# zxhuang1698/ZeroShape

Hardware: AMD Instinct MI355X
Metric: sdf_query_points_per_sec_vox128 (higher is better)
Workload: dtype f16x3; 1 GPU; compute_level_grid vox_res=128: (128+1)^3 = 2146689 points/image, range [-1.5,1.5], prologue + fused decoder (f32) + sigmoid; batch = n_gpus images, each sharded into equal point ranges, RCCL all_gather for n_gpus>1; global_batch_images=1, weights=seeded random (zeroshape_amd/synthetic.py)

## Files before the change

include/zeroshape_hip.h:

```cpp
#ifndef ZEROSHAPE_HIP_H
#define ZEROSHAPE_HIP_H

#include <stddef.h>
#include <stdint.h>

#ifdef __cplusplus
extern "C" {
#endif

#define ZS_ABI_VERSION 38

int zs_abi_version(void);

const char *zs_last_error(void);


int zs_chamfer_forward(const float *xyz1, const float *xyz2, int b, int n, int m,
                       float *dist1, float *dist2, int *idx1, int *idx2, void *stream);

size_t zs_chamfer_workspace_bytes(int b, int n, int m);
int zs_chamfer_forward_ws(const float *xyz1, const float *xyz2, int b, int n, int m,
                          float *dist1, float *dist2, int *idx1, int *idx2,
                          void *workspace, size_t workspace_bytes, void *stream);

int zs_chamfer_backward(const float *xyz1, const float *xyz2, int b, int n, int m,
                        float *gradxyz1, float *gradxyz2,
                        const float *graddist1, const float *graddist2,
                        const int *idx1, const int *idx2, void *stream);


size_t zs_sdf_program_bytes(void);
size_t zs_sdf_prologue_scratch_bytes(void);
size_t zs_sdf_workspace_bytes(void);
size_t zs_sdf_attn_scratch_bytes(int batch, int m);

int zs_sdf_prologue(void *programs, size_t program_stride_bytes, const float *lat_params,
                    const float *latent_depth, int batch, void *scratch, void *stream);
#define ZS_SDF_POS_PERLAYER 1
int zs_sdf_prologue_ex(void *programs, size_t program_stride_bytes, const float *lat_params,
                       const float *latent_depth, int batch, void *scratch, int flags, void *stream);

int zs_sdf_verdict_stats(const float *got, const float *want, int batch, int m, float flip_band, float tol, float tol_occ,
                         float *stats, int *flags, void *stream);

int zs_sdf_query_points(const void *programs, size_t program_stride_bytes, int batch,
                        const float *points, int m, float *logits, float *attn,
                        const int *tile_mask, void *workspace, void *stream);

int zs_sdf_query_grid(const void *programs, size_t program_stride_bytes, int batch,
                      const float *axis, int G, int slice_begin, int slice_end,
                      int apply_sigmoid, float *out, const int *tile_mask, void *workspace,
                      void *stream);

int zs_sdf_split_programs(const void *programs, size_t program_stride_bytes, void *split_programs,
                          size_t split_stride_bytes, int batch, void *stream);
int zs_sdf_query_points_split(const void *split_programs, size_t program_stride_bytes, int batch,
                              const float *points, int m, float *logits, int *tile_flags,
                              void *workspace, void *stream);
int zs_sdf_query_grid_split(const void *split_programs, size_t program_stride_bytes, int batch,
                            const float *axis, int G, int slice_begin, int slice_end,
                            int apply_sigmoid, float *out, int *tile_flags, void *workspace,
                            void *stream);

int zs_sdf_query_grid_range(const void *programs, size_t program_stride_bytes, int batch,
                            const float *axis, int G, long long point_begin, long long point_end,
                            int apply_sigmoid, float *out, const int *tile_mask, void *workspace,
                            void *stream);
int zs_sdf_query_grid_range_split(const void *split_programs, size_t program_stride_bytes, int batch,
                                  const float *axis, int G, long long point_begin,
                                  long long point_end, int apply_sigmoid, float *out,
                                  int *tile_flags, void *workspace, void *stream);

size_t zs_bf_grid_bytes(void);
size_t zs_bf_scratch_bytes(void);
int zs_bf_lower_bounds(const float *pred, int n, const float *gt_normalized, int m,
                       const float *rotations, int k, float *grid_gt, float *grid_pred,
                       void *scratch, float *lower_bounds, void *stream);

int zs_pose_max_batch(void);
size_t zs_pose_scratch_bytes(int n, int m, int count);
size_t zs_pose_best_bytes(void);
int zs_pose_best_init(float *best, void *stream);
int zs_pose_search_batch(const float *pred, int n, const float *gt_normalized, int m,
                         const float *rotations, const int *order, int count, int index_offset,
                         const float *lower_bound, const float *thresholds6, float *best,
                         void *scratch, void *stream);
size_t zs_pose_grid_bytes(int n, int m, int count);
int zs_pose_gt_grid(const float *gt_normalized, int m, void *grids, void *stream);
int zs_pose_search_batch_grid(const float *pred, int n, const float *gt_normalized, int m, const float *rotations,
                              const int *order, int count, int index_offset, const float *lower_bound,
                              const float *thresholds6, float *best, void *scratch, void *grids, const float *pred_stats,
                              void *stream);
size_t zs_morton_scratch_bytes(int n);
int zs_morton_sort(const float *points, int n, float *sorted, int *perm, float *tile_boxes, int tile, void *scratch,
                   void *stream);
size_t zs_str_scratch_bytes(int n);
int zs_str_sort(const float *points, int n, float *sorted, int *perm, void *scratch, void *stream);
size_t zs_pose_pack_bytes(int points);
int zs_pose_pack(const float *sorted_points, int points, float *pack, void *stream);
size_t zs_pose_sorted_scratch_bytes(int n, int m, int count);
int zs_pose_search_batch_sorted(const float *pred, const float *pred_sorted, int n, const float *gt_sorted,
                                const float *gt_pack, int m, const float *rotations, const int *order, int count,
                                int index_offset, const float *lower_bound, const float *thresholds6, float *best,
                                void *scratch, int mode, void *stream);
int zs_pose_apply(const float *pred, int n, const float *rotations, const int *index, float *out,
                  void *scratch, void *stream);
int zs_normalize_pc(const float *pc, int b, int n, float *out, void *scratch, void *stream);
int zs_standardize_pc(const float *pc, int b, int n, float *out, void *stream);
size_t zs_icp_scratch_bytes(int b);
int zs_icp_step(const float *x1, int n, const float *x2, int m, const int *idx1, int b, float *x1_out, void *scratch,
                void *stream);
int zs_fscore(const float *dist1, int n, const float *dist2, int m, int b, const float *thresholds,
              int n_thresholds, float *out, void *stream);

size_t zs_mc_scratch_bytes(int G);
size_t zs_mesh_sample_scratch_doubles(int n_tris);
int zs_mc_count(const float *vol, int G, float iso, const uint8_t *tri_count, void *scratch,
                int *total, void *stream);
int zs_mc_emit(const float *vol, int G, float iso, const int8_t *tri_table, int table_stride,
               const uint8_t *tri_count, const void *scratch, float scale, float offset,
               float *tris, int n_tris, void *stream);
int zs_mesh_sample(const float *tris, int n_tris, int n_samples, uint64_t seed, double *cum_area,
                   float *points, void *stream);

int zs_intr_param2mtx(const float *params, int batch, int H, int W, float *intr, void *stream);
int zs_unproj_depth(const float *depth, const float *intr, int batch, int H, int W, float *points,
                    void *stream);
int zs_valid_norm_fac(const float *points, const uint8_t *mask, int batch, int n, float *mean,
                      float *max_dist, void *stream);
int zs_masked_resample(const float *map, const float *mask, int batch, int channels, int H, int W,
                       int Ho, int Wo, float bg, float *out, float *mask_out, void *stream);
int zs_seen_surface(const float *depth, const float *intr, const float *mask, int batch, int H, int W,
                    int Ho, int Wo, float *seen_points, float *mean, float *scale, float *coord_dsp,
                    float *mask_dsp, void *stream);
size_t zs_seen_surface_workspace_bytes(int batch);
int zs_seen_surface_ws(const float *depth, const float *intr, const float *mask, int batch, int H, int W,
                       int Ho, int Wo, float *seen_points, float *mean, float *scale, float *coord_dsp,
                       float *mask_dsp, void *workspace, void *stream);

#define ZS_DEPTH_PRED_IS_DISPARITY 1
#define ZS_DEPTH_SOLVE_ONLY 2
int zs_depth_metrics(const float *prediction, const float *target, const float *mask, int batch, int n,
                     int flags, float depth_cap, const float *thresholds,
                     int n_thresholds, float *metrics, float *prediction_depth, float *scale_shift,
                     void *stream);

#define ZS_ACT_NONE 0
#define ZS_ACT_RELU 1
#define ZS_ACT_GELU 2
#define ZS_ACT_RELU_CLAMP1 3
#define ZS_ACT_SOFTPLUS 4
#define ZS_CONV_IN_RELU 1
#define ZS_CONV_FORCE_LARGE 2
#define ZS_CONV_FORCE_SMALL 4
#define ZS_CONV_F16X3 16
#define ZS_CONV_SPLIT_SMALL 32
#define ZS_CONV_STREAM_K 64
#define ZS_CONV_STREAM_K_ALWAYS 256
#define ZS_CONV_W_PRESPLIT 128
#define ZS_CONV_IN_DILATE2 8
#define ZS_CONV_FORCE_TILE256 1024
#define ZS_CONV_OUT_K16 2048
#define ZS_CONV_IN_K16 4096
#define ZS_CONV_IN_UPSAMPLE2 512
size_t zs_conv2d_packed_floats(int Cin, int Cout, int kh, int kw);
int zs_conv2d_presplit_weight(const float *packed_w, float *split_w, int Cin, int Cout, int kh, int kw, void *stream);
int zs_conv2d_presplit_weight_multi(const void *const *packed, void *const *split, const int *cout_pad,
                                    const unsigned long long *pair_prefix, int n, unsigned long long total_pairs,
                                    void *stream);
int zs_conv2d_nhwc(const float *in, const float *packed_w, const float *scale, const float *shift,
                   const float *res1, const float *res2, float *out, int batch, int Hin, int Win, int Cin,
                   int Hout, int Wout, int Cout, int kh, int kw, int stride, int pad_t, int pad_l, int flags,
                   float in_scale, float in_shift, int act, void *stream);
size_t zs_conv2d_splitk_workspace_bytes(void);
int zs_conv2d_nhwc_ws(const float *in, const float *packed_w, const float *scale, const float *shift,
                   const float *res1, const float *res2, float *out, int batch, int Hin, int Win, int Cin,
                   int Hout, int Wout, int Cout, int kh, int kw, int stride, int pad_t, int pad_l, int flags,
                   float in_scale, float in_shift, int act, void *workspace, void *stream);

typedef struct zs_conv_fuse {
    int in_mode, in_tiles, in_groups;
    int in_gshift;
    const float *in_stats, *in_gamma, *in_beta;
    float in_eps;
    int out_mode, out_groups;
    float *out_stats;
} zs_conv_fuse;
int zs_conv2d_nhwc_fused(const float *in, const float *packed_w, const float *scale, const float *shift,
                         const float *res1, const float *res2, float *out, int batch, int Hin, int Win,
                         int Cin, int Hout, int Wout, int Cout, int kh, int kw, int stride, int pad_t,
                         int pad_l, int flags, float in_scale, float in_shift, int act, const zs_conv_fuse *fuse,
                         void *workspace, void *stream);
int zs_conv2d_fused_cols(int M, int Cout);
int zs_conv2d_k16_ok(int M, int Cin, int Cout, int flags, int ln_in_tiles, int row_stats_out, int has_res);
int zs_gn_relu_max_pool_nhwc(const float *x, const float *stats, int tiles, const float *gamma, const float *beta,
                             float *table, float *y, int batch, int Hin, int Win, int C, int Hout, int Wout, int k,
                             int stride, int pad_t, int pad_l, float eps, void *stream);
int zs_group_norm_apply_stats(const float *x, const float *stats, int tiles, const float *gamma, const float *beta,
                              const float *residual, const float *res_stats, int res_tiles, const float *res_gamma,
                              const float *res_beta, float *y, int batch, int HW, int C, float eps, int relu, void *stream);
int zs_conv3x3_tail_nhwc(const float *in, const float *packed_w, const float *scale, const float *shift, float *out,
                         int batch, int H, int W, int Cin, int Cout, int flags, int act, const float *tail_w,
                         const float *tail_b, int tail_act, void *stream);
int zs_group_norm_nhwc(const float *x, const float *gamma, const float *beta, const float *residual, float *y,
                       int batch, int HW, int C, int groups, float eps, int relu, void *stream);
size_t zs_group_norm_workspace_bytes(int batch, int HW, int C, int groups);
int zs_group_norm_nhwc_ws(const float *x, const float *gamma, const float *beta, const float *residual, float *y,
                          int batch, int HW, int C, int groups, float eps, int relu, void *workspace, void *stream);
int zs_layer_norm(const float *x, const float *gamma, const float *beta, float *y, int rows, int C, float eps,
                  void *stream);
int zs_attention(const float *qkv, float *out, int batch, int L, int heads, int head_dim, void *stream);
int zs_attention_split(const float *qkv, float *out, int batch, int L, int heads, int head_dim, void *stream);
int zs_max_pool_nhwc(const float *x, float *y, int batch, int Hin, int Win, int C, int Hout, int Wout, int k,
                     int stride, int pad_t, int pad_l, void *stream);
int zs_global_mean_nhwc(const float *x, float *y, int batch, int HW, int C, void *stream);
int zs_upsample2x_nhwc(const float *x, float *y, int batch, int Hin, int Win, int C, void *stream);
int zs_nchw_to_nhwc(const float *x, const float *mask, float *y, int batch, int C, int HW, int Cpad,
                    void *stream);
int zs_nhwc_to_nchw(const float *x, float *y, int batch, int C, int HW, void *stream);
int zs_assemble_tokens(const float *feat, const float *cls, const float *pos, float *tokens, int batch, int n,
                       int C, void *stream);
int zs_readout_concat(const float *tokens, float *out, int batch, int n, int C, void *stream);
int zs_window_tokens(const float *emb, const uint8_t *mask, const float *invalid_token, const float *cls,
                     const float *pos, float *out, int batch, int H, int W, int C, int win, void *stream);

typedef struct zs_tensor_entry {
    float *param;
    const float *grad;
    float *exp_avg, *exp_avg_sq;
    unsigned long long n;
    float lr, weight_decay;
} zs_tensor_entry;

int zs_pack_conv_weight(const float *w, float *packed, int Cout, int Cin, int cin0, int CinTot, int kh, int kw,
                        int dgrad, void *stream);
typedef struct zs_pack_entry {
    const float *src;
    float *dst;
    int Cout, Cin, cin0, ld, taps, dgrad, K16, NPad;
} zs_pack_entry;
int zs_pack_chunk_elems(void);
int zs_pack_entry_chunks(int Cout, int Cin, int taps, int dgrad, int K16, int NPad);
int zs_pack_conv_weight_multi(const zs_pack_entry *table, const int *chunk_entry, const unsigned long long *chunk_start,
                              int n_chunks, void *stream);
int zs_pack_entry_inline_split(int Cout, int Cin, int taps, int dgrad);
int zs_pack_conv_weight_multi_split(const zs_pack_entry *table, const int *chunk_entry,
                                    const unsigned long long *chunk_start, int n_chunks, float *const *split_dst,
                                    int split_only, void *stream);
size_t zs_conv2d_wgrad_workspace_bytes(int batch, int Hout, int Wout, int Cin, int Cout, int kh, int kw);
int zs_conv2d_wgrad(const float *in, const float *dy, float *dw, float *db, void *workspace, int batch, int Hin, int Win,
                    int CinP, int Hout, int Wout, int Cout, int kh, int kw, int stride, int pad_t, int pad_l,
                    int flags, float in_scale, float in_shift, int Cin, int cin0, int CinTot, int accumulate,
                    void *stream);
int zs_conv2d_dgrad_small_cin(const float *dy, const float *w, float *dx, int batch, int H, int W, int CinP, int Hout,
                              int Wout, int Cout, int kh, int kw, int stride, int pad_t, int pad_l, int Cin, int cin0,
                              int CinTot, float scale, void *stream);
int zs_standardize_weight(const float *w, float *out, int Cout, int n, float eps, void *stream);
typedef struct zs_std_entry {
    const float *w;
    float *out;
    int rows, n;
    float eps;
    int pad;
} zs_std_entry;
int zs_standardize_weight_multi(const zs_std_entry *table, const int *row_prefix, int n_entries, int total_rows, void *stream);
int zs_standardize_weight_bwd(const float *w, const float *grad_out, float *dw, int Cout, int n, float eps,
                              void *stream);
int zs_act_forward(const float *x, float *y, size_t n, int act, float beta, void *stream);
int zs_act_backward(const float *dy, const float *ref, float *dx, size_t n, int act, float beta, void *stream);
int zs_posenc3d(const float *points, size_t n, int L, float *out, int stride, void *stream);
int zs_add_scaled_rows(const float *x, const float *branch, const float *scale, float *y, int batch,
                       size_t per_sample, void *stream);
size_t zs_column_sum_workspace_bytes(int rows, int C);
int zs_column_sum(const float *x, float *out, int rows, int C, float scale, void *workspace, void *stream);
size_t zs_layer_norm_bwd_workspace_bytes(int rows, int C);
int zs_layer_norm_bwd(const float *dy, const float *x, const float *gamma, float *dx, float *dgamma, float *dbeta,
                      int rows, int C, float eps, void *workspace, void *stream);
int zs_layer_norm_bwd_add(const float *dy, const float *x, const float *gamma, const float *add, float *dx, float *dgamma,
                          float *dbeta, int rows, int C, float eps, void *workspace, void *stream);
size_t zs_attention_bwd_workspace_bytes(int batch, int L, int heads);
int zs_attention_bwd(const float *qkv, const float *dout, float *dqkv, void *workspace, int batch, int L, int heads,
                     int head_dim, void *stream);
int zs_point_attention(const float *qkv_points, const float *qkv_latent, float *out, int batch, int M, int Ll,
                       int heads, int head_dim, void *stream);
int zs_point_attention_probs(const float *qkv_points, const float *qkv_latent, float *attn, int batch, int M, int Ll,
                             int heads, int head_dim, float weight, int accumulate, void *stream);
size_t zs_point_attention_bwd_workspace_bytes(int batch, int M, int Ll, int heads);
int zs_point_attention_bwd(const float *qkv_points, const float *qkv_latent, const float *dout, float *dqkv_points,
                           float *dqkv_latent, int accumulate_latent, void *workspace, int batch, int M, int Ll,
                           int heads, int head_dim, void *stream);
size_t zs_bce_logits_workspace_bytes(size_t n);
int zs_bce_logits(const float *logits, const float *sdf, size_t n, float impt_thres, float impt_weight, float *loss,
                  void *workspace, void *stream);
int zs_bce_logits_bwd(const float *logits, const float *sdf, size_t n, float impt_thres, float impt_weight,
                      const float *grad_loss, float *dlogits, void *stream);
int zs_erode_mask(const float *mask, int batch, int H, int W, int pool, float *out, void *stream);
size_t zs_midas_loss_workspace_bytes(int batch);
int zs_midas_loss(const float *prediction, const float *target, const float *mask, int batch, int H, int W, float alpha,
                  int scales, int inverse_depth, float *loss, void *workspace, void *stream);
int zs_midas_loss_bwd(const float *prediction, const float *target, const float *mask, int batch, int H, int W,
                      float alpha, int scales, int inverse_depth, const void *workspace, const float *grad_loss,
                      float *dprediction, void *stream);
int zs_intr_loss(const float *seen_pred, const float *seen_gt, const float *mask, size_t n, float *out2, void *stream);
int zs_intr_loss_bwd(const float *seen_pred, const float *seen_gt, const float *mask, size_t n, const float *out2,
                     const float *grad_loss, float *dseen_pred, void *stream);
int zs_multi_tensor_chunk_elems(void);
int zs_adamw_multi(const zs_tensor_entry *table, const int *chunk_tensor, const unsigned long long *chunk_start,
                   int n_chunks, float beta1, float beta2, float eps, int step, const float *grad_scale,
                   const int *skipped_steps, void *stream);
int zs_copy_multi(const zs_tensor_entry *table, const int *chunk_tensor, const unsigned long long *chunk_start,
                  int n_chunks, float scale, void *stream);
int zs_sumsq_multi(const zs_tensor_entry *table, const int *chunk_tensor, const unsigned long long *chunk_start,
                   int n_chunks, float *partial, float *sumsq, void *stream);

size_t zs_batch_norm_workspace_bytes(int rows, int C);
int zs_batch_norm_train(const float *x, const float *gamma, const float *beta, const float *residual, float *y,
                        float *running_mean, float *running_var, float *save_mean, float *save_rstd, int rows, int C,
                        float eps, float momentum, int relu, void *workspace, void *stream);
int zs_batch_norm_bwd(const float *x, const float *dy, const float *y_relu, const float *gamma, const float *save_mean,
                      const float *save_rstd, float *dx, float *dresidual, float *dgamma, float *dbeta, int rows, int C,
                      void *workspace, void *stream);
size_t zs_group_norm_bwd_workspace_bytes(int batch, int C);
int zs_group_norm_bwd(const float *x, const float *dy, const float *y_relu, const float *gamma, float *dx,
                      float *dresidual, float *dgamma, float *dbeta, int batch, int HW, int C, int groups, float eps,
                      void *workspace, void *stream);
int zs_max_pool_bwd_nhwc(const float *x, const float *dy, float *dx, int batch, int Hin, int Win, int C, int Hout,
                         int Wout, int k, int stride, int pad_t, int pad_l, void *stream);
int zs_global_mean_bwd_nhwc(const float *dy, float *dx, int batch, int HW, int C, void *stream);
int zs_upsample2x_bwd_nhwc(const float *dy, float *dx, int batch, int Hin, int Win, int C, void *stream);
int zs_nhwc_to_nchw_masked(const float *x, const float *mask, float *y, int batch, int C, int HW, int Cpad,
                           void *stream);
int zs_seen_surface_bwd(const float *depth, const float *intr, const float *mask, const float *mean, const float *scale,
                        const float *d_seen_points, const float *d_coord_dsp, int batch, int H, int W, float *d_depth,
                        float *d_intr, void *stream);
int zs_intr_param2mtx_bwd(const float *params, const float *d_intr, int batch, int H, int W, float *d_params,
                          void *stream);
int zs_window_tokens_bwd(const float *d_out, const uint8_t *mask, float *d_emb, float *d_inv_rows, float *d_cls_rows,
                         int batch, int H, int W, int C, int win, void *stream);
int zs_coord_dsp2_bwd(const float *d_dsp, const float *mask, const float *mask_dsp, float *d_full, int batch, int H,
                      int W, void *stream);
int zs_transform_points(const float *points, const float *pose, const float *mean, const float *scale, float *out,
                        int batch, int n, void *stream);
int zs_resize_bilinear_nhwc(const float *x, float *y, int Hi, int Wi, int Ho, int Wo, int C, int backward,
                            void *stream);
int zs_readout_concat_bwd(const float *dout, float *dtokens, int batch, int n, int C, void *stream);

#ifdef __cplusplus
}
#endif
#endif
```

zeroshape_amd/_lib.py:

```python
import contextlib
import ctypes
import os

_HERE = os.path.dirname(os.path.abspath(__file__))
LIB_PATH = os.environ.get("ZS_LIB_PATH") or os.path.join(_HERE, "libzeroshape_hip.so")

_c_void_p = ctypes.c_void_p
_c_int = ctypes.c_int
_c_size_t = ctypes.c_size_t
_c_float = ctypes.c_float

class ConvFuse(ctypes.Structure):
    _fields_ = [("in_mode", ctypes.c_int), ("in_tiles", ctypes.c_int), ("in_groups", ctypes.c_int), ("in_gshift", ctypes.c_int),
                ("in_stats", ctypes.c_void_p), ("in_gamma", ctypes.c_void_p), ("in_beta", ctypes.c_void_p),
                ("in_eps", ctypes.c_float), ("out_mode", ctypes.c_int), ("out_groups", ctypes.c_int),
                ("out_stats", ctypes.c_void_p)]


SIGNATURES = {
    "zs_abi_version": (_c_int, []),
    "zs_last_error": (ctypes.c_char_p, []),
    "zs_chamfer_forward": (_c_int, [_c_void_p, _c_void_p, _c_int, _c_int, _c_int,
                                    _c_void_p, _c_void_p, _c_void_p, _c_void_p, _c_void_p]),
    "zs_chamfer_workspace_bytes": (_c_size_t, [_c_int, _c_int, _c_int]),
    "zs_chamfer_forward_ws": (_c_int, [_c_void_p, _c_void_p, _c_int, _c_int, _c_int,
                                       _c_void_p, _c_void_p, _c_void_p, _c_void_p, _c_void_p, _c_size_t,
                                       _c_void_p]),
    "zs_chamfer_backward": (_c_int, [_c_void_p, _c_void_p, _c_int, _c_int, _c_int,
                                     _c_void_p, _c_void_p, _c_void_p, _c_void_p,
                                     _c_void_p, _c_void_p, _c_void_p]),
    "zs_sdf_program_bytes": (_c_size_t, []),
    "zs_sdf_prologue_scratch_bytes": (_c_size_t, []),
    "zs_sdf_workspace_bytes": (_c_size_t, []),
    "zs_sdf_attn_scratch_bytes": (_c_size_t, [_c_int, _c_int]),
    "zs_sdf_prologue": (_c_int, [_c_void_p, _c_size_t, _c_void_p, _c_void_p, _c_int,
                                 _c_void_p, _c_void_p]),
    "zs_sdf_prologue_ex": (_c_int, [_c_void_p, _c_size_t, _c_void_p, _c_void_p, _c_int,
                                    _c_void_p, _c_int, _c_void_p]),
    "zs_sdf_verdict_stats": (_c_int, [_c_void_p, _c_void_p, _c_int, _c_int, _c_float, _c_float, _c_float, _c_void_p, _c_void_p,
                                      _c_void_p]),
    "zs_sdf_query_points": (_c_int, [_c_void_p, _c_size_t, _c_int, _c_void_p, _c_int,
                                     _c_void_p, _c_void_p, _c_void_p, _c_void_p, _c_void_p]),
    "zs_sdf_query_grid": (_c_int, [_c_void_p, _c_size_t, _c_int, _c_void_p, _c_int, _c_int,
                                   _c_int, _c_int, _c_void_p, _c_void_p, _c_void_p, _c_void_p]),
    "zs_sdf_split_programs": (_c_int, [_c_void_p, _c_size_t, _c_void_p, _c_size_t, _c_int, _c_void_p]),
    "zs_sdf_query_points_split": (_c_int, [_c_void_p, _c_size_t, _c_int, _c_void_p, _c_int,
                                           _c_void_p, _c_void_p, _c_void_p, _c_void_p]),
    "zs_sdf_query_grid_split": (_c_int, [_c_void_p, _c_size_t, _c_int, _c_void_p, _c_int, _c_int,
                                         _c_int, _c_int, _c_void_p, _c_void_p, _c_void_p, _c_void_p]),
    "zs_sdf_query_grid_range": (_c_int, [_c_void_p, _c_size_t, _c_int, _c_void_p, _c_int, ctypes.c_longlong,
                                         ctypes.c_longlong, _c_int, _c_void_p, _c_void_p, _c_void_p, _c_void_p]),
    "zs_sdf_query_grid_range_split": (_c_int, [_c_void_p, _c_size_t, _c_int, _c_void_p, _c_int,
                                               ctypes.c_longlong, ctypes.c_longlong, _c_int, _c_void_p,
                                               _c_void_p, _c_void_p, _c_void_p]),
    "zs_erode_mask": (_c_int, [_c_void_p, _c_int, _c_int, _c_int, _c_int, _c_void_p, _c_void_p]),
    "zs_bf_grid_bytes": (_c_size_t, []),
    "zs_bf_scratch_bytes": (_c_size_t, []),
    "zs_bf_lower_bounds": (_c_int, [_c_void_p, _c_int, _c_void_p, _c_int, _c_void_p, _c_int, _c_void_p,
                                    _c_void_p, _c_void_p, _c_void_p, _c_void_p]),
    "zs_pose_max_batch": (_c_int, []),
    "zs_pose_scratch_bytes": (_c_size_t, [_c_int, _c_int, _c_int]),
    "zs_pose_best_bytes": (_c_size_t, []),
    "zs_pose_best_init": (_c_int, [_c_void_p, _c_void_p]),
    "zs_pose_search_batch": (_c_int, [_c_void_p, _c_int, _c_void_p, _c_int, _c_void_p, _c_void_p, _c_int, _c_int,
                                      _c_void_p, _c_void_p, _c_void_p, _c_void_p, _c_void_p]),
    "zs_pose_grid_bytes": (_c_size_t, [_c_int, _c_int, _c_int]),
    "zs_pose_gt_grid": (_c_int, [_c_void_p, _c_int, _c_void_p, _c_void_p]),
    "zs_pose_search_batch_grid": (_c_int, [_c_void_p, _c_int, _c_void_p, _c_int, _c_void_p, _c_void_p, _c_int, _c_int,
                                           _c_void_p, _c_void_p, _c_void_p, _c_void_p, _c_void_p, _c_void_p, _c_void_p]),
    "zs_morton_scratch_bytes": (_c_size_t, [_c_int]),
    "zs_morton_sort": (_c_int, [_c_void_p, _c_int, _c_void_p, _c_void_p, _c_void_p, _c_int, _c_void_p, _c_void_p]),
    "zs_str_scratch_bytes": (_c_size_t, [_c_int]),
    "zs_str_sort": (_c_int, [_c_void_p, _c_int, _c_void_p, _c_void_p, _c_void_p, _c_void_p]),
    "zs_pose_pack_bytes": (_c_size_t, [_c_int]),
    "zs_pose_pack": (_c_int, [_c_void_p, _c_int, _c_void_p, _c_void_p]),
    "zs_pose_sorted_scratch_bytes": (_c_size_t, [_c_int, _c_int, _c_int]),
    "zs_pose_search_batch_sorted": (_c_int, [_c_void_p, _c_void_p, _c_int, _c_void_p, _c_void_p, _c_int, _c_void_p,
                                             _c_void_p, _c_int, _c_int, _c_void_p, _c_void_p, _c_void_p, _c_void_p,
                                             _c_int, _c_void_p]),
    "zs_pose_apply": (_c_int, [_c_void_p, _c_int, _c_void_p, _c_void_p, _c_void_p, _c_void_p, _c_void_p]),
    "zs_standardize_pc": (_c_int, [_c_void_p, _c_int, _c_int, _c_void_p, _c_void_p]),
    "zs_icp_scratch_bytes": (_c_size_t, [_c_int]),
    "zs_icp_step": (_c_int, [_c_void_p, _c_int, _c_void_p, _c_int, _c_void_p, _c_int, _c_void_p, _c_void_p, _c_void_p]),
    "zs_normalize_pc": (_c_int, [_c_void_p, _c_int, _c_int, _c_void_p, _c_void_p, _c_void_p]),
    "zs_fscore": (_c_int, [_c_void_p, _c_int, _c_void_p, _c_int, _c_int, _c_void_p, _c_int, _c_void_p, _c_void_p]),
    "zs_mc_scratch_bytes": (_c_size_t, [_c_int]),
    "zs_mesh_sample_scratch_doubles": (_c_size_t, [_c_int]),
    "zs_mc_count": (_c_int, [_c_void_p, _c_int, ctypes.c_float, _c_void_p, _c_void_p, _c_void_p, _c_void_p]),
    "zs_mc_emit": (_c_int, [_c_void_p, _c_int, ctypes.c_float, _c_void_p, _c_int, _c_void_p, _c_void_p,
                            ctypes.c_float, ctypes.c_float, _c_void_p, _c_int, _c_void_p]),
    "zs_mesh_sample": (_c_int, [_c_void_p, _c_int, _c_int, ctypes.c_uint64, _c_void_p, _c_void_p, _c_void_p]),
    "zs_intr_param2mtx": (_c_int, [_c_void_p, _c_int, _c_int, _c_int, _c_void_p, _c_void_p]),
    "zs_unproj_depth": (_c_int, [_c_void_p, _c_void_p, _c_int, _c_int, _c_int, _c_void_p, _c_void_p]),
    "zs_valid_norm_fac": (_c_int, [_c_void_p, _c_void_p, _c_int, _c_int, _c_void_p, _c_void_p, _c_void_p]),
    "zs_masked_resample": (_c_int, [_c_void_p, _c_void_p, _c_int, _c_int, _c_int, _c_int, _c_int, _c_int,
                                    ctypes.c_float, _c_void_p, _c_void_p, _c_void_p]),
    "zs_seen_surface": (_c_int, [_c_void_p, _c_void_p, _c_void_p, _c_int, _c_int, _c_int, _c_int, _c_int,
                                 _c_void_p, _c_void_p, _c_void_p, _c_void_p, _c_void_p, _c_void_p]),
    "zs_seen_surface_workspace_bytes": (_c_size_t, [_c_int]),
    "zs_seen_surface_ws": (_c_int, [_c_void_p, _c_void_p, _c_void_p, _c_int, _c_int, _c_int, _c_int, _c_int,
                                    _c_void_p, _c_void_p, _c_void_p, _c_void_p, _c_void_p, _c_void_p, _c_void_p]),
    "zs_depth_metrics": (_c_int, [_c_void_p, _c_void_p, _c_void_p, _c_int, _c_int, _c_int, ctypes.c_float,
                                  ctypes.POINTER(ctypes.c_float), _c_int, _c_void_p, _c_void_p, _c_void_p,
                                  _c_void_p]),
    "zs_conv2d_packed_floats": (_c_size_t, [_c_int, _c_int, _c_int, _c_int]),
    "zs_conv2d_presplit_weight": (_c_int, [_c_void_p, _c_void_p, _c_int, _c_int, _c_int, _c_int, _c_void_p]),
    "zs_conv2d_nhwc": (_c_int, [_c_void_p] * 7 + [_c_int] * 13 + [ctypes.c_float, ctypes.c_float, _c_int,
                                                                  _c_void_p]),
    "zs_conv2d_splitk_workspace_bytes": (_c_size_t, []),
    "zs_conv2d_presplit_weight_multi": (_c_int, [_c_void_p] * 4 + [_c_int, ctypes.c_ulonglong, _c_void_p]),
    "zs_conv3x3_tail_nhwc": (_c_int, [_c_void_p] * 5 + [_c_int] * 7 + [_c_void_p, _c_void_p, _c_int, _c_void_p]),
    "zs_conv2d_nhwc_ws": (_c_int, [_c_void_p] * 7 + [_c_int] * 13 + [ctypes.c_float, ctypes.c_float, _c_int,
                                                                     _c_void_p, _c_void_p]),
    "zs_conv2d_nhwc_fused": (_c_int, [_c_void_p] * 7 + [_c_int] * 13 + [ctypes.c_float, ctypes.c_float, _c_int,
                                                                        _c_void_p, _c_void_p, _c_void_p]),
    "zs_conv2d_fused_cols": (_c_int, [_c_int, _c_int]),
    "zs_conv2d_k16_ok": (_c_int, [_c_int] * 7),
    "zs_gn_relu_max_pool_nhwc": (_c_int, [_c_void_p, _c_void_p, _c_int] + [_c_void_p] * 4 + [_c_int] * 10 + [ctypes.c_float, _c_void_p]),
    "zs_group_norm_apply_stats": (_c_int, [_c_void_p, _c_void_p, _c_int] + [_c_void_p] * 4 + [_c_int] + [_c_void_p] * 3 +
                                  [_c_int, _c_int, _c_int, ctypes.c_float, _c_int, _c_void_p]),
    "zs_group_norm_nhwc": (_c_int, [_c_void_p] * 5 + [_c_int, _c_int, _c_int, _c_int, ctypes.c_float, _c_int,
                                                      _c_void_p]),
    "zs_group_norm_workspace_bytes": (_c_size_t, [_c_int, _c_int, _c_int, _c_int]),
    "zs_group_norm_nhwc_ws": (_c_int, [_c_void_p] * 5 + [_c_int, _c_int, _c_int, _c_int, ctypes.c_float, _c_int,
                                       _c_void_p, _c_void_p]),
    "zs_layer_norm": (_c_int, [_c_void_p] * 4 + [_c_int, _c_int, ctypes.c_float, _c_void_p]),
    "zs_attention": (_c_int, [_c_void_p, _c_void_p, _c_int, _c_int, _c_int, _c_int, _c_void_p]),
    "zs_attention_split": (_c_int, [_c_void_p, _c_void_p, _c_int, _c_int, _c_int, _c_int, _c_void_p]),
    "zs_max_pool_nhwc": (_c_int, [_c_void_p, _c_void_p] + [_c_int] * 10 + [_c_void_p]),
    "zs_global_mean_nhwc": (_c_int, [_c_void_p, _c_void_p, _c_int, _c_int, _c_int, _c_void_p]),
    "zs_upsample2x_nhwc": (_c_int, [_c_void_p, _c_void_p, _c_int, _c_int, _c_int, _c_int, _c_void_p]),
    "zs_nchw_to_nhwc": (_c_int, [_c_void_p, _c_void_p, _c_void_p, _c_int, _c_int, _c_int, _c_int, _c_void_p]),
    "zs_window_tokens": (_c_int, [_c_void_p] * 6 + [_c_int] * 5 + [_c_void_p]),
    "zs_nhwc_to_nchw": (_c_int, [_c_void_p, _c_void_p, _c_int, _c_int, _c_int, _c_void_p]),
    "zs_assemble_tokens": (_c_int, [_c_void_p] * 4 + [_c_int, _c_int, _c_int, _c_void_p]),
    "zs_readout_concat": (_c_int, [_c_void_p, _c_void_p, _c_int, _c_int, _c_int, _c_void_p]),
    "zs_pack_conv_weight": (_c_int, [_c_void_p, _c_void_p] + [_c_int] * 7 + [_c_void_p]),
    "zs_pack_chunk_elems": (_c_int, []),
    "zs_pack_entry_chunks": (_c_int, [_c_int] * 6),
    "zs_pack_conv_weight_multi": (_c_int, [_c_void_p, _c_void_p, _c_void_p, _c_int, _c_void_p]),
    "zs_pack_entry_inline_split": (_c_int, [_c_int] * 4),
    "zs_pack_conv_weight_multi_split": (_c_int, [_c_void_p, _c_void_p, _c_void_p, _c_int, _c_void_p, _c_int, _c_void_p]),
    "zs_conv2d_wgrad_workspace_bytes": (_c_size_t, [_c_int] * 7),
    "zs_conv2d_wgrad": (_c_int, [_c_void_p] * 5 + [_c_int] * 13 + [_c_float, _c_float] + [_c_int] * 4 + [_c_void_p]),
    "zs_conv2d_dgrad_small_cin": (_c_int, [_c_void_p] * 3 + [_c_int] * 15 + [_c_float, _c_void_p]),
    "zs_standardize_weight": (_c_int, [_c_void_p, _c_void_p, _c_int, _c_int, _c_float, _c_void_p]),
    "zs_standardize_weight_multi": (_c_int, [_c_void_p, _c_void_p, _c_int, _c_int, _c_void_p]),
    "zs_standardize_weight_bwd": (_c_int, [_c_void_p, _c_void_p, _c_void_p, _c_int, _c_int, _c_float, _c_void_p]),
    "zs_act_forward": (_c_int, [_c_void_p, _c_void_p, _c_size_t, _c_int, _c_float, _c_void_p]),
    "zs_act_backward": (_c_int, [_c_void_p, _c_void_p, _c_void_p, _c_size_t, _c_int, _c_float, _c_void_p]),
    "zs_posenc3d": (_c_int, [_c_void_p, _c_size_t, _c_int, _c_void_p, _c_int, _c_void_p]),
    "zs_add_scaled_rows": (_c_int, [_c_void_p] * 4 + [_c_int, _c_size_t, _c_void_p]),
    "zs_column_sum_workspace_bytes": (_c_size_t, [_c_int, _c_int]),
    "zs_column_sum": (_c_int, [_c_void_p, _c_void_p, _c_int, _c_int, _c_float, _c_void_p, _c_void_p]),
    "zs_layer_norm_bwd_workspace_bytes": (_c_size_t, [_c_int, _c_int]),
    "zs_layer_norm_bwd": (_c_int, [_c_void_p] * 6 + [_c_int, _c_int, _c_float, _c_void_p, _c_void_p]),
    "zs_layer_norm_bwd_add": (_c_int, [_c_void_p] * 7 + [_c_int, _c_int, _c_float, _c_void_p, _c_void_p]),
    "zs_attention_bwd_workspace_bytes": (_c_size_t, [_c_int, _c_int, _c_int]),
    "zs_attention_bwd": (_c_int, [_c_void_p] * 4 + [_c_int] * 4 + [_c_void_p]),
    "zs_point_attention": (_c_int, [_c_void_p] * 3 + [_c_int] * 5 + [_c_void_p]),
    "zs_point_attention_probs": (_c_int, [_c_void_p, _c_void_p, _c_void_p, _c_int, _c_int, _c_int, _c_int, _c_int, _c_float, _c_int,
                                          _c_void_p]),
    "zs_point_attention_bwd_workspace_bytes": (_c_size_t, [_c_int] * 4),
    "zs_point_attention_bwd": (_c_int, [_c_void_p] * 5 + [_c_int, _c_void_p] + [_c_int] * 5 + [_c_void_p]),
    "zs_bce_logits_workspace_bytes": (_c_size_t, [_c_size_t]),
    "zs_bce_logits": (_c_int, [_c_void_p, _c_void_p, _c_size_t, _c_float, _c_float, _c_void_p, _c_void_p,
                               _c_void_p]),
    "zs_bce_logits_bwd": (_c_int, [_c_void_p, _c_void_p, _c_size_t, _c_float, _c_float, _c_void_p, _c_void_p,
                                   _c_void_p]),
    "zs_midas_loss_workspace_bytes": (_c_size_t, [_c_int]),
    "zs_midas_loss": (_c_int, [_c_void_p] * 3 + [_c_int] * 3 + [_c_float, _c_int, _c_int, _c_void_p, _c_void_p, _c_void_p]),
    "zs_midas_loss_bwd": (_c_int, [_c_void_p] * 3 + [_c_int] * 3 + [_c_float, _c_int, _c_int, _c_void_p, _c_void_p,
                                                                    _c_void_p, _c_void_p]),
    "zs_intr_loss": (_c_int, [_c_void_p] * 3 + [_c_size_t, _c_void_p, _c_void_p]),
    "zs_intr_loss_bwd": (_c_int, [_c_void_p] * 3 + [_c_size_t] + [_c_void_p] * 4),
    "zs_multi_tensor_chunk_elems": (_c_int, []),
    "zs_adamw_multi": (_c_int, [_c_void_p, _c_void_p, _c_void_p, _c_int, _c_float, _c_float, _c_float, _c_int,
                                _c_void_p, _c_void_p, _c_void_p]),
    "zs_copy_multi": (_c_int, [_c_void_p, _c_void_p, _c_void_p, _c_int, _c_float, _c_void_p]),
    "zs_sumsq_multi": (_c_int, [_c_void_p, _c_void_p, _c_void_p, _c_int, _c_void_p, _c_void_p, _c_void_p]),
    "zs_batch_norm_workspace_bytes": (_c_size_t, [_c_int, _c_int]),
    "zs_batch_norm_train": (_c_int, [_c_void_p] * 9 + [_c_int, _c_int, _c_float, _c_float, _c_int, _c_void_p,
                                                       _c_void_p]),
    "zs_batch_norm_bwd": (_c_int, [_c_void_p] * 10 + [_c_int, _c_int, _c_void_p, _c_void_p]),
    "zs_group_norm_bwd_workspace_bytes": (_c_size_t, [_c_int, _c_int]),
    "zs_group_norm_bwd": (_c_int, [_c_void_p] * 8 + [_c_int, _c_int, _c_int, _c_int, _c_float, _c_void_p, _c_void_p]),
    "zs_max_pool_bwd_nhwc": (_c_int, [_c_void_p] * 3 + [_c_int] * 10 + [_c_void_p]),
    "zs_global_mean_bwd_nhwc": (_c_int, [_c_void_p, _c_void_p, _c_int, _c_int, _c_int, _c_void_p]),
    "zs_upsample2x_bwd_nhwc": (_c_int, [_c_void_p, _c_void_p, _c_int, _c_int, _c_int, _c_int, _c_void_p]),
    "zs_nhwc_to_nchw_masked": (_c_int, [_c_void_p, _c_void_p, _c_void_p, _c_int, _c_int, _c_int, _c_int, _c_void_p]),
    "zs_seen_surface_bwd": (_c_int, [_c_void_p] * 7 + [_c_int, _c_int, _c_int, _c_void_p, _c_void_p, _c_void_p]),
    "zs_intr_param2mtx_bwd": (_c_int, [_c_void_p, _c_void_p, _c_int, _c_int, _c_int, _c_void_p, _c_void_p]),
    "zs_window_tokens_bwd": (_c_int, [_c_void_p] * 5 + [_c_int] * 5 + [_c_void_p]),
    "zs_coord_dsp2_bwd": (_c_int, [_c_void_p] * 4 + [_c_int] * 3 + [_c_void_p]),
    "zs_transform_points": (_c_int, [_c_void_p] * 5 + [_c_int, _c_int, _c_void_p]),
    "zs_resize_bilinear_nhwc": (_c_int, [_c_void_p, _c_void_p] + [_c_int] * 6 + [_c_void_p]),
    "zs_readout_concat_bwd": (_c_int, [_c_void_p, _c_void_p, _c_int, _c_int, _c_int, _c_void_p]),
}

ABI_VERSION = 38
_lib = None


class ZeroShapeHipError(RuntimeError):
    pass


def load():
    global _lib
    if _lib is not None:
        return _lib
    if not os.path.exists(LIB_PATH):
        raise ZeroShapeHipError(
            "HIP library not built: %s is missing (run `python -m zeroshape_amd.build`). "
            "zeroshape_amd has no CPU/PyTorch fallback for this path." % LIB_PATH)
    import torch
    try:
        lib = ctypes.CDLL(LIB_PATH)
    except OSError as e:
        raise ZeroShapeHipError("cannot load %s: %s" % (LIB_PATH, e)) from e
    for name, (res, args) in SIGNATURES.items():
        try:
            fn = getattr(lib, name)
        except AttributeError as e:
            raise ZeroShapeHipError("%s does not export %s" % (LIB_PATH, name)) from e
        fn.restype = res
        fn.argtypes = args
    v = lib.zs_abi_version()
    if v != ABI_VERSION:
        raise ZeroShapeHipError("ABI mismatch: library %d, binding %d" % (v, ABI_VERSION))
    _lib = lib
    return lib


CALLS = [0]


def check(rc, what):
    CALLS[0] += 1
    if rc != 1:
        msg = load().zs_last_error()
        raise ZeroShapeHipError("%s failed: %s" % (what, (msg or b"").decode(errors="replace")))


def ptr(t):
    return None if t is None else ctypes.c_void_p(t.data_ptr())


def current_stream_ptr(device=None):
    import torch
    idx = getattr(device, "index", device)
    if idx is None:
        idx = torch.cuda.current_device()
    return ctypes.c_void_p(torch._C._cuda_getCurrentRawStream(idx))


_NULL_GUARD = contextlib.nullcontext()


def on(device):
    import torch
    idx = getattr(device, "index", device)
    if idx is None or idx == torch.cuda.current_device():
        return _NULL_GUARD
    return torch.cuda.device(device)
```

zeroshape_amd/csrc/sdf_decoder_split.hip:

```cpp
#include "zs_common.h"
#include <stdlib.h>
#include "sdf_layout.h"
#include "sdf_math.h"
#include "zs_split16.h"
#include "../../include/zeroshape_hip.h"

#include <math.h>
#include <stdint.h>
#include <type_traits>

namespace {

using namespace zs::lay;
using zs::dm::gelu_erf;
using zs::dm::softplus100;

typedef float f32x16 __attribute__((ext_vector_type(16)));
typedef float f32x4 __attribute__((ext_vector_type(4)));
typedef float f32x2 __attribute__((ext_vector_type(2)));
typedef unsigned u32x4 __attribute__((ext_vector_type(4)));

constexpr float S_GUARD = 64.0f;
constexpr int WAVES = 4;
constexpr int PTS_PER_WAVE = 32;
constexpr int PTS_PER_BLOCK = WAVES * PTS_PER_WAVE;
constexpr int MAX_WGS = 256;
constexpr int KB_U4 = 128;
constexpr int CK = 8;
constexpr int KPW = CK / WAVES;
constexpr int CHUNK_BYTES = CK * KB_U4 * 16;
constexpr int NBUF = 2;
constexpr int KB_TOTAL = G_TOTAL / 2;
constexpr int PRM_WINDOW = 4096;
constexpr int STAGE_FLOATS = NBUF * CHUNK_BYTES / 4;
constexpr int SLAB_TILES = NT - 1;
constexpr int SLAB_U4 = SLAB_TILES * 4 * 64;
constexpr int ZTILES_F4 = NT * 4 * 64;
constexpr int ZSLAB_F4 = 3 * ZTILES_F4;
constexpr int LDS_FLOATS = PRM_WINDOW + STAGE_FLOATS + WAVES * SLAB_U4 * 4;
static_assert(LDS_FLOATS * 4 == 160 * 1024, "the kernel owns the whole LDS of a CU");
static_assert(KB_TOTAL % CK == 0 && CK % WAVES == 0 && KPW * 2048 <= 4096, "chunking");
static_assert((RING * GROUP_FLOATS + PARAM_FLOATS) * 4 >= NBUF * CHUNK_BYTES, "prefetch stays inside the program");

constexpr int W_PP = P_PP;
constexpr int W_BLK = P_BLK0;
constexpr int W_IA = P_LNFG;
constexpr int W_IB = P_IMPL_PAIR + P_IMPL_PAIR_STRIDE;
static_assert(P_BLK_STRIDE <= PRM_WINDOW && W_IB - W_IA <= PRM_WINDOW && P_USED - W_IB <= PRM_WINDOW,
              "params windows");

#define DEV __device__ __forceinline__
#ifdef ZS_FENCE_SCHED
#define ZS_FENCE __builtin_amdgcn_sched_barrier(0)
#else
#define ZS_FENCE do { } while (0)
#endif

DEV void pin(u32x4 &a, u32x4 &b) { asm volatile("" : "+v"(a), "+v"(b) : : "memory"); }

using zs::s16::mfma3;
using zs::s16::split2;

struct PT {
    u32x4 v[4];
};
template <typename T>
DEV PT pack_tile(const T &x) {
    PT p;
#pragma unroll
    for (int j = 0; j < 2; j++)
#pragma unroll
        for (int i = 0; i < 4; i++) {
            unsigned h, l;
            split2(x[8 * j + 2 * i], x[8 * j + 2 * i + 1], h, l);
            p.v[2 * j][i] = h;
            p.v[2 * j + 1][i] = l;
        }
    return p;
}

DEV void glds_kblocks(const char *gsrc, unsigned lds_dst) {
#ifdef ZS_EXP_NO_DMA
    if (gsrc != nullptr) return;
#endif
#ifndef ZS_DMA_MOD
#define ZS_DMA_MOD ""
#endif
    asm volatile("s_mov_b32 m0, %1\n\ts_nop 0\n\tglobal_load_lds_dwordx4 %0, off" ZS_DMA_MOD
                 "\n\tglobal_load_lds_dwordx4 %0, off offset:1024" ZS_DMA_MOD
                 "\n\tglobal_load_lds_dwordx4 %0, off offset:2048" ZS_DMA_MOD
                 "\n\tglobal_load_lds_dwordx4 %0, off offset:3072" ZS_DMA_MOD
                 :
                 : "v"(gsrc), "s"(lds_dst)
                 : "memory");
}

struct AStream {
    const u32x4 *buf[NBUF];
    unsigned dst[NBUF];
    u32x4 hi, lo;
    const char *gsrc;

    DEV void init(const char *prog, u32x4 *stage, unsigned stage_addr, int wave, int lane) {
        const char *g = prog + wave * (KPW * KB_U4 * 16) + lane * 16;
        asm volatile("s_waitcnt vmcnt(0) lgkmcnt(0)\n\ts_barrier" ::: "memory");
#pragma unroll
        for (int i = 0; i < NBUF; i++) {
            buf[i] = stage + i * (CK * KB_U4) + lane;
            dst[i] = stage_addr + i * CHUNK_BYTES + wave * (KPW * KB_U4 * 16);
            glds_kblocks(g + i * CHUNK_BYTES, dst[i]);
        }
        gsrc = g + NBUF * CHUNK_BYTES;
        asm volatile("s_waitcnt vmcnt(4)\n\ts_barrier" ::: "memory");
        hi = buf[0][0];
        lo = buf[0][64];
    }
    template <int EXTRA_VM = 0>
    DEV void step(int pos, u32x4 &ahi, u32x4 &alo) {
        ahi = hi;
        alo = lo;
        if (pos == CK - 1) {
            static_assert(EXTRA_VM == 0 || EXTRA_VM == 4, "wait-count variants");
            if (EXTRA_VM == 4)
                asm volatile("s_waitcnt vmcnt(4) lgkmcnt(0)\n\ts_barrier" ::: "memory");
            else
                asm volatile("s_waitcnt vmcnt(0) lgkmcnt(0)\n\ts_barrier" ::: "memory");
            glds_kblocks(gsrc, dst[0]);
            gsrc += CHUNK_BYTES;
            const u32x4 *t = buf[0];
            const unsigned u = dst[0];
            buf[0] = buf[1];
            dst[0] = dst[1];
            buf[1] = t;
            dst[1] = u;
            hi = buf[0][0];
            lo = buf[0][64];
        } else {
#ifndef ZS_EXP_NO_AREAD
            hi = buf[0][(pos + 1) * KB_U4];
            lo = buf[0][(pos + 1) * KB_U4 + 64];
#endif
        }
    }
    DEV void drain() { asm volatile("s_waitcnt vmcnt(0) lgkmcnt(0)" ::: "memory"); }
};

struct Slab {
    u32x4 *fl;
    PT t7;
    DEV void store(int tile, const PT &p) {
        if (tile == SLAB_TILES) {
            t7 = p;
        } else {
#pragma unroll
            for (int q = 0; q < 4; q++) fl[(tile * 4 + q) * 64] = p.v[q];
        }
    }
};

DEV f32x16 zero16() {
    f32x16 v;
#pragma unroll
    for (int r = 0; r < 16; r++) v[r] = 0.f;
    return v;
}

struct NoSide {
    DEV void operator()(int, int) const {}
};
template <typename SIDE>
DEV void mfma3_gaps(f32x16 &acc, const u32x4 &ahi, const u32x4 &alo, const u32x4 &bhi, const u32x4 &blo, int kb,
                    SIDE &side) {
    using zs::s16::as_h;
    if (std::is_same<SIDE, NoSide>::value) {
        mfma3(acc, ahi, alo, bhi, blo);
        return;
    }
    acc = __builtin_amdgcn_mfma_f32_32x32x16_f16(as_h(alo), as_h(bhi), acc, 0, 0, 0);
    ZS_FENCE;
    side(kb, 0);
    ZS_FENCE;
    acc = __builtin_amdgcn_mfma_f32_32x32x16_f16(as_h(ahi), as_h(blo), acc, 0, 0, 0);
    ZS_FENCE;
    side(kb, 1);
    ZS_FENCE;
    acc = __builtin_amdgcn_mfma_f32_32x32x16_f16(as_h(ahi), as_h(bhi), acc, 0, 0, 0);
    ZS_FENCE;
    side(kb, 2);
    ZS_FENCE;
}

struct TilePacker {
    PT p;
    float prev;
    DEV void feed(int kb, float v) {
        if (kb & 1) {
            unsigned h, l;
            split2(prev, v, h, l);
            p.v[2 * (kb >> 3)][(kb & 7) >> 1] = h;
            p.v[2 * (kb >> 3) + 1][(kb & 7) >> 1] = l;
        }
        prev = v;
    }
};

struct GeluStager {
    float x, u, q, t, e, p;
    DEV void s0(float v) {
        x = v;
        u = fabsf(v) * 0.70710678118654752440f;
        q = (u * u) * -1.44269504088896340736f;
    }
    DEV void s1() { t = __builtin_amdgcn_rcpf(fmaf(0.3275911f, u, 1.0f)); }
    DEV void s2() {
        e = __builtin_amdgcn_exp2f(q);
        p = fmaf(0.75052702f, t, -1.02753365f);
    }
    DEV void s3() {
        p = fmaf(p, t, 1.00509130f);
        p = fmaf(p, t, -0.20116957f);
        p = fmaf(p, t, 0.18019173f);
        p = p * t;
        u = u * p;
    }
    DEV float s4() const { return fmaf(-u, e, fmaxf(x, 0.0f)); }
    DEV float all(float v) {
        s0(v); s1(); s2(); s3();
        return s4();
    }
    DEV void stage(int st, float v, int idx, TilePacker &pk) {
        if (st == 0) s0(v);
        else if (st == 1) s1();
        else if (st == 2) s2();
        else if (st == 3) s3();
        else if (st == 4) pk.feed(idx, s4());
    }
};
struct SoftplusStager {
    float x, t;
    DEV void s0(float v) {
        x = v;
        t = __builtin_amdgcn_exp2f(fabsf(v) * -144.26950408889634074f);
    }
    DEV void s1() { t = __builtin_amdgcn_logf(1.0f + t); }
    DEV float s2() const { return fmaf(t, 0.0069314718055994530942f, fmaxf(x, 0.0f)); }
};

DEV float kblock_gelu(f32x16 &acc, const u32x4 &ahi, const u32x4 &alo, const u32x4 &bhi, const u32x4 &blo, float x) {
    float u, q, d, t, e, m, p;
    const float c0 = 0.70710678118654752440f, c1 = 0.3275911f, c2 = -1.02753365f;
    asm volatile(
#ifndef ZS_EXP_TWO_TERM
                 "v_mfma_f32_32x32x16_f16 %[acc], %[alo], %[bh], %[acc]\n\t"
#endif
                 "v_mul_f32_e64 %[u], |%[x]|, %[c0]\n\t"
                 "v_mul_f32_e32 %[q], %[u], %[u]\n\t"
                 "v_mul_f32_e32 %[q], 0xbfb8aa3b, %[q]\n\t"
                 "v_fma_f32 %[d], %[u], %[c1], 1.0\n\t"
                 "v_mfma_f32_32x32x16_f16 %[acc], %[ahi], %[bl], %[acc]\n\t"
                 "v_rcp_f32_e32 %[t], %[d]\n\t"
                 "v_exp_f32_e32 %[e], %[q]\n\t"
                 "v_max_f32_e32 %[m], 0, %[x]\n\t"
                 "v_mfma_f32_32x32x16_f16 %[acc], %[ahi], %[bh], %[acc]\n\t"
                 "v_fmamk_f32 %[p], %[t], 0x3f40228a, %[c2]\n\t"
                 "v_fmaak_f32 %[p], %[p], %[t], 0x3f80a6d5\n\t"
                 "v_fmaak_f32 %[p], %[p], %[t], 0xbe4dff65\n\t"
                 "v_fmaak_f32 %[p], %[p], %[t], 0x3e38842e\n\t"
                 "v_mul_f32_e64 %[p], %[t], -%[p]\n\t"
                 "v_mul_f32_e32 %[p], %[u], %[p]\n\t"
                 "v_fmac_f32_e32 %[m], %[p], %[e]"
                 : [acc] "+v"(acc), [u] "=&v"(u), [q] "=&v"(q), [d] "=&v"(d), [t] "=&v"(t), [e] "=&v"(e), [m] "=&v"(m),
                   [p] "=&v"(p)
                 : [alo] "v"(alo), [ahi] "v"(ahi), [bh] "v"(bhi), [bl] "v"(blo), [x] "v"(x), [c0] "s"(c0), [c1] "s"(c1),
                   [c2] "v"(c2));
    return m;
}
DEV float kblock_softplus(f32x16 &acc, const u32x4 &ahi, const u32x4 &alo, const u32x4 &bhi, const u32x4 &blo, float x) {
    float t, m;
    const float c0 = -144.26950408889634074f;
    asm volatile(
#ifndef ZS_EXP_TWO_TERM
                 "v_mfma_f32_32x32x16_f16 %[acc], %[alo], %[bh], %[acc]\n\t"
#endif
                 "v_mul_f32_e64 %[t], |%[x]|, %[c0]\n\t"
                 "v_exp_f32_e32 %[t], %[t]\n\t"
                 "v_mfma_f32_32x32x16_f16 %[acc], %[ahi], %[bl], %[acc]\n\t"
                 "v_max_f32_e32 %[m], 0, %[x]\n\t"
                 "v_add_f32_e32 %[t], 1.0, %[t]\n\t"
                 "v_log_f32_e32 %[t], %[t]\n\t"
                 "v_mfma_f32_32x32x16_f16 %[acc], %[ahi], %[bh], %[acc]\n\t"
                 "s_nop 0\n\t"
                 "v_fmac_f32_e32 %[m], 0x3be32166, %[t]"
                 : [acc] "+v"(acc), [t] "=&v"(t), [m] "=&v"(m)
                 : [alo] "v"(alo), [ahi] "v"(ahi), [bh] "v"(bhi), [bl] "v"(blo), [x] "v"(x), [c0] "s"(c0));
    return m;
}

template <int KT, int EXTRA_VM = 0, typename SIDE = NoSide>
DEV void gemm_reg(AStream &s, const PT *X, f32x16 &acc, SIDE side = SIDE()) {
#pragma unroll
    for (int kt = 0; kt < KT; kt++)
#pragma unroll
        for (int j = 0; j < 2; j++) {
            u32x4 ahi, alo;
            s.step((kt * 2 + j) & (CK - 1), ahi, alo);
            pin(ahi, alo);
            mfma3_gaps(acc, ahi, alo, X[kt].v[2 * j], X[kt].v[2 * j + 1], kt * 2 + j, side);
        }
}
template <typename SIDE>
DEV void mfma3_breg(f32x16 &acc, const u32x4 &ahi, const u32x4 &alo, const u32x4 &bhi, const u32x4 &blo, int kb,
                    SIDE &side) {
    asm volatile("s_nop 1\n\tv_mfma_f32_32x32x16_f16 %0, %1, %2, %0" : "+v"(acc) : "v"(alo), "a"(bhi));
    ZS_FENCE;
    side(kb, 0);
    ZS_FENCE;
    asm volatile("s_nop 1\n\tv_mfma_f32_32x32x16_f16 %0, %1, %2, %0" : "+v"(acc) : "v"(ahi), "a"(blo));
    ZS_FENCE;
    side(kb, 1);
    ZS_FENCE;
    asm volatile("s_nop 1\n\tv_mfma_f32_32x32x16_f16 %0, %1, %2, %0" : "+v"(acc) : "v"(ahi), "a"(bhi));
    ZS_FENCE;
    side(kb, 2);
    ZS_FENCE;
}
template <int KT, typename SIDE = NoSide>
DEV void gemm_areg(AStream &s, const PT *X, f32x16 &acc, SIDE side = SIDE()) {
#pragma unroll
    for (int kt = 0; kt < KT; kt++)
#pragma unroll
        for (int j = 0; j < 2; j++) {
            u32x4 ahi, alo;
            s.step((kt * 2 + j) & (CK - 1), ahi, alo);
            pin(ahi, alo);
            mfma3_breg(acc, ahi, alo, X[kt].v[2 * j], X[kt].v[2 * j + 1], kt * 2 + j, side);
        }
}
template <typename SIDE>
DEV void mfma3_cacc(f32x16 &acc, const u32x4 &ahi, const u32x4 &alo, const u32x4 &bhi, const u32x4 &blo, int kb,
                    SIDE &side) {
    asm volatile("s_nop 1\n\tv_mfma_f32_32x32x16_f16 %0, %1, %2, %0" : "+a"(acc) : "v"(alo), "v"(bhi));
    ZS_FENCE;
    side(kb, 0);
    ZS_FENCE;
    asm volatile("s_nop 1\n\tv_mfma_f32_32x32x16_f16 %0, %1, %2, %0" : "+a"(acc) : "v"(ahi), "v"(blo));
    ZS_FENCE;
    side(kb, 1);
    ZS_FENCE;
    asm volatile("s_nop 1\n\tv_mfma_f32_32x32x16_f16 %0, %1, %2, %0" : "+a"(acc) : "v"(ahi), "v"(bhi));
    ZS_FENCE;
    side(kb, 2);
    ZS_FENCE;
}
template <bool YACC = false, typename SIDE = NoSide>
DEV void gemm_one(AStream &s, const PT &X, f32x16 &acc, int pos0, int kb0 = 0, SIDE side = SIDE()) {
#pragma unroll
    for (int j = 0; j < 2; j++) {
        u32x4 ahi, alo;
        s.step((pos0 + j) & (CK - 1), ahi, alo);
        pin(ahi, alo);
        if (YACC)
            mfma3_cacc(acc, ahi, alo, X.v[2 * j], X.v[2 * j + 1], kb0 + j, side);
        else
            mfma3_gaps(acc, ahi, alo, X.v[2 * j], X.v[2 * j + 1], kb0 + j, side);
    }
}
DEV void slab_b(const Slab &sl, int kb, u32x4 &bh, u32x4 &bl) {
    if (kb >= SLAB_TILES * 2) {
        bh = sl.t7.v[(kb & 1) * 2];
        bl = sl.t7.v[(kb & 1) * 2 + 1];
    } else {
        bh = sl.fl[kb * KB_U4];
        bl = sl.fl[kb * KB_U4 + 64];
    }
}
template <typename SIDE = NoSide>
DEV void gemm_lds(AStream &s, const Slab &sl, f32x16 &acc, int pos0 = 0, SIDE side = SIDE()) {
    u32x4 bh, bl;
    slab_b(sl, 0, bh, bl);
#pragma unroll
    for (int kb = 0; kb < NT * 2; kb++) {
        u32x4 ahi, alo;
        s.step((pos0 + kb) & (CK - 1), ahi, alo);
        u32x4 nh = bh, nl = bl;
        if (kb + 1 < NT * 2) slab_b(sl, kb + 1, nh, nl);
        pin(ahi, alo);
        mfma3_gaps(acc, ahi, alo, bh, bl, kb, side);
        bh = nh;
        bl = nl;
    }
}

template <int ACT, typename FIN, typename TAIL>
DEV void gemm_lds_act(AStream &s, const Slab &sl, f32x16 &acc, const f32x16 &cur, FIN fin, TAIL tail) {
    u32x4 bh, bl;
    slab_b(sl, 0, bh, bl);
#pragma unroll
    for (int kb = 0; kb < NT * 2; kb++) {
        u32x4 ahi, alo;
        s.step(kb & (CK - 1), ahi, alo);
        u32x4 nh = bh, nl = bl;
        if (kb + 1 < NT * 2) slab_b(sl, kb + 1, nh, nl);
        const float r = ACT == 0 ? kblock_gelu(acc, ahi, alo, bh, bl, cur[kb]) : kblock_softplus(acc, ahi, alo, bh, bl, cur[kb]);
        bh = nh;
        bl = nl;
        fin(kb, r);
        tail(kb);
    }
}
template <int ACT, typename FIN, typename TAIL>
DEV void gemm_reg_act(AStream &s, const PT *X, f32x16 &acc, const f32x16 &cur, FIN fin, TAIL tail) {
#pragma unroll
    for (int kt = 0; kt < NT; kt++)
#pragma unroll
        for (int j = 0; j < 2; j++) {
            u32x4 ahi, alo;
            const int kb = kt * 2 + j;
            s.step(kb & (CK - 1), ahi, alo);
            const float r = ACT == 0 ? kblock_gelu(acc, ahi, alo, X[kt].v[2 * j], X[kt].v[2 * j + 1], cur[kb])
                                     : kblock_softplus(acc, ahi, alo, X[kt].v[2 * j], X[kt].v[2 * j + 1], cur[kb]);
            fin(kb, r);
            tail(kb);
        }
}

#ifndef ZS_SPLIT_PERMLANE
DEV float half_sum(float v) { return v + __shfl_xor(v, 32, 64); }
DEV float half_max(float v) { return fmaxf(v, __shfl_xor(v, 32, 64)); }
#else
DEV void half_pair(float v, float &lo, float &hi) {
    lo = v;
    hi = v;
    asm volatile("s_nop 4\n\tv_permlane32_swap_b32 %0, %1\n\ts_nop 4" : "+v"(lo), "+v"(hi));
}
DEV float half_sum(float v) {
    float lo, hi;
    half_pair(v, lo, hi);
    return lo + hi;
}
#ifdef ZS_SPLIT_PERMLANE_SUM_ONLY
DEV float half_max(float v) { return fmaxf(v, __shfl_xor(v, 32, 64)); }
#else
DEV float half_max(float v) {
    float lo, hi;
    half_pair(v, lo, hi);
    return fmaxf(lo, hi);
}
#endif
#endif

DEV void rp(const float *prm, int off, int tile, int hi, float *v) {
    const f32x4 *q = reinterpret_cast<const f32x4 *>(prm + off + tile * 32 + hi * 16);
#pragma unroll
    for (int i = 0; i < 4; i++) {
        const f32x4 a = q[i];
        v[4 * i + 0] = a.x; v[4 * i + 1] = a.y; v[4 * i + 2] = a.z; v[4 * i + 3] = a.w;
    }
}
DEV f32x16 rp16(const float *prm, int off, int tile, int hi) {
    float t[16];
    rp(prm, off, tile, hi, t);
    f32x16 v;
#pragma unroll
    for (int r = 0; r < 16; r++) v[r] = t[r];
    return v;
}
DEV f32x16 xyz_affine(const float *prm, int off, int tile, int hi, float x, float y, float z) {
    const f32x4 *q = reinterpret_cast<const f32x4 *>(prm + off + tile * 128 + hi * 64);
    f32x16 v;
#pragma unroll
    for (int r = 0; r < 16; r++) {
        const f32x4 w = q[r];
        v[r] = fmaf(w.z, z, fmaf(w.y, y, fmaf(w.x, x, w.w)));
    }
    return v;
}

struct XyzInit {
    const f32x4 *q;
    f32x4 w;
    f32x16 v;
    DEV void start(const float *prm, int off, int tile, int hi) {
        q = reinterpret_cast<const f32x4 *>(prm + off + tile * 128 + hi * 64);
        w = q[0];
    }
    DEV void step(int r, float x, float y, float z) {
        v[r] = fmaf(w.z, z, fmaf(w.y, y, fmaf(w.x, x, w.w)));
        if (r + 1 < 16) w = q[r + 1];
    }
};
struct RowInit {
    const f32x4 *q;
    f32x4 w;
    f32x16 v;
    DEV void start(const float *prm, int off, int tile, int hi) {
        q = reinterpret_cast<const f32x4 *>(prm + off + tile * 32 + hi * 16);
        w = q[0];
    }
    DEV void step(int r) {
        if ((r & 3) == 0) {
            v[r] = w.x; v[r + 1] = w.y; v[r + 2] = w.z; v[r + 3] = w.w;
            if (r + 4 < 16) w = q[(r >> 2) + 1];
        }
    }
};

DEV void ln_stats(const f32x16 *x, float &mean, float &rstd) {
    float s = 0.f;
#pragma unroll
    for (int kt = 0; kt < NT; kt++)
#pragma unroll
        for (int r = 0; r < 16; r++) s += x[kt][r];
    s = half_sum(s);
    mean = s * (1.0f / 256.0f);
    float v = 0.f;
#pragma unroll
    for (int kt = 0; kt < NT; kt++)
#pragma unroll
        for (int r = 0; r < 16; r++) {
            const float d = x[kt][r] - mean;
            v = fmaf(d, d, v);
        }
    v = half_sum(v);
    rstd = 1.0f / sqrtf(v * (1.0f / 256.0f) + 1e-6f);
}
DEV void layer_norm_lds(const f32x16 *x, Slab &sl, const float *prm, int g_off, int b_off, int hi) {
    float mean, rstd;
    ln_stats(x, mean, rstd);
#pragma unroll
    for (int kt = 0; kt < NT; kt++) {
        float g[16], b[16], t[16];
        rp(prm, g_off, kt, hi, g);
        rp(prm, b_off, kt, hi, b);
#pragma unroll
        for (int r = 0; r < 16; r++) t[r] = fmaf((x[kt][r] - mean) * rstd, g[r], b[r]);
        sl.store(kt, pack_tile(t));
    }
}

DEV void load_params(float *prm, const float *prog_params, int start, int count) {
    __syncthreads();
    const f32x4 *src = reinterpret_cast<const f32x4 *>(prog_params + start);
    f32x4 *dst = reinterpret_cast<f32x4 *>(prm);
    for (int i = threadIdx.x; i < count / 4; i += WAVES * 64) dst[i] = src[i];
    __syncthreads();
}

template <bool MASK>
DEV void attn_tile(AStream &s, const PT &q, f32x16 &o, float &m_run, float &z_run, float c, int hi,
                   int pos0) {
    f32x16 S = zero16();
    gemm_one(s, q, S, pos0);
    float mt = -INFINITY;
#pragma unroll
    for (int r = 0; r < 16; r++) {
        if (MASK) {
            const int rw = (r & 3) + 8 * (r >> 2) + 4 * hi;
            S[r] = rw < L - 32 * (LT - 1) ? S[r] : -INFINITY;
        }
        mt = fmaxf(mt, S[r]);
    }
    mt *= c;
    constexpr float LAZY = 8.0f;
    if (__builtin_amdgcn_ballot_w64(mt > m_run + LAZY) != 0) {
        mt = half_max(mt);
        const float m_new = fmaxf(m_run, mt);
        const float alpha = __builtin_amdgcn_exp2f(m_run - m_new);
        z_run *= alpha;
#pragma unroll
        for (int r = 0; r < 16; r++) o[r] *= alpha;
        m_run = m_new;
    }
    float zs_ = 0.f;
#pragma unroll
    for (int r = 0; r < 16; r++) {
        const float p = __builtin_amdgcn_exp2f(fmaf(S[r], c, -m_run));
        S[r] = p;
        zs_ += p;
    }
    z_run += zs_;
    gemm_one(s, pack_tile(S), o, pos0 + 2);
}

#ifdef ZS_EXP_TIMING
#define ZS_STAMP(i) do { if (dbg) dbg[i] = __builtin_amdgcn_s_memtime(); } while (0)
#else
#define ZS_STAMP(i) do { } while (0)
#endif
DEV float decode_tile(const char *prog, float *prm, u32x4 *stage, unsigned stage_addr, u32x4 *slab,
                      f32x4 *zs, float px, float py, float pz, int wave, int lane, float &guard,
                      unsigned long long *dbg) {
    const int hi = lane >> 5;
    const float *prog_params = reinterpret_cast<const float *>(prog) + REC_FLOATS;
    AStream s;
    s.init(prog, stage, stage_addr, wave, lane);
    Slab sl;
    sl.fl = slab;
    ZS_STAMP(0);

    load_params(prm, prog_params, W_PP, 1024);
    f32x16 y[NT];
#pragma unroll
    for (int kt = 0; kt < NT; kt++) y[kt] = xyz_affine(prm, 0, kt, hi, px, py, pz);

    ZS_STAMP(1);

    const float scale = 0.17677669529663688110f;

#pragma unroll 1
    for (int blk = 0; blk < BLOCKS; blk++) {
        load_params(prm, prog_params, W_BLK + blk * P_BLK_STRIDE, P_BLK_STRIDE);
        layer_norm_lds(y, sl, prm, PB_LN1G, PB_LN1B, hi);
        ZS_STAMP(2 + blk * 4);
#pragma unroll
        for (int nt = 0; nt < NT; nt++) y[nt] += rp16(prm, PB_BPROJ, nt, hi);

        auto head = [&](int hd, auto Ptag) {
            constexpr int P = decltype(Ptag)::value;
            f32x16 q = rp16(prm, PB_BQKV, hd * 3 + 0, hi);
            gemm_lds(s, sl, q, P);
            f32x16 k = rp16(prm, PB_BQKV, hd * 3 + 1, hi);
            gemm_lds(s, sl, k, P);
            f32x16 v = rp16(prm, PB_BQKV, hd * 3 + 2, hi);
            gemm_lds(s, sl, v, P);

            const float c = scale * 1.44269504088896340736f;
            float s_self = 0.f;
            float qq = 0.f;
#pragma unroll
            for (int r = 0; r < 16; r++) {
                s_self = fmaf(q[r], k[r], s_self);
                qq = fmaf(q[r], q[r], qq);
            }
            s_self = half_sum(s_self) * c;
            {
                const float km = prog_params[P_KMAX + blk * HEADS + hd] * scale;
                guard = fmaxf(guard, half_sum(qq) * (km * km));
            }
            const PT qp = pack_tile(q);

            float m_run = -INFINITY, z_run = 0.f;
            f32x16 o = zero16();
#pragma unroll 1
            for (int l2 = 0; l2 < (LT - 1) / 2; l2++) {
                attn_tile<false>(s, qp, o, m_run, z_run, c, hi, P);
                attn_tile<false>(s, qp, o, m_run, z_run, c, hi, (P + 4) & (CK - 1));
            }
            attn_tile<true>(s, qp, o, m_run, z_run, c, hi, P);
            {
                const float m_new = fmaxf(m_run, s_self);
                const float alpha = __builtin_amdgcn_exp2f(m_run - m_new);
                const float p_self = __builtin_amdgcn_exp2f(s_self - m_new);
                const float z = fmaf(half_sum(z_run), alpha, p_self);
                const float inv = 1.0f / z;
                const float a_i = alpha * inv, p_i = p_self * inv;
#pragma unroll
                for (int r = 0; r < 16; r++) o[r] = fmaf(p_i, v[r], o[r] * a_i);
            }
            const PT op = pack_tile(o);
#pragma unroll
            for (int nt = 0; nt < NT; nt++) gemm_one(s, op, y[nt], (P + 4 + 2 * nt) & (CK - 1));
        };
        static_assert((LT - 1) % 2 == 0 && (3 * NT * 2 + LT * 4 + NT * 2) % CK == 4, "head = 11.5 chunks");
#pragma unroll 1
        for (int hd = 0; hd < HEADS; hd += 2) {
            head(hd, std::integral_constant<int, 0>());
            head(hd + 1, std::integral_constant<int, 4>());
        }

        ZS_STAMP(3 + blk * 4);
        layer_norm_lds(y, sl, prm, PB_LN2G, PB_LN2B, hi);
#pragma unroll
        for (int nt = 0; nt < NT; nt++) y[nt] += rp16(prm, PB_B2, nt, hi);
        ZS_STAMP(4 + blk * 4);
        RowInit bi;
        f32x16 hid = rp16(prm, PB_B1, 0, hi);
        bi.start(prm, PB_B1, 1, hi);
        gemm_lds(s, sl, hid, 0, [&](int kb, int g) {
            if (g == 2 && (kb & 3) == 1) bi.step(kb & ~3);
        });
#pragma unroll 1
        for (int ht = 0; ht < HT - 1; ht++) {
            f32x16 nxt = bi.v;
            bi.start(prm, PB_B1, ht + 2 < HT ? ht + 2 : HT - 1, hi);
            TilePacker e;
            gemm_lds_act<0>(s, sl, nxt, hid, [&](int kb, float r) { e.feed(kb, r); },
                            [&](int kb) { if ((kb & 3) == 1) bi.step(kb & ~3); });
#pragma unroll
            for (int nt = 0; nt < NT; nt++) gemm_one(s, e.p, y[nt], (2 * nt) & (CK - 1));
            hid = nxt;
        }
        {
#pragma unroll
            for (int r = 0; r < 16; r++) hid[r] = gelu_erf(hid[r]);
            const PT hp = pack_tile(hid);
#pragma unroll
            for (int nt = 0; nt < NT; nt++) gemm_one(s, hp, y[nt], (2 * nt) & (CK - 1));
        }
        ZS_STAMP(5 + blk * 4);
    }

    load_params(prm, prog_params, W_IA, W_IB - W_IA);
    float h[NT * 16];
    {
        float mean, rstd;
        ln_stats(y, mean, rstd);
#pragma unroll
        for (int kt = 0; kt < NT; kt++) {
            float g[16], b[16];
            rp(prm, P_LNFG - W_IA, kt, hi, g);
            rp(prm, P_LNFB - W_IA, kt, hi, b);
#pragma unroll
            for (int r = 0; r < 16; r++) h[kt * 16 + r] = fmaf((y[kt][r] - mean) * rstd, g[r], b[r]);
        }
    }
    ZS_STAMP(10);
    PT hp[NT];

#pragma unroll
    for (int kt = 0; kt < NT; kt++) hp[kt] = pack_tile(h + kt * 16);
    {
        f32x16 prev;
        XyzInit ini;
        ini.v = xyz_affine(prm, P_IMPL0 - W_IA, 0, hi, px, py, pz);
#pragma unroll
        for (int nt = 0; nt <= NT; nt++) {
            TilePacker e;
            if (nt < NT) {
                f32x16 acc = ini.v;
                if (nt + 1 < NT) ini.start(prm, P_IMPL0 - W_IA, nt + 1, hi);
                if (nt > 0)
                    gemm_reg_act<1>(s, hp, acc, prev, [&](int kb, float r) { e.feed(kb, r); },
                                    [&](int kb) { if (nt + 1 < NT) ini.step(kb, px, py, pz); });
                else
                    gemm_reg<NT, 0>(s, hp, acc, [&](int kb, int g) { if (g == 2) ini.step(kb, px, py, pz); });
                if (nt > 0) sl.store(nt - 1, e.p);
                prev = acc;
            } else {
#pragma unroll
                for (int kb = 0; kb < 16; kb++) e.feed(kb, softplus100(prev[kb]));
                sl.store(nt - 1, e.p);
            }
        }
    }
    ZS_STAMP(11);
    const float rsqrt2 = 0.70710678118654752440f;
    PT fp[NT];
#pragma unroll
    for (int kt = 0; kt < NT; kt++) {
        float t[16];
#pragma unroll
        for (int r = 0; r < 16; r++) t[r] = h[kt * 16 + r] * rsqrt2;
        fp[kt] = pack_tile(t);
    }
    const float sx = px * rsqrt2, sy = py * rsqrt2, sz = pz * rsqrt2;

    ZS_STAMP(12);
    {
        f32x16 prev;
        RowInit ini;
        ini.v = rp16(prm, P_IMPL1 - W_IA, 0, hi);
#pragma unroll
        for (int nt = 0; nt <= NT; nt++) {
            TilePacker e;
            if (nt < NT) {
                f32x16 acc = ini.v;
                if (nt + 1 < NT) ini.start(prm, P_IMPL1 - W_IA, nt + 1, hi);
                if (nt > 0)
                    gemm_lds_act<1>(s, sl, acc, prev, [&](int kb, float r) { e.feed(kb, r * rsqrt2); },
                                    [&](int kb) { if (nt + 1 < NT) ini.step(kb); });
                else
                    gemm_lds(s, sl, acc, 0, [&](int kb, int g) { if (g == 2) ini.step(kb); });
                if (nt > 0) hp[nt - 1] = e.p;
                prev = acc;
            } else {
#pragma unroll
                for (int kb = 0; kb < 16; kb++) e.feed(kb, softplus100(prev[kb]) * rsqrt2);
                hp[nt - 1] = e.p;
            }
        }
    }
    ZS_STAMP(13);
    float out = 0.f;
#pragma unroll 1
    for (int i = 0; i < 3; i++) {
        if (i == 1) load_params(prm, prog_params, W_IB, P_USED - W_IB);
        const int pp = i == 0 ? P_IMPL_PAIR - W_IA : (i - 1) * P_IMPL_PAIR_STRIDE;
        {
            f32x16 prev;
            XyzInit ini;
            ini.v = xyz_affine(prm, pp, 0, hi, sx, sy, sz);
#pragma unroll
            for (int nt = 0; nt <= NT; nt++) {
                TilePacker e;
                if (nt < NT) {
                    f32x16 acc = ini.v;
                    if (nt + 1 < NT) ini.start(prm, pp, nt + 1, hi);
                    if (nt > 0)
                        gemm_reg_act<1>(s, hp, acc, prev, [&](int kb, float r) { e.feed(kb, r); }, [&](int) {});
                    else
                        gemm_reg<NT>(s, hp, acc);
                    gemm_areg<NT>(s, fp, acc, [&](int kb, int g) {
                        if (g == 2 && nt + 1 < NT) ini.step(kb, sx, sy, sz);
                    });
                    if (nt > 0) sl.store(nt - 1, e.p);
                    prev = acc;
                } else {
#pragma unroll
                    for (int kb = 0; kb < 16; kb++) e.feed(kb, softplus100(prev[kb]));
                    sl.store(nt - 1, e.p);
                }
            }
        }
        const float post = i < 2 ? rsqrt2 : 1.0f;
        {
            f32x16 prev;
            RowInit ini, w8;
            const float wsel = i == 2 ? 1.0f : 0.0f;
            ini.v = rp16(prm, pp + 1024, 0, hi);
#pragma unroll
            for (int r = 0; r < 16; r++) w8.v[r] = 0.f;
#pragma unroll
            for (int nt = 0; nt <= NT; nt++) {
                TilePacker e;
                const f32x16 w = w8.v * wsel;
                auto finish = [&](int kb, float v) {
                    const float t = v * post;
                    e.feed(kb, t);
                    out = fmaf(t, w[kb], out);
                };
                if (nt < NT) {
                    f32x16 acc = ini.v;
                    if (nt + 1 < NT) ini.start(prm, pp + 1024, nt + 1, hi);
                    w8.start(prm, P_W8 - W_IB, nt, hi);
                    auto tail = [&](int kb) {
                        if (nt + 1 < NT) ini.step(kb);
                        w8.step(kb);
                    };
                    if (nt > 0)
                        gemm_lds_act<1>(s, sl, acc, prev, [&](int kb, float r) { finish(kb, r); }, tail);
                    else
                        gemm_lds(s, sl, acc, 0, [&](int kb, int g) { if (g == 2) tail(kb); });
                    if (nt > 0) hp[nt - 1] = e.p;
                    prev = acc;
                } else {
#pragma unroll
                    for (int kb = 0; kb < 16; kb++) finish(kb, softplus100(prev[kb]));
                    hp[nt - 1] = e.p;
                }
            }
        }
    }
    ZS_STAMP(14);
    s.drain();
    out = half_sum(out);
    ZS_STAMP(15);
    return out + prm[P_B8 - W_IB];
}

template <bool GRID>
__global__ __launch_bounds__(WAVES * 64, 1) void sdf_decode_split_kernel(
    const char *__restrict__ programs, size_t program_stride_bytes, int batch,
    const float *__restrict__ points,
    const float *__restrict__ axis,
    int G, long long first_point,
    int m,
    float *__restrict__ out, int apply_sigmoid, f32x4 *__restrict__ workspace,
    int *__restrict__ tile_flags,
    int static_order) {
    __shared__ __attribute__((aligned(16))) float lds[LDS_FLOATS];
    float *prm = lds;
    const int lane = threadIdx.x & 63;
    const int wave = __builtin_amdgcn_readfirstlane(threadIdx.x >> 6);
    u32x4 *stage = reinterpret_cast<u32x4 *>(lds + PRM_WINDOW);
    const unsigned stage_addr = __builtin_amdgcn_readfirstlane(
        (unsigned)(uintptr_t)(__attribute__((address_space(3))) float *)(lds + PRM_WINDOW));
    u32x4 *fl = reinterpret_cast<u32x4 *>(lds + PRM_WINDOW + STAGE_FLOATS) + wave * SLAB_U4 + lane;
    f32x4 *zslab = workspace + ((size_t)blockIdx.x * WAVES + wave) * ZSLAB_F4 + lane;

    const int tiles_per_img = (m + PTS_PER_BLOCK - 1) / PTS_PER_BLOCK;
    const int total = tiles_per_img * batch;
    int *tile_counter = reinterpret_cast<int *>(workspace + (size_t)MAX_WGS * WAVES * ZSLAB_F4) + 256;
    int *tile_slot = tile_counter + 16 + blockIdx.x;
    const int dyn_tiles = total > (int)gridDim.x ? total - (int)gridDim.x : 0;
    for (int tile = blockIdx.x;;) {
      if (tile < total) {
        const int img = tile / tiles_per_img;
        const int t = tile - img * tiles_per_img;
        const char *prog = programs + (size_t)img * program_stride_bytes;

        const int p = t * PTS_PER_BLOCK + wave * PTS_PER_WAVE + (lane & 31);
        const int pc = p < m ? p : m - 1;
        float px, py, pz;
        if (GRID) {
            const long long gp = first_point + pc;
            const long long gg = (long long)G * G;
            const int ix = (int)(gp / gg);
            const int rem = (int)(gp - (long long)ix * gg);
            const int iy = rem / G;
            const int iz = rem - iy * G;
            px = axis[ix];
            py = axis[iy];
            pz = axis[iz];
        } else {
            const float *q = points + ((size_t)img * m + pc) * 3;
            px = q[0];
            py = q[1];
            pz = q[2];
        }
#ifdef ZS_EXP_TIMING
        unsigned long long *dbg = (blockIdx.x == 0 && threadIdx.x == 0 && tile == 0)
            ? reinterpret_cast<unsigned long long *>(workspace + (size_t)MAX_WGS * WAVES * ZSLAB_F4) : nullptr;
#else
        unsigned long long *dbg = nullptr;
#endif
        float guard = 0.f;
        float logit = decode_tile(prog, prm, stage, stage_addr, fl, zslab, px, py, pz, wave, lane, guard, dbg);
        if (apply_sigmoid) logit = 1.0f / (1.0f + expf(-logit));
        const unsigned bad = reinterpret_cast<const unsigned *>(prog)[REC_FLOATS + P_FLAG];
        const bool pt_bad = (__builtin_bit_cast(unsigned, px) & 0x7f800000u) == 0x7f800000u ||
                            (__builtin_bit_cast(unsigned, py) & 0x7f800000u) == 0x7f800000u ||
                            (__builtin_bit_cast(unsigned, pz) & 0x7f800000u) == 0x7f800000u;
        if (bad || pt_bad) logit = __builtin_bit_cast(float, 0x7fc00000u);
        if (tile_flags) {
            const bool over = !(__builtin_bit_cast(unsigned, guard) <= __builtin_bit_cast(unsigned, S_GUARD * S_GUARD));
            if (__builtin_amdgcn_ballot_w64(over || bad != 0) != 0 && lane == 0) tile_flags[tile] = 1;
        }
        if (lane < 32 && p < m) out[(size_t)img * m + p] = logit;
      }
        if (static_order) {
            tile += (int)gridDim.x;
            if (tile >= total) break;
            continue;
        }
        if (threadIdx.x == 0) {
            const int d = __hip_atomic_fetch_add(tile_counter, 1, __ATOMIC_RELAXED, __HIP_MEMORY_SCOPE_AGENT);
            if (d == dyn_tiles + (int)gridDim.x - 1)
                __hip_atomic_store(tile_counter, 0, __ATOMIC_RELAXED, __HIP_MEMORY_SCOPE_AGENT);
            __hip_atomic_store(tile_slot, d, __ATOMIC_RELAXED, __HIP_MEMORY_SCOPE_AGENT);
        }
        __syncthreads();
        const int d = __builtin_amdgcn_readfirstlane(__hip_atomic_load(tile_slot, __ATOMIC_RELAXED, __HIP_MEMORY_SCOPE_AGENT));
        if ((unsigned)d >= (unsigned)dyn_tiles) break;
        tile = (int)gridDim.x + d;
    }
}

DEV bool out_of_range(const f32x4 &v) {
    const unsigned lim = 0x477fe000u;
    return (__builtin_bit_cast(unsigned, v.x) & 0x7fffffffu) > lim || (__builtin_bit_cast(unsigned, v.y) & 0x7fffffffu) > lim ||
           (__builtin_bit_cast(unsigned, v.z) & 0x7fffffffu) > lim || (__builtin_bit_cast(unsigned, v.w) & 0x7fffffffu) > lim;
}

__host__ __device__ inline int split_source_kblock(int kb) {
    constexpr int KB_BLOCK = G_BLOCK / 2, KB_ATT = HEADS * G_HEAD / 2;
    static_assert(KB_BLOCK - KB_ATT == HT * 32, "an MLP section is 32 K-blocks per hidden tile");
    constexpr int KB_IMPL0 = BLOCKS * KB_BLOCK, KB_L = NT * NT * 2;
    if (kb >= KB_IMPL0 + G_IMPL / 2) return kb;
    if (kb >= KB_IMPL0) {
        const int p = kb - KB_IMPL0;
        if (p < KB_L) return kb;
        if (p < 2 * KB_L) return KB_IMPL0 + 4 * KB_L + (p - KB_L);
        const int q = p - 2 * KB_L, pair = q / (3 * KB_L), r = q - pair * 3 * KB_L;
        if (r >= 2 * KB_L) return KB_IMPL0 + (5 + 2 * pair + 1) * KB_L + (r - 2 * KB_L);
        const int nt = r / (4 * NT), w = r - nt * 4 * NT;
        return w < 2 * NT ? KB_IMPL0 + (5 + 2 * pair) * KB_L + nt * 2 * NT + w
                          : KB_IMPL0 + (1 + pair) * KB_L + nt * 2 * NT + (w - 2 * NT);
    }
    const int blk = kb / KB_BLOCK, p = kb - blk * KB_BLOCK - KB_ATT;
    if (p < 16) return kb;
    const int q = p - 16, it = q >> 5, r = q & 31;
    int src;
    if (it < HT - 1)
        src = r < 16 ? (it + 1) * 32 + r : it * 32 + r;
    else
        src = it * 32 + 16 + r;
    return blk * KB_BLOCK + KB_ATT + src;
}

__global__ __launch_bounds__(256) void split_program_kernel(const float *__restrict__ src,
                                                            size_t src_stride_floats,
                                                            u32x4 *__restrict__ dst,
                                                            size_t dst_stride_u4) {
    const int img = blockIdx.y;
    const float *s = src + (size_t)img * src_stride_floats;
    u32x4 *d = dst + (size_t)img * dst_stride_u4;
    const int e = blockIdx.x * 256 + threadIdx.x;
    constexpr int REC_KB = REC_FLOATS / (KB_U4 * 4);
    if (e < REC_KB * 64) {
        const int kb = e >> 6, lane = e & 63;
        const f32x4 *g = reinterpret_cast<const f32x4 *>(s) + (size_t)split_source_kblock(kb) * 128;
        const f32x4 a = g[lane], b = g[64 + lane];
        if (out_of_range(a) || out_of_range(b)) atomicOr(reinterpret_cast<unsigned *>(d) + REC_FLOATS + P_FLAG, 1u);
        unsigned h[4], l[4];
        split2(a.x, a.y, h[0], l[0]);
        split2(a.z, a.w, h[1], l[1]);
        split2(b.x, b.y, h[2], l[2]);
        split2(b.z, b.w, h[3], l[3]);
        const u32x4 hi = {h[0], h[1], h[2], h[3]}, lo = {l[0], l[1], l[2], l[3]};
        d[(size_t)kb * KB_U4 + lane] = hi;
        d[(size_t)kb * KB_U4 + 64 + lane] = lo;
    } else {
        const int i = e - REC_KB * 64;
        if (i < PARAM_FLOATS / 4 && i != P_FLAG / 4 && (i < P_KMAX / 4 || i >= (P_KMAX + BLOCKS * HEADS) / 4)) {
            const f32x4 v = reinterpret_cast<const f32x4 *>(s + REC_FLOATS)[i];
            if (i < (P_USED + 3) / 4 && out_of_range(v))
                atomicOr(reinterpret_cast<unsigned *>(d) + REC_FLOATS + P_FLAG, 1u);
            d[REC_FLOATS / 4 + i] = __builtin_bit_cast(u32x4, v);
        }
    }
}

__global__ __launch_bounds__(256) void k_bound_kernel(const float *__restrict__ src, size_t src_stride_floats,
                                                      u32x4 *__restrict__ dst, size_t dst_stride_u4) {
    __shared__ float red[256];
    const int img = blockIdx.y, bh = blockIdx.x, blk = bh / HEADS, hd = bh - blk * HEADS;
    const float *kv = src + (size_t)img * src_stride_floats +
                      (size_t)(blk * G_BLOCK + hd * G_HEAD + G_QKV_HEAD) * GROUP_FLOATS;
    float sq = 0.f;
    const int t = threadIdx.x;
    if (t < LT * 32) {
        const int lt = t >> 5;
#pragma unroll
        for (int half = 0; half < 2; half++)
#pragma unroll
            for (int g = 0; g < 4; g++) {
                const f32x4 v = reinterpret_cast<const f32x4 *>(kv + (lt * 8 + g) * GROUP_FLOATS)[(t & 31) + 32 * half];
                sq = fmaf(v.x, v.x, fmaf(v.y, v.y, fmaf(v.z, v.z, fmaf(v.w, v.w, sq))));
            }
    }
    red[t] = sq;
    __syncthreads();
    for (int o = 128; o > 0; o >>= 1) {
        if (t < o) red[t] = fmaxf(red[t], red[t + o]);
        __syncthreads();
    }
    if (t == 0)
        reinterpret_cast<float *>(dst + (size_t)img * dst_stride_u4)[REC_FLOATS + P_KMAX + bh] = sqrtf(red[0]);
}

int decode_grid_size(int batch, int m) {
    const long long tiles = (long long)batch * ((m + PTS_PER_BLOCK - 1) / PTS_PER_BLOCK);
    return (int)(tiles < MAX_WGS ? tiles : MAX_WGS);
}

bool check_programs(const char *what, const void *programs, size_t stride) {
    if (!programs) {
        zs::set_err("%s: null pointer", what);
        return false;
    }
    if (stride % 16 != 0 || stride < zs_sdf_program_bytes()) {
        zs::set_err("%s: bad program stride %zu", what, stride);
        return false;
    }
    return true;
}

}

extern "C" int zs_sdf_split_programs(const void *programs, size_t program_stride_bytes,
                                     void *split_programs, size_t split_stride_bytes, int batch,
                                     void *stream) {
    if (batch < 0 || batch > 65535) {
        zs::set_err("zs_sdf_split_programs: bad batch %d", batch);
        return 0;
    }
    if (batch == 0) return 1;
    if (!check_programs("zs_sdf_split_programs", programs, program_stride_bytes) ||
        !check_programs("zs_sdf_split_programs", split_programs, split_stride_bytes))
        return 0;
    const int elems = (REC_FLOATS / (KB_U4 * 4)) * 64 + PARAM_FLOATS / 4;
    hipStream_t st = static_cast<hipStream_t>(stream);
    if (hipMemset2DAsync(static_cast<char *>(split_programs) + (size_t)(REC_FLOATS + P_FLAG) * 4, split_stride_bytes,
                         0, 16, batch, st) != hipSuccess) {
        zs::set_err("zs_sdf_split_programs: hipMemset2DAsync failed");
        return 0;
    }
    hipLaunchKernelGGL(split_program_kernel, dim3((elems + 255) / 256, batch), dim3(256), 0, st,
                       static_cast<const float *>(programs), program_stride_bytes / sizeof(float),
                       static_cast<u32x4 *>(split_programs), split_stride_bytes / sizeof(u32x4));
    hipLaunchKernelGGL(k_bound_kernel, dim3(BLOCKS * HEADS, batch), dim3(256), 0, st,
                       static_cast<const float *>(programs), program_stride_bytes / sizeof(float),
                       static_cast<u32x4 *>(split_programs), split_stride_bytes / sizeof(u32x4));
    return zs::check_launch("zs_sdf_split_programs") ? 1 : 0;
}

static int launch_counter_reset(void *workspace, hipStream_t st) {
    const char *e = getenv("ZS_SPLIT_STATIC_TILES");
    if (e && atoi(e) != 0) return 1;
    int *tile_counter = reinterpret_cast<int *>(static_cast<f32x4 *>(workspace) + (size_t)MAX_WGS * WAVES * ZSLAB_F4) + 256;
    (void)hipMemsetAsync(tile_counter, 0, sizeof(int), st);
    return 0;
}

extern "C" int zs_sdf_query_points_split(const void *split_programs, size_t program_stride_bytes,
                                         int batch, const float *points, int m, float *logits,
                                         int *tile_flags, void *workspace, void *stream) {
    if (batch < 0 || m < 0) {
        zs::set_err("zs_sdf_query_points_split: negative size (batch=%d m=%d)", batch, m);
        return 0;
    }
    if (batch == 0 || m == 0) return 1;
    if (!points || !logits || !workspace) {
        zs::set_err("zs_sdf_query_points_split: null pointer");
        return 0;
    }
    if (!check_programs("zs_sdf_query_points_split", split_programs, program_stride_bytes)) return 0;
    if ((long long)batch * ((m + PTS_PER_BLOCK - 1) / PTS_PER_BLOCK) > 0x7fffffffLL) {
        zs::set_err("zs_sdf_query_points_split: too many tiles");
        return 0;
    }
    const int static_order = launch_counter_reset(workspace, static_cast<hipStream_t>(stream));
    hipLaunchKernelGGL((sdf_decode_split_kernel<false>), dim3(decode_grid_size(batch, m)),
                       dim3(WAVES * 64), 0, static_cast<hipStream_t>(stream),
                       static_cast<const char *>(split_programs), program_stride_bytes, batch, points,
                       nullptr, 0, 0LL, m, logits, 0, static_cast<f32x4 *>(workspace), tile_flags, static_order);
    return zs::check_launch("zs_sdf_query_points_split") ? 1 : 0;
}

extern "C" int zs_sdf_query_grid_range_split(const void *split_programs, size_t program_stride_bytes,
                                             int batch, const float *axis, int G, long long point_begin,
                                             long long point_end, int apply_sigmoid, float *out,
                                             int *tile_flags, void *workspace, void *stream) {
    const long long P = (long long)G * G * G;
    if (batch < 0 || G <= 0 || point_begin < 0 || point_end > P || point_begin > point_end) {
        zs::set_err("zs_sdf_query_grid_range_split: bad range (batch=%d G=%d points=[%lld,%lld))", batch, G,
                    point_begin, point_end);
        return 0;
    }
    const long long mm = point_end - point_begin;
    if (batch == 0 || mm == 0) return 1;
    if (!axis || !out || !workspace) {
        zs::set_err("zs_sdf_query_grid_range_split: null pointer");
        return 0;
    }
    if (mm > 0x7fffffffLL - PTS_PER_BLOCK) {
        zs::set_err("zs_sdf_query_grid_range_split: %lld points per launch exceed 2^31; split the range", mm);
        return 0;
    }
    if (!check_programs("zs_sdf_query_grid_range_split", split_programs, program_stride_bytes)) return 0;
    const int m = (int)mm;
    const int static_order = launch_counter_reset(workspace, static_cast<hipStream_t>(stream));
    hipLaunchKernelGGL((sdf_decode_split_kernel<true>), dim3(decode_grid_size(batch, m)),
                       dim3(WAVES * 64), 0, static_cast<hipStream_t>(stream),
                       static_cast<const char *>(split_programs), program_stride_bytes, batch, nullptr,
                       axis, G, point_begin, m, out, apply_sigmoid, static_cast<f32x4 *>(workspace), tile_flags, static_order);
    return zs::check_launch("zs_sdf_query_grid_range_split") ? 1 : 0;
}

extern "C" int zs_sdf_query_grid_split(const void *split_programs, size_t program_stride_bytes,
                                       int batch, const float *axis, int G, int slice_begin,
                                       int slice_end, int apply_sigmoid, float *out, int *tile_flags,
                                       void *workspace, void *stream) {
    if (batch < 0 || G <= 0 || slice_begin < 0 || slice_end > G || slice_begin > slice_end) {
        zs::set_err("zs_sdf_query_grid_split: bad range (batch=%d G=%d slices=[%d,%d))", batch, G,
                    slice_begin, slice_end);
        return 0;
    }
    const long long mm = (long long)(slice_end - slice_begin) * G * G;
    if (batch == 0 || mm == 0) return 1;
    if (!axis || !out || !workspace) {
        zs::set_err("zs_sdf_query_grid_split: null pointer");
        return 0;
    }
    if (mm > 0x7fffffffLL - PTS_PER_BLOCK) {
        zs::set_err("zs_sdf_query_grid_split: %lld points per launch exceed 2^31; split the slab", mm);
        return 0;
    }
    if (!check_programs("zs_sdf_query_grid_split", split_programs, program_stride_bytes)) return 0;
    const int m = (int)mm;
    const int static_order = launch_counter_reset(workspace, static_cast<hipStream_t>(stream));
    hipLaunchKernelGGL((sdf_decode_split_kernel<true>), dim3(decode_grid_size(batch, m)),
                       dim3(WAVES * 64), 0, static_cast<hipStream_t>(stream),
                       static_cast<const char *>(split_programs), program_stride_bytes, batch, nullptr,
                       axis, G, (long long)slice_begin * G * G, m, out, apply_sigmoid,
                       static_cast<f32x4 *>(workspace), tile_flags, static_order);
    return zs::check_launch("zs_sdf_query_grid_split") ? 1 : 0;
}
```

zeroshape_amd/csrc/sdf_layout.h:

```cpp
#pragma once

namespace zs {
namespace lay {

constexpr int C = 256, NT = 8, HEADS = 8, HD = 32, L = 197, LT = 7, HID = 1024, HT = 32;
constexpr int BLOCKS = 2;
constexpr int GROUP_FLOATS = 256;
constexpr int RING = 8;

constexpr int G_QKV_HEAD = 3 * NT * 4;
constexpr int G_KV_HEAD = LT * 8;
constexpr int G_PROJ_HEAD = NT * 4;
constexpr int G_HEAD = G_QKV_HEAD + G_KV_HEAD + G_PROJ_HEAD;
constexpr int G_MLP_TILE = 64;
constexpr int G_BLOCK = HEADS * G_HEAD + HT * G_MLP_TILE;
constexpr int G_IMPL = 256 * 5 + 512 * 3;
constexpr int G_TOTAL = BLOCKS * G_BLOCK + G_IMPL;
constexpr int REC_FLOATS = (G_TOTAL + RING) * GROUP_FLOATS;
constexpr int PARAM_FLOATS = 13824;
constexpr int PROGRAM_FLOATS = REC_FLOATS + PARAM_FLOATS;

constexpr int P_PP = 0;
constexpr int P_BLK0 = 1024;
constexpr int P_BLK_STRIDE = 3328;
constexpr int PB_LN1G = 0, PB_LN1B = 256, PB_BPROJ = 512, PB_BQKV = 768, PB_LN2G = 1536,
              PB_LN2B = 1792, PB_B2 = 2048, PB_B1 = 2304;
constexpr int P_LNFG = 7680, P_LNFB = 7936;
constexpr int P_IMPL0 = 8192;
constexpr int P_IMPL1 = 9216;
constexpr int P_IMPL_PAIR = 9472;
constexpr int P_IMPL_PAIR_STRIDE = 1280;
constexpr int P_W8 = 13312, P_B8 = 13568;
constexpr int P_USED = 13584;
constexpr int P_FLAG = 13600;
constexpr int P_KMAX = 13616;
constexpr int P_PHASE_B = 8192;

constexpr int LQ_WLP = 0, LQ_BLP = 65536, LQ_POS = 65792, LQ_LN1G0 = 116224, LQ_LN1B0 = 116480,
              LQ_WQKV0 = 116736, LQ_BQKV0 = 313344, LQ_WPROJ0 = 314112, LQ_BPROJ0 = 379648,
              LQ_LN2G0 = 379904, LQ_LN2B0 = 380160, LQ_W1 = 380416, LQ_B1 = 642560,
              LQ_W2 = 643584, LQ_B2 = 905728, LQ_LN1G1 = 905984, LQ_LN1B1 = 906240,
              LQ_WKV1 = 906496, LQ_BKV1 = 1037568, LQ_TOTAL = 1038080;

constexpr int LPAD = 200;
constexpr int S_LAT = 0;
constexpr int S_X1 = S_LAT + LPAD * C;
constexpr int S_X2 = S_X1 + LPAD * C;
constexpr int S_QKV0 = S_X2 + LPAD * C;
constexpr int S_ATT = S_QKV0 + LPAD * 3 * C;
constexpr int S_HID = S_ATT + LPAD * C;
constexpr int S_KV1 = S_HID + LPAD * HID;
constexpr int SCRATCH_FLOATS = S_KV1 + LPAD * 2 * C;

}
}
```

zeroshape_amd/model/shape/implicit.py:

```python
import contextlib
import os
from functools import partial

import numpy as np
import torch
import torch.nn as nn

from ... import _lib
from ... import program as P
from ...nn import autograd as A
from ...utils.pos_embed import get_2d_sincos_pos_embed


class _Mlp(nn.Module):

    def __init__(self, in_features, hidden_features):
        super().__init__()
        self.fc1 = nn.Linear(in_features, hidden_features)
        self.fc2 = nn.Linear(hidden_features, in_features)


class _Attention(nn.Module):
    def __init__(self, dim):
        super().__init__()
        self.qkv = nn.Linear(dim, dim * 3, bias=True)
        self.proj = nn.Linear(dim, dim)


class _Block(nn.Module):
    def __init__(self, dim, mlp_ratio, norm_layer):
        super().__init__()
        self.norm1 = norm_layer(dim)
        self.attn = _Attention(dim)
        self.norm2 = norm_layer(dim)
        self.mlp = _Mlp(dim, int(dim * mlp_ratio))


class _Proj3D(nn.Module):
    def __init__(self, embed_dim):
        super().__init__()
        self.proj = nn.Linear(3, embed_dim)


class _MLPBlocks(nn.Module):
    def __init__(self, num_hidden_layers, n_channels, latent_dim, skip_in, posenc_res=0):
        super().__init__()
        dims = [3 + 6 * int(posenc_res) + latent_dim] + [n_channels] * num_hidden_layers + [1]
        self.layers = nn.ModuleList([
            nn.Linear(dims[l] + (dims[0] if l in skip_in else 0), dims[l + 1])
            for l in range(len(dims) - 1)])


class DecoderState(object):

    def __init__(self, programs, batch, precision="f32", exact=None):
        self.programs, self.batch, self.precision, self.exact = programs, batch, precision, exact
        self.image_flags = None
        self.image_flags_occ = None
        self.check_event = None
        self.logit_ok = True
        self.occ_ok = True

    @property
    def stride_bytes(self):
        return self.programs.stride(0) * 4


class Implicit(nn.Module):

    def __init__(self, num_patches, latent_dim=768, semantic=False, n_channels=512,
                 n_blocks_attn=2, n_layers_mlp=6, num_heads=16, posenc_3D=0,
                 mlp_ratio=4., norm_layer=partial(nn.LayerNorm, eps=1e-6), drop_path=0.1,
                 skip_in=[], pos_perlayer=True):
        super().__init__()
        self.num_patches = num_patches
        self.pos_perlayer = pos_perlayer
        self.semantic = semantic
        self.num_heads = num_heads
        self.skip_in = tuple(skip_in)
        self.cfg = dict(num_patches=num_patches, latent_dim=latent_dim, n_channels=n_channels,
                        n_blocks_attn=n_blocks_attn, n_layers_mlp=n_layers_mlp, num_heads=num_heads,
                        posenc_3D=posenc_3D, mlp_ratio=float(mlp_ratio), skip_in=tuple(skip_in),
                        pos_perlayer=bool(pos_perlayer), semantic=bool(semantic))
        self.point_proj = _Proj3D(n_channels)
        self.latent_proj = nn.Linear(latent_dim, n_channels, bias=True)
        self.pos_embed = nn.Parameter(torch.zeros(1, num_patches + 1, n_channels), requires_grad=False)
        self.blocks_attn = nn.ModuleList([_Block(n_channels, mlp_ratio, norm_layer)
                                          for _ in range(n_blocks_attn)])
        self.norm = norm_layer(n_channels)
        self.posenc_3D = int(posenc_3D)
        self.impl_mlp = _MLPBlocks(n_layers_mlp, n_channels, n_channels, self.skip_in, self.posenc_3D) \
            if n_layers_mlp > 0 else None
        if self.impl_mlp is None:
            self.pred_head = nn.Linear(n_channels, 1, bias=True)
        self.drop_path = float(drop_path)
        self.drop_scales = None
        self.initialize_weights()
        self._packed = None
        self.precision = os.environ.get("ZS_DECODER_PRECISION", "f16x3")
        self._workspace = {}
        self._check_streams = {}
        self._probe_cache = {}
        self._check_keepalive = []
        self.last_tile_flags = None
        self.envelope_guard = True
        self.calibrate = os.environ.get("ZS_DECODER_CALIBRATE", "1") != "0"
        self.image_check = os.environ.get("ZS_DECODER_IMAGE_CHECK", "1") != "0"
        self.calibration_range = (-1.5, 1.5)
        self._last_calibration = None
        self._last_check_event = None
        self._calibration = None

    def initialize_weights(self):
        pe = get_2d_sincos_pos_embed(self.pos_embed.shape[-1], int(self.num_patches ** .5), cls_token=True)
        self.pos_embed.data.copy_(torch.from_numpy(pe).float().unsqueeze(0))
        self.apply(self._init_weights)

    def _init_weights(self, m):
        if isinstance(m, nn.Linear):
            torch.nn.init.xavier_uniform_(m.weight)
            if m.bias is not None:
                nn.init.constant_(m.bias, 0)
        elif isinstance(m, nn.LayerNorm):
            nn.init.constant_(m.bias, 0)
            nn.init.constant_(m.weight, 1.0)

    @property
    def fused(self):
        c = self.cfg
        want = dict(num_patches=P.L - 1, n_channels=P.C, latent_dim=P.C, n_blocks_attn=P.BLOCKS,
                    n_layers_mlp=P.MLP_LAYERS - 1, num_heads=P.HEADS, posenc_3D=0, mlp_ratio=4.0,
                    skip_in=P.SKIP_IN, semantic=False)
        return all(c[k] == v for k, v in want.items())

    def _check_supported(self, fused=True):
        c = self.cfg
        if fused:
            if not self.fused:
                raise NotImplementedError(
                    "the fused HIP decoder kernels are specialised for options/shape.yaml:19-44; this configuration (%s) runs "
                    "layer by layer - call the module (forward) instead of prepare / query_*" % c)
            return
        if c["n_channels"] % c["num_heads"] or c["n_channels"] // c["num_heads"] != 32:
            raise NotImplementedError("the HIP attention kernels need a head dimension of 32 (n_channels %d / num_heads %d)"
                                      % (c["n_channels"], c["num_heads"]))
        if c["num_patches"] + 1 > 256 or c["n_blocks_attn"] < 1:
            raise NotImplementedError("the HIP point-attention kernels take at most 256 latent rows (num_patches + 1 = %d) and "
                                      "at least one attention block" % (c["num_patches"] + 1))

    def _weights_key(self):
        return (A.GENERATION[0], bool(self.pos_perlayer)) + tuple((p.data_ptr(), p._version) for p in self.parameters())

    def packed(self, device):
        key = (str(device),) + self._weights_key()
        if self._packed is None or self._packed[0] != key:
            self._check_supported()
            sd = {k: v.detach().float().cpu().numpy() for k, v in self.state_dict().items()}
            prog = torch.from_numpy(P.pack_program(sd)).to(device)
            lat = torch.from_numpy(P.pack_latent_params(sd)).to(device)
            self._packed = (key, prog, lat, P.split_envelope(sd)[0])
        return self._packed[1], self._packed[2]

    @property
    def last_calibration(self):
        ev = self._last_check_event
        if ev is not None:
            torch.cuda.current_stream().wait_event(ev)
        return self._last_calibration

    @last_calibration.setter
    def last_calibration(self, value):
        self._last_calibration = value

    def split_allowed(self, device):
        self.packed(device)
        return self._packed[3]

    def workspace(self, device, extra_bytes=0):
        key = (str(device), torch.cuda.current_stream(device).cuda_stream)
        need = (_lib.load().zs_sdf_workspace_bytes() + extra_bytes + 3) // 4
        if key not in self._workspace or self._workspace[key].numel() < need:
            self._workspace[key] = torch.zeros(need, dtype=torch.float32, device=device)
        return self._workspace[key]

    CALIBRATION_POINTS = 4096
    CALIBRATION_TOL = 2.5e-5
    CALIBRATION_TOL_OCC = 2.5e-5
    FLIP_BAND = 1e-5

    def _probe_points(self, device):
        cached = self._probe_cache.get(str(device))
        if cached is not None:
            return cached
        i = torch.arange(self.CALIBRATION_POINTS, dtype=torch.float64)
        lo, hi = self.calibration_range
        frac = torch.stack([(i * a + b) % 1.0 for a, b in ((0.7548776662466927, 0.5), (0.5698402909980532, 0.25),
                                                            (0.4301597090019468, 0.75))], -1)
        pts = self._probe_cache[str(device)] = (lo + (hi - lo) * frac).to(torch.float32)[None].to(device)
        return pts

    def _verdict_stats(self, got, want):
        lib = _lib.load()
        got, want = got.contiguous(), want.contiguous()
        B, M = got.shape
        stats = torch.empty(B, 5, dtype=torch.float32, device=got.device)
        flags = torch.empty(B, 2, dtype=torch.int32, device=got.device)
        with _lib.on(got.device):
            _lib.check(lib.zs_sdf_verdict_stats(_lib.ptr(got), _lib.ptr(want), B, M, float(self.FLIP_BAND), float(self.CALIBRATION_TOL),
                                                float(self.CALIBRATION_TOL_OCC), _lib.ptr(stats), _lib.ptr(flags),
                                                _lib.current_stream_ptr(got.device)), "zs_sdf_verdict_stats")
        return stats, flags

    @torch.no_grad()
    def _calibrate(self, split, exact):
        key = self._weights_key()
        if self._calibration is not None and self._calibration[0] == key:
            self.last_calibration = self._calibration[1]
            return self.last_calibration["selected"] == "f16x3", self.last_calibration["selected_occ"] == "f16x3"
        if torch.cuda.is_current_stream_capturing():
            raise RuntimeError("Implicit.prepare: the f16x3 calibration of new weights needs one host read; run one "
                               "eager prepare() before capturing, or request precision='f32'")
        pts = self._probe_points(split.device)
        guard, flags = self.envelope_guard, self.last_tile_flags
        self.envelope_guard = False
        try:
            raw = DecoderState(split[:1], 1, "f16x3", exact=exact[:1])
            got = self.query_points(raw, pts)
        finally:
            self.envelope_guard, self.last_tile_flags = guard, flags
        want = self.query_points(DecoderState(exact[:1], 1), pts)
        stats = self._verdict_stats(got, want)[0][0].cpu()
        if not bool(torch.isfinite(stats[2])):
            self.last_calibration = None
            return False, False
        finite = bool(torch.isfinite(stats).all())
        ok = finite and float(stats[0]) <= self.CALIBRATION_TOL
        ok_occ = finite and float(stats[3]) <= self.CALIBRATION_TOL_OCC and float(stats[4]) == 0.0
        self.last_calibration = dict(max_abs_diff=float(stats[0]), mean_abs_diff=float(stats[1]),
                                     max_abs_logit=float(stats[2]), max_abs_occ_diff=float(stats[3]),
                                     flips_outside_band=int(stats[4]) if finite else -1,
                                     points=self.CALIBRATION_POINTS, tol=self.CALIBRATION_TOL, tol_occ=self.CALIBRATION_TOL_OCC,
                                     flip_band=self.FLIP_BAND,
                                     selected="f16x3" if ok else "f32", selected_occ="f16x3" if ok_occ else "f32")
        self._calibration = (key, self.last_calibration)
        return ok, ok_occ

    @torch.no_grad()
    def prepare(self, latent_depth, precision=None, calibrate=None, shard=None):
        precision = self.precision if precision is None else precision
        calibrate = self.calibrate if calibrate is None else calibrate
        self._check_supported()
        if precision not in ("f32", "f16x3"):
            raise ValueError("decoder precision must be 'f32' or 'f16x3', got %r" % (precision,))
        if not latent_depth.is_cuda:
            raise ValueError("latent_depth must be a GPU tensor; zeroshape_amd has no CPU path")
        lib = _lib.load()
        lat = latent_depth.detach().to(torch.float32).contiguous()
        B = lat.shape[0]
        if tuple(lat.shape[1:]) != (P.L, P.C):
            raise ValueError("latent_depth must be [B,%d,%d], got %s" % (P.L, P.C, tuple(lat.shape)))
        template, lat_params = self.packed(lat.device)
        assert lib.zs_sdf_program_bytes() == P.PROGRAM_BYTES, "layout mismatch between program.py and the library"
        programs = template.unsqueeze(0).repeat(B, 1)
        scratch = torch.empty(B * (lib.zs_sdf_prologue_scratch_bytes() // 4), dtype=torch.float32,
                              device=lat.device)
        with _lib.on(lat.device):
            rc = lib.zs_sdf_prologue_ex(_lib.ptr(programs), programs.stride(0) * 4, _lib.ptr(lat_params),
                                        _lib.ptr(lat), B, _lib.ptr(scratch), 1 if self.pos_perlayer else 0,
                                        _lib.current_stream_ptr(lat.device))
        _lib.check(rc, "zs_sdf_prologue_ex")
        if precision == "f16x3" and self.split_allowed(lat.device):
            split = torch.empty_like(programs)
            with _lib.on(lat.device):
                rc = lib.zs_sdf_split_programs(_lib.ptr(programs), programs.stride(0) * 4, _lib.ptr(split),
                                               split.stride(0) * 4, B, _lib.current_stream_ptr(lat.device))
            _lib.check(rc, "zs_sdf_split_programs")
            if not calibrate:
                return DecoderState(split, B, "f16x3", exact=programs)
            ok, ok_occ = self._calibrate(split, programs)
            if ok or ok_occ:
                state = DecoderState(split, B, "f16x3", exact=programs)
                state.logit_ok, state.occ_ok = ok, ok_occ
                if self.image_check:
                    self._launch_image_check(state, split, programs, shard)
                return state
        return DecoderState(programs, B)

    def _sharded_image_check(self, split, exact, shard, streams=None):
        rank, world, exchange = shard
        B = split.shape[0]
        k = (B + world - 1) // world
        a = streams[0] if streams is not None else None
        ctx = (lambda st: torch.cuda.stream(st)) if streams is not None else (lambda st: contextlib.nullcontext())
        mine = len(range(rank, B, world))
        if mine:
            f, f_occ, mx, mx_occ = self._image_check(split[rank::world], exact[rank::world], streams=streams)
        with ctx(a):
            own = torch.zeros(k, 2, dtype=torch.int32, device=split.device)
            maxima = torch.full((B,), -1.0, dtype=torch.float32, device=split.device)
            maxima_occ = maxima.clone()
            if mine:
                own[:mine, 0], own[:mine, 1] = f, f_occ
                maxima[rank::world], maxima_occ[rank::world] = mx, mx_occ
            flags = exchange(own, B)
            return flags[:, 0].contiguous(), flags[:, 1].contiguous(), maxima, maxima_occ

    def _launch_image_check(self, state, split, exact, shard=None):
        dev = split.device
        main = torch.cuda.current_stream(dev)
        if torch.cuda.is_current_stream_capturing() or os.environ.get("ZS_DECODER_CHECK_INLINE", "0") != "0":
            state.image_flags, state.image_flags_occ, maxima, maxima_occ = \
                self._image_check(split, exact) if shard is None else self._sharded_image_check(split, exact, shard)
            self._last_check_event = None
        else:
            pair = self._check_streams.get(str(dev))
            if pair is None:
                pair = self._check_streams[str(dev)] = (torch.cuda.Stream(device=dev, priority=-1),
                                                        torch.cuda.Stream(device=dev, priority=-1))
            side, side2 = pair
            side.wait_stream(main)
            side2.wait_stream(main)
            for st_ in (side, side2):
                head = torch.cuda.Event()
                head.record(st_)
                main.wait_event(head)
            state.image_flags, state.image_flags_occ, maxima, maxima_occ = \
                self._image_check(split, exact, streams=(side, side2)) if shard is None else \
                self._sharded_image_check(split, exact, shard, streams=(side, side2))
            state.check_event = torch.cuda.Event()
            state.check_event.record(side)
            if os.environ.get("ZS_DECODER_CHECK_RECORD_STREAM", "0") != "0":
                for t in (split, exact):
                    t.record_stream(side)
                    t.record_stream(side2)
            else:
                while self._check_keepalive and self._check_keepalive[0][0].query():
                    self._check_keepalive.pop(0)
                self._check_keepalive.append((state.check_event, split, exact))
            for t in (state.image_flags, state.image_flags_occ, maxima, maxima_occ):
                t.record_stream(main)
            self._last_check_event = state.check_event
        self._last_calibration = dict(self._last_calibration, per_image_max_abs_diff=maxima, per_image_max_abs_occ_diff=maxima_occ)

    @torch.no_grad()
    def _image_check(self, split, exact, streams=None):
        B = split.shape[0]
        a, b = streams if streams is not None else (None, None)
        ctx = (lambda st: torch.cuda.stream(st)) if streams is not None else (lambda st: contextlib.nullcontext())
        with ctx(a):
            pts = self._probe_points(split.device).expand(B, -1, -1).contiguous()
        if b is not None:
            b.wait_stream(a)
        with ctx(a):
            want = self.query_points(DecoderState(exact, B), pts)
        guard, flags = self.envelope_guard, self.last_tile_flags
        self.envelope_guard = False
        try:
            with ctx(b):
                got = self.query_points(DecoderState(split, B, "f16x3", exact=exact), pts)
        finally:
            self.envelope_guard, self.last_tile_flags = guard, flags
        if b is not None:
            a.wait_stream(b)
            got.record_stream(a)
            pts.record_stream(b)
        with ctx(a):
            st, flags = self._verdict_stats(got, want)
            return flags[:, 0], flags[:, 1], st[:, 0], st[:, 3]

    def _tile_flags(self, batch, m, device, state=None):
        if not self.envelope_guard and getattr(state, "image_flags", None) is None:
            return None
        return torch.zeros(batch * ((m + 127) // 128), dtype=torch.int32, device=device)

    @staticmethod
    def _for_space(state, occupancy):
        if state.precision == "f16x3" and not (state.occ_ok if occupancy else state.logit_ok):
            return DecoderState(state.exact, state.batch)
        return state

    @staticmethod
    def _join_image_check(state, flags, occupancy=False):
        image_flags = getattr(state, "image_flags_occ" if occupancy else "image_flags", None)
        if image_flags is None or flags is None:
            return
        if state.check_event is not None:
            torch.cuda.current_stream(flags.device).wait_event(state.check_event)
        flags.view(state.batch, -1).bitwise_or_(image_flags[:, None])

    @torch.no_grad()
    def query_points(self, state, points_3D, need_attn=False):
        lib = _lib.load()
        state = self._for_space(state, False)
        pts = points_3D.detach().to(torch.float32).contiguous()
        if pts.dim() != 3 or pts.shape[2] != 3 or pts.shape[0] != state.batch:
            raise ValueError("points_3D must be [%d,M,3], got %s" % (state.batch, tuple(pts.shape)))
        if pts.device != state.programs.device:
            raise ValueError("points_3D and latent_depth live on different devices")
        M = pts.shape[1]
        out = torch.empty(state.batch, M, dtype=torch.float32, device=pts.device)
        attn, extra = None, 0
        if state.precision == "f16x3":
            if need_attn:
                raise ValueError("the attention map needs an fp32 DecoderState (prepare(..., precision='f32'))")
            flags = self._tile_flags(state.batch, M, pts.device, state)
            ws, st = _lib.ptr(self.workspace(pts.device)), _lib.current_stream_ptr(pts.device)
            with _lib.on(pts.device):
                rc = lib.zs_sdf_query_points_split(_lib.ptr(state.programs), state.stride_bytes, state.batch,
                                                   _lib.ptr(pts), M, _lib.ptr(out), _lib.ptr(flags), ws, st)
                _lib.check(rc, "zs_sdf_query_points_split")
                self._join_image_check(state, flags)
                if flags is not None:
                    rc = lib.zs_sdf_query_points(_lib.ptr(state.exact), state.exact.stride(0) * 4, state.batch,
                                                 _lib.ptr(pts), M, _lib.ptr(out), None, _lib.ptr(flags), ws, st)
            _lib.check(rc, "zs_sdf_query_points")
            self.last_tile_flags = flags
            return out
        if need_attn:
            attn = torch.empty(state.batch, M, P.L, dtype=torch.float32, device=pts.device)
            extra = lib.zs_sdf_attn_scratch_bytes(state.batch, M)
        with _lib.on(pts.device):
            rc = lib.zs_sdf_query_points(_lib.ptr(state.programs), state.stride_bytes, state.batch,
                                         _lib.ptr(pts), M, _lib.ptr(out), _lib.ptr(attn), None,
                                         _lib.ptr(self.workspace(pts.device, extra)),
                                         _lib.current_stream_ptr(pts.device))
        _lib.check(rc, "zs_sdf_query_points")
        return (out, attn) if need_attn else out

    @torch.no_grad()
    def query_grid(self, latent_depth, axis, apply_sigmoid=True, slice_begin=0, slice_end=None,
                   state=None):
        lib = _lib.load()
        if state is None:
            state = self.prepare(latent_depth)
        state = self._for_space(state, bool(apply_sigmoid))
        axis = axis.detach().to(torch.float32).contiguous()
        if axis.device != state.programs.device:
            raise ValueError("axis and latent_depth live on different devices")
        G = axis.numel()
        slice_end = G if slice_end is None else slice_end
        out = torch.empty(state.batch, slice_end - slice_begin, G, G, dtype=torch.float32,
                          device=axis.device)
        if state.precision == "f16x3":
            flags = self._tile_flags(state.batch, (slice_end - slice_begin) * G * G, axis.device, state)
            ws, st = _lib.ptr(self.workspace(axis.device)), _lib.current_stream_ptr(axis.device)
            with _lib.on(axis.device):
                rc = lib.zs_sdf_query_grid_split(_lib.ptr(state.programs), state.stride_bytes, state.batch,
                                                 _lib.ptr(axis), G, slice_begin, slice_end,
                                                 1 if apply_sigmoid else 0, _lib.ptr(out), _lib.ptr(flags), ws, st)
                _lib.check(rc, "zs_sdf_query_grid_split")
                self._join_image_check(state, flags, occupancy=bool(apply_sigmoid))
                if flags is not None:
                    rc = lib.zs_sdf_query_grid(_lib.ptr(state.exact), state.exact.stride(0) * 4, state.batch,
                                               _lib.ptr(axis), G, slice_begin, slice_end,
                                               1 if apply_sigmoid else 0, _lib.ptr(out), _lib.ptr(flags), ws, st)
            _lib.check(rc, "zs_sdf_query_grid")
            self.last_tile_flags = flags
            return out
        with _lib.on(axis.device):
            rc = lib.zs_sdf_query_grid(_lib.ptr(state.programs), state.stride_bytes, state.batch,
                                       _lib.ptr(axis), G, slice_begin, slice_end,
                                       1 if apply_sigmoid else 0, _lib.ptr(out), None,
                                       _lib.ptr(self.workspace(axis.device)),
                                       _lib.current_stream_ptr(axis.device))
        _lib.check(rc, "zs_sdf_query_grid")
        return out

    @torch.no_grad()
    def query_grid_range(self, latent_depth, axis, point_begin, point_end, apply_sigmoid=True, state=None):
        lib = _lib.load()
        if state is None:
            state = self.prepare(latent_depth)
        state = self._for_space(state, bool(apply_sigmoid))
        axis = axis.detach().to(torch.float32).contiguous()
        if axis.device != state.programs.device:
            raise ValueError("axis and latent_depth live on different devices")
        G = axis.numel()
        out = torch.empty(state.batch, point_end - point_begin, dtype=torch.float32, device=axis.device)
        ws, st = _lib.ptr(self.workspace(axis.device)), _lib.current_stream_ptr(axis.device)
        sig = 1 if apply_sigmoid else 0
        with _lib.on(axis.device):
            if state.precision == "f16x3":
                flags = self._tile_flags(state.batch, point_end - point_begin, axis.device, state)
                rc = lib.zs_sdf_query_grid_range_split(_lib.ptr(state.programs), state.stride_bytes, state.batch,
                                                       _lib.ptr(axis), G, point_begin, point_end, sig, _lib.ptr(out),
                                                       _lib.ptr(flags), ws, st)
                _lib.check(rc, "zs_sdf_query_grid_range_split")
                self._join_image_check(state, flags, occupancy=bool(apply_sigmoid))
                if flags is not None:
                    rc = lib.zs_sdf_query_grid_range(_lib.ptr(state.exact), state.exact.stride(0) * 4, state.batch,
                                                     _lib.ptr(axis), G, point_begin, point_end, sig, _lib.ptr(out),
                                                     _lib.ptr(flags), ws, st)
                self.last_tile_flags = flags
            else:
                rc = lib.zs_sdf_query_grid_range(_lib.ptr(state.programs), state.stride_bytes, state.batch,
                                                 _lib.ptr(axis), G, point_begin, point_end, sig, _lib.ptr(out),
                                                 None, ws, st)
        _lib.check(rc, "zs_sdf_query_grid_range")
        return out

    def forward(self, latent_depth, latent_semantic, points_3D, need_attn=True):
        if self.semantic:
            if latent_semantic is None:
                raise ValueError("this Implicit was built with semantic=True: latent_semantic is required")
            latent_depth = torch.cat([latent_depth.to(torch.float32), latent_semantic.to(torch.float32)], dim=-1)
        elif latent_semantic is not None:
            raise ValueError("latent_semantic given to an Implicit built with semantic=False")
        if not self.fused:
            return self._forward_autograd(latent_depth, points_3D, want_attn=need_attn)
        if torch.is_grad_enabled() and (self.training or points_3D.requires_grad or latent_depth.requires_grad):
            logits = self._forward_autograd(latent_depth, points_3D)[0]
            if not need_attn:
                return logits, None
            with torch.no_grad():
                return logits, self.query_points(self.prepare(latent_depth, "f32"), points_3D, need_attn=True)[1]
        state = self.prepare(latent_depth)
        if need_attn and state.precision == "f32":
            return self.query_points(state, points_3D, need_attn=True)
        logits = self.query_points(state, points_3D)
        if not need_attn:
            return logits, None
        return logits, self.query_points(DecoderState(state.exact, state.batch), points_3D, need_attn=True)[1]

    def _drop_scale(self, B, device):
        if not self.training or self.drop_path <= 0.0:
            return None
        keep = 1.0 - self.drop_path
        return torch.empty(B, dtype=torch.float32, device=device).bernoulli_(keep).div_(keep)

    def _forward_autograd(self, latent_depth, points_3D, want_attn=False):
        self._check_supported(fused=False)
        if not (latent_depth.is_cuda and points_3D.is_cuda):
            raise ValueError("latent_depth / points_3D must be GPU tensors; zeroshape_amd has no CPU path")
        lat = latent_depth.to(torch.float32)
        pts = points_3D.detach().to(torch.float32).contiguous()
        B, M = pts.shape[0], pts.shape[1]
        H = self.num_heads
        Ll = self.num_patches + 1
        if tuple(lat.shape[1:]) != (Ll, self.latent_proj.in_features):
            raise ValueError("latent codes must be [B,%d,%d], got %s" % (Ll, self.latent_proj.in_features, tuple(lat.shape)))
        attn = torch.empty(B, M, Ll, dtype=torch.float32, device=pts.device) if want_attn else None
        pts4 = A._pad_channels(pts, 4)
        xp = A.linear(pts4, self.point_proj.proj.weight, self.point_proj.proj.bias, cin=3)
        pos = self.pos_embed.detach().expand(B, -1, -1).contiguous()
        cl = lat.shape[-1]
        if cl % 4:
            lat = A.pad_channels(lat.contiguous(), (cl + 3) // 4 * 4)
        xl = A.linear(lat, self.latent_proj.weight, self.latent_proj.bias, res1=pos, cin=cl)
        nb = len(self.blocks_attn)
        scales = list(self.drop_scales) if self.drop_scales is not None else \
            [self._drop_scale(B, pts.device) for _ in range(2 * nb)]

        def residual(x, branch_in, w, b, scale):
            if scale is None:
                return A.linear(branch_in, w, b, res1=x)
            return A.add_scaled_rows(x, A.linear(branch_in, w, b), scale)

        ones = torch.ones(B, dtype=torch.float32, device=pts.device) if self.pos_perlayer and nb > 1 else None
        for i, blk in enumerate(self.blocks_attn):
            last = i == nb - 1
            s_attn, s_mlp = scales[2 * i], scales[2 * i + 1]
            if self.pos_perlayer and i > 0:
                xl = A.add_scaled_rows(xl, pos, ones)
            if last:
                hl, xl_res = A.layer_norm(xl, blk.norm1.weight, blk.norm1.bias), None
            else:
                hl, xl_res = A.layer_norm(xl, blk.norm1.weight, blk.norm1.bias, fork=True)
            qkv_l = A.linear(hl, blk.attn.qkv.weight, blk.attn.qkv.bias)
            hp, xp = A.layer_norm(xp, blk.norm1.weight, blk.norm1.bias, fork=True)
            qkv_p = A.linear(hp, blk.attn.qkv.weight, blk.attn.qkv.bias)
            if want_attn:
                A.point_attention_probs(qkv_p, qkv_l, H, attn, weight=1.0 / nb, accumulate=i > 0)
            op = A.point_attention(qkv_p, qkv_l, H)
            xp = residual(xp, op, blk.attn.proj.weight, blk.attn.proj.bias, s_attn)
            hp, xp = A.layer_norm(xp, blk.norm2.weight, blk.norm2.bias, fork=True)
            hp = A.gelu(A.linear(hp, blk.mlp.fc1.weight, blk.mlp.fc1.bias))
            xp = residual(xp, hp, blk.mlp.fc2.weight, blk.mlp.fc2.bias, s_mlp)
            if not last:
                ol = A.attention(qkv_l, H)
                xl = residual(xl_res, ol, blk.attn.proj.weight, blk.attn.proj.bias, s_attn)
                hl, xl = A.layer_norm(xl, blk.norm2.weight, blk.norm2.bias, fork=True)
                hl = A.gelu(A.linear(hl, blk.mlp.fc1.weight, blk.mlp.fc1.bias))
                xl = residual(xl, hl, blk.mlp.fc2.weight, blk.mlp.fc2.bias, s_mlp)
        feat = A.layer_norm(xp, self.norm.weight, self.norm.bias)
        if self.impl_mlp is None:
            return A.linear(feat, self.pred_head.weight, self.pred_head.bias).squeeze(-1), attn
        C = feat.shape[-1]
        layers = self.impl_mlp.layers
        r2 = 0.7071067811865476
        x = None
        E = 3 + 6 * self.posenc_3D
        enc = pts4 if self.posenc_3D == 0 else A.posenc3d(pts, self.posenc_3D)
        for l, lin in enumerate(layers):
            if l == 0:
                y = A.linear(enc, lin.weight, None, cin0=0, cin=E)
                y = A.linear(feat, lin.weight, lin.bias, res1=y, cin0=E, cin=C)
            elif l in self.skip_in:
                y = A.linear(enc, lin.weight, None, in_scale=r2, cin0=C, cin=E)
                y = A.linear(feat, lin.weight, None, in_scale=r2, res1=y, cin0=C + E, cin=C)
                y = A.linear(x, lin.weight, lin.bias, in_scale=r2, res1=y, cin0=0, cin=C)
            else:
                y = A.linear(x, lin.weight, lin.bias)
            x = A.softplus(y, 100.0) if l < len(layers) - 1 else y
        return x.squeeze(-1), attn
```

zeroshape_amd/program.py:

```python
import numpy as np

C = 256
NT = C // 32
HEADS = 8
HD = 32
L = 197
LT = 7
HID = 1024
HT = HID // 32
BLOCKS = 2
MLP_LAYERS = 9
SKIP_IN = (2, 4, 6)
GROUP_FLOATS = 256
RING = 8

LANE = np.arange(64)
LANE_I = LANE & 31
LANE_HI = LANE >> 5


def row(r, hi):
    return (r & 3) + 8 * (r >> 2) + 4 * hi


ROW_TABLE = np.array([[row(r, hi) for r in range(16)] for hi in range(2)])


def _records_linear(W, nt, kt):
    rows = 32 * nt + LANE_I
    cols = 32 * kt + ROW_TABLE[LANE_HI][:, :].T
    return W[rows[None, :], cols]


def _interleave(recs):
    n = recs.shape[0]
    assert n % 4 == 0
    return recs.reshape(n // 4, 4, 64).transpose(0, 2, 1).reshape(-1)


def records_for_linear(W, n_out_tiles=None, k_tiles=None):
    W = np.asarray(W, np.float32)
    n_out_tiles = W.shape[0] // 32 if n_out_tiles is None else n_out_tiles
    k_tiles = W.shape[1] // 32 if k_tiles is None else k_tiles
    out = [_records_linear(W, nt, kt) for nt in range(n_out_tiles) for kt in range(k_tiles)]
    return np.concatenate(out, axis=0)


def kv_records(K_h, V_h):
    Kp = np.zeros((LT * 32, HD), np.float32)
    Vp = np.zeros((LT * 32, HD), np.float32)
    Kp[:L], Vp[:L] = K_h, V_h
    out = []
    for lt in range(LT):
        krec = Kp[(32 * lt + LANE_I)[None, :], ROW_TABLE[LANE_HI].T]
        vrec = Vp[32 * lt + ROW_TABLE[LANE_HI].T, LANE_I[None, :]]
        out += [krec, vrec]
    return np.concatenate(out, axis=0)


G_QKV_HEAD = 3 * NT * 4
G_KV_HEAD = LT * 8
G_PROJ_HEAD = NT * 4
G_HEAD = G_QKV_HEAD + G_KV_HEAD + G_PROJ_HEAD
G_MLP_TILE = NT * 4 + NT * 4
G_BLOCK = HEADS * G_HEAD + HT * G_MLP_TILE
G_IMPL_PLAIN = NT * NT * 4
G_IMPL_SKIP = 2 * G_IMPL_PLAIN
G_IMPL = G_IMPL_PLAIN * 5 + G_IMPL_SKIP * 3
G_TOTAL = BLOCKS * G_BLOCK + G_IMPL
REC_FLOATS = (G_TOTAL + RING) * GROUP_FLOATS
PARAM_FLOATS = 13824
PROGRAM_FLOATS = REC_FLOATS + PARAM_FLOATS
PROGRAM_BYTES = PROGRAM_FLOATS * 4


def kv_group_offset(blk, head):
    return blk * G_BLOCK + head * G_HEAD + G_QKV_HEAD


def pack_records(sd, kv=None):
    out = []
    for blk in range(BLOCKS):
        p = "blocks_attn.%d." % blk
        Wqkv = np.asarray(sd[p + "attn.qkv.weight"], np.float32)
        Wproj = np.asarray(sd[p + "attn.proj.weight"], np.float32)
        W1 = np.asarray(sd[p + "mlp.fc1.weight"], np.float32)
        W2 = np.asarray(sd[p + "mlp.fc2.weight"], np.float32)
        for h in range(HEADS):
            for part in range(3):
                Wt = Wqkv[part * C + h * HD: part * C + (h + 1) * HD]
                out.append(records_for_linear(Wt))
            if kv is not None:
                out.append(kv_records(*kv[(blk, h)]))
            else:
                out.append(np.zeros((G_KV_HEAD * 4, 64), np.float32))
            out.append(records_for_linear(Wproj[:, h * HD:(h + 1) * HD]))
        for ht in range(HT):
            out.append(records_for_linear(W1[ht * 32:(ht + 1) * 32]))
            out.append(records_for_linear(W2[:, ht * 32:(ht + 1) * 32]))
    Wl = [np.asarray(sd["impl_mlp.layers.%d.weight" % l], np.float32) for l in range(MLP_LAYERS)]
    out.append(records_for_linear(Wl[0][:, 3:]))
    for l in SKIP_IN:
        out.append(records_for_linear(Wl[l][:, C + 3:]))
    for l in range(1, MLP_LAYERS - 1):
        if l in SKIP_IN:
            out.append(records_for_linear(Wl[l][:, :C]))
        else:
            out.append(records_for_linear(Wl[l]))
    recs = np.concatenate(out, axis=0)
    assert recs.shape == (G_TOTAL * 4, 64), recs.shape
    flat = _interleave(recs)
    out = np.concatenate([flat, np.zeros(RING * GROUP_FLOATS, np.float32)])
    assert out.size == REC_FLOATS
    return out


def rowparam(v):
    v = np.asarray(v, np.float32)
    T = v.shape[0] // 32
    idx = (32 * np.arange(T))[:, None, None] + ROW_TABLE[None, :, :]
    return v[idx].reshape(-1)


def rowparam4(cols):
    stacked = np.stack([rowparam(c).reshape(-1) for c in cols], axis=-1)
    return stacked.reshape(-1)


class ParamLayout(object):

    def __init__(self):
        o = 0

        def take(n):
            nonlocal o
            s = o
            o += n
            return s
        self.PP = take(C * 4)
        self.blk = []
        for _ in range(BLOCKS):
            d = {}
            d["ln1_g"] = take(C)
            d["ln1_b"] = take(C)
            d["bproj"] = take(C)
            d["bqkv"] = take(HEADS * 3 * 32)
            d["ln2_g"] = take(C)
            d["ln2_b"] = take(C)
            d["b2"] = take(C)
            d["b1"] = take(HID)
            self.blk.append(d)
        self.lnf_g = take(C)
        self.lnf_b = take(C)
        self.impl = []
        for l in range(MLP_LAYERS - 1):
            if l == 0 or l in SKIP_IN:
                self.impl.append(take(C * 4))
            else:
                self.impl.append(take(C))
        self.w8 = take(C)
        self.b8 = take(16)
        self.total = o


PARAMS = ParamLayout()
assert PARAMS.total <= PARAM_FLOATS
P_FLAG = 13600
P_KMAX = 13616
assert PARAMS.total <= P_FLAG and P_FLAG + 4 <= P_KMAX and P_KMAX + BLOCKS * HEADS <= PARAM_FLOATS
BLOCK_PARAM_FLOATS = 3 * C + HEADS * 96 + 3 * C + HID


def pack_params(sd):
    g = lambda k: np.asarray(sd[k], np.float32)
    out = np.zeros(PARAM_FLOATS, np.float32)

    def put(off, arr):
        out[off:off + arr.size] = arr
    Wp = g("point_proj.proj.weight")
    put(PARAMS.PP, rowparam4([Wp[:, 0], Wp[:, 1], Wp[:, 2], g("point_proj.proj.bias")]))
    for blk in range(BLOCKS):
        p, d = "blocks_attn.%d." % blk, PARAMS.blk[blk]
        put(d["ln1_g"], rowparam(g(p + "norm1.weight")))
        put(d["ln1_b"], rowparam(g(p + "norm1.bias")))
        put(d["bproj"], rowparam(g(p + "attn.proj.bias")))
        bq = g(p + "attn.qkv.bias")
        parts = []
        for h in range(HEADS):
            for part in range(3):
                parts.append(rowparam(bq[part * C + h * HD: part * C + (h + 1) * HD]))
        put(d["bqkv"], np.concatenate(parts))
        put(d["ln2_g"], rowparam(g(p + "norm2.weight")))
        put(d["ln2_b"], rowparam(g(p + "norm2.bias")))
        put(d["b2"], rowparam(g(p + "mlp.fc2.bias")))
        put(d["b1"], rowparam(g(p + "mlp.fc1.bias")))
    put(PARAMS.lnf_g, rowparam(g("norm.weight")))
    put(PARAMS.lnf_b, rowparam(g("norm.bias")))
    for l in range(MLP_LAYERS - 1):
        W, b = g("impl_mlp.layers.%d.weight" % l), g("impl_mlp.layers.%d.bias" % l)
        if l == 0:
            put(PARAMS.impl[l], rowparam4([W[:, 0], W[:, 1], W[:, 2], b]))
        elif l in SKIP_IN:
            put(PARAMS.impl[l], rowparam4([W[:, C], W[:, C + 1], W[:, C + 2], b]))
        else:
            put(PARAMS.impl[l], rowparam(b))
    put(PARAMS.w8, rowparam(g("impl_mlp.layers.8.weight")[0]))
    out[PARAMS.b8] = g("impl_mlp.layers.8.bias")[0]
    return out


def pack_program(sd, kv=None):
    out = np.concatenate([pack_records(sd, kv), pack_params(sd)])
    assert out.size == PROGRAM_FLOATS
    return out


class LatentLayout(object):
    def __init__(self, latent_dim=C):
        o = 0

        def take(n):
            nonlocal o
            s = o
            o += n
            return s
        self.latent_dim = latent_dim
        self.Wlp = take(latent_dim * C)
        self.blp = take(C)
        self.pos = take(L * C)
        self.ln1g0 = take(C)
        self.ln1b0 = take(C)
        self.Wqkv0 = take(C * 3 * C)
        self.bqkv0 = take(3 * C)
        self.Wproj0 = take(C * C)
        self.bproj0 = take(C)
        self.ln2g0 = take(C)
        self.ln2b0 = take(C)
        self.W1 = take(C * HID)
        self.b1 = take(HID)
        self.W2 = take(HID * C)
        self.b2 = take(C)
        self.ln1g1 = take(C)
        self.ln1b1 = take(C)
        self.Wkv1 = take(C * 2 * C)
        self.bkv1 = take(2 * C)
        self.total = o


LATENT = LatentLayout()


def pack_latent_params(sd):
    g = lambda k: np.asarray(sd[k], np.float32)
    assert g("latent_proj.weight").shape == (C, LATENT.latent_dim)
    out = np.zeros(LATENT.total, np.float32)

    def put(off, arr):
        arr = np.ascontiguousarray(arr, np.float32).reshape(-1)
        out[off:off + arr.size] = arr
    put(LATENT.Wlp, g("latent_proj.weight").T)
    put(LATENT.blp, g("latent_proj.bias"))
    put(LATENT.pos, g("pos_embed").reshape(L, C))
    b0, b1 = "blocks_attn.0.", "blocks_attn.1."
    put(LATENT.ln1g0, g(b0 + "norm1.weight"))
    put(LATENT.ln1b0, g(b0 + "norm1.bias"))
    put(LATENT.Wqkv0, g(b0 + "attn.qkv.weight").T)
    put(LATENT.bqkv0, g(b0 + "attn.qkv.bias"))
    put(LATENT.Wproj0, g(b0 + "attn.proj.weight").T)
    put(LATENT.bproj0, g(b0 + "attn.proj.bias"))
    put(LATENT.ln2g0, g(b0 + "norm2.weight"))
    put(LATENT.ln2b0, g(b0 + "norm2.bias"))
    put(LATENT.W1, g(b0 + "mlp.fc1.weight").T)
    put(LATENT.b1, g(b0 + "mlp.fc1.bias"))
    put(LATENT.W2, g(b0 + "mlp.fc2.weight").T)
    put(LATENT.b2, g(b0 + "mlp.fc2.bias"))
    put(LATENT.ln1g1, g(b1 + "norm1.weight"))
    put(LATENT.ln1b1, g(b1 + "norm1.bias"))
    put(LATENT.Wkv1, g(b1 + "attn.qkv.weight")[C:].T)
    put(LATENT.bkv1, g(b1 + "attn.qkv.bias")[C:])
    return out


LPAD = 200
SCRATCH_FLOATS = LPAD * (3 * C + 3 * C + C + HID + 2 * C)


KB_TOTAL = G_TOTAL // 2
KB_WORDS = 512


def split_source_kblocks(n=None):
    n = REC_FLOATS // GROUP_FLOATS // 2 if n is None else n
    src = np.arange(n)
    kb_block, kb_att = G_BLOCK // 2, HEADS * G_HEAD // 2
    order = list(range(16))
    for t in range(HT - 1):
        order += [(t + 1) * 32 + r for r in range(16)] + [t * 32 + 16 + r for r in range(16)]
    order += [(HT - 1) * 32 + 16 + r for r in range(16)]
    assert sorted(order) == list(range(HT * 32))
    for blk in range(BLOCKS):
        base = blk * kb_block + kb_att
        src[base:base + HT * 32] = base + np.array(order)
    b0, kl = BLOCKS * kb_block, NT * NT * 2
    impl = list(range(kl)) + [4 * kl + i for i in range(kl)]
    for pair in range(3):
        for nt in range(NT):
            impl += [(5 + 2 * pair) * kl + nt * 2 * NT + w for w in range(2 * NT)]
            impl += [(1 + pair) * kl + nt * 2 * NT + w for w in range(2 * NT)]
        impl += [(6 + 2 * pair) * kl + i for i in range(kl)]
    assert sorted(impl) == list(range(G_IMPL // 2))
    src[b0:b0 + G_IMPL // 2] = b0 + np.array(impl)
    return src


def f16_round(x):
    x = np.ascontiguousarray(x, np.float32)
    with np.errstate(over="ignore"):
        h = x.astype(np.float16)
    return h.view(np.uint16), h.astype(np.float32)


def f16_rtz(x):
    x = np.ascontiguousarray(x, np.float32)
    with np.errstate(over="ignore"):
        h = x.astype(np.float16)
    away = np.abs(h.astype(np.float32)) > np.abs(x)
    h = np.where(away, np.nextafter(h, np.float16(0)), h).astype(np.float16)
    return h.view(np.uint16), h.astype(np.float32)


def split_program(prog):
    prog = np.ascontiguousarray(prog, np.float32)
    rec = prog[:REC_FLOATS].reshape(-1, 2, 64, 4)
    rec = rec[split_source_kblocks(rec.shape[0])]
    vals = rec.transpose(0, 2, 1, 3).reshape(-1, 64, 8)
    hi16, hif = f16_round(vals)
    with np.errstate(invalid="ignore"):
        lo16, _ = f16_round(vals - hif)
    out = np.stack([hi16, lo16], axis=1)
    words = np.ascontiguousarray(out).reshape(-1).view(np.uint32)
    params = prog[REC_FLOATS:].copy()
    params[P_KMAX:P_KMAX + BLOCKS * HEADS] = latent_k_bounds(prog).reshape(-1)
    bad = not (np.all(np.isfinite(prog)) and float(np.abs(prog).max()) <= F16_MAX)
    params[P_FLAG:P_FLAG + 1].view(np.uint32)[0] = 1 if bad else 0
    return np.concatenate([words, params.view(np.uint32)])


S_GUARD = 64.0
W_MAX = 16.0
F16_MAX = 65504.0


def split_envelope(sd):
    vals = [np.asarray(v, np.float32) for k, v in sd.items() if k != "pos_embed"]
    wmax = max(float(np.max(np.abs(v))) if np.all(np.isfinite(v)) else float("inf") for v in vals)
    return wmax <= W_MAX, dict(max_abs_weight=wmax)


def latent_k_bounds(prog):
    prog = np.ascontiguousarray(prog, np.float32)
    out = np.zeros((BLOCKS, HEADS), np.float32)
    for blk in range(BLOCKS):
        for h in range(HEADS):
            o = kv_group_offset(blk, h) * GROUP_FLOATS
            g = prog[o:o + G_KV_HEAD * GROUP_FLOATS].reshape(LT, 8, 64, 4)[:, :4]
            rec = g.transpose(0, 1, 3, 2).reshape(LT, 16, 64)
            sq = (rec.astype(np.float64) ** 2).sum(1)
            row = sq[:, :32] + sq[:, 32:]
            out[blk, h] = np.sqrt(row.max())
    return out
```

Before: 76.11 million points/s.

## Fold first-block LayerNorm and QKV projection into low-rank per-point attention

```diff
diff --git a/include/zeroshape_hip.h b/include/zeroshape_hip.h
--- a/include/zeroshape_hip.h
+++ b/include/zeroshape_hip.h
@@ -8,7 +8,7 @@
 extern "C" {
 #endif
 
-#define ZS_ABI_VERSION 38
+#define ZS_ABI_VERSION 39
 
 int zs_abi_version(void);
 
@@ -70,6 +70,22 @@
                                   const float *axis, int G, long long point_begin,
                                   long long point_end, int apply_sigmoid, float *out,
                                   int *tile_flags, void *workspace, void *stream);
+
+size_t zs_sdf_fold_program_bytes(void);
+int zs_sdf_fold_programs(const void *programs, size_t program_stride_bytes, const void *split_programs,
+                         size_t split_stride_bytes, const float *fold_params, void *folded_programs,
+                         size_t folded_stride_bytes, int batch, void *stream);
+int zs_sdf_query_points_fold(const void *folded_programs, size_t program_stride_bytes, int batch,
+                             const float *points, int m, float *logits, int *tile_flags,
+                             void *workspace, void *stream);
+int zs_sdf_query_grid_fold(const void *folded_programs, size_t program_stride_bytes, int batch,
+                           const float *axis, int G, int slice_begin, int slice_end,
+                           int apply_sigmoid, float *out, int *tile_flags, void *workspace,
+                           void *stream);
+int zs_sdf_query_grid_range_fold(const void *folded_programs, size_t program_stride_bytes, int batch,
+                                 const float *axis, int G, long long point_begin,
+                                 long long point_end, int apply_sigmoid, float *out,
+                                 int *tile_flags, void *workspace, void *stream);
 
 size_t zs_bf_grid_bytes(void);
 size_t zs_bf_scratch_bytes(void);
diff --git a/zeroshape_amd/_lib.py b/zeroshape_amd/_lib.py
--- a/zeroshape_amd/_lib.py
+++ b/zeroshape_amd/_lib.py
@@ -53,6 +53,16 @@
     "zs_sdf_query_grid_range_split": (_c_int, [_c_void_p, _c_size_t, _c_int, _c_void_p, _c_int,
                                                ctypes.c_longlong, ctypes.c_longlong, _c_int, _c_void_p,
                                                _c_void_p, _c_void_p, _c_void_p]),
+    "zs_sdf_fold_program_bytes": (_c_size_t, []),
+    "zs_sdf_fold_programs": (_c_int, [_c_void_p, _c_size_t, _c_void_p, _c_size_t, _c_void_p, _c_void_p, _c_size_t, _c_int,
+                                      _c_void_p]),
+    "zs_sdf_query_points_fold": (_c_int, [_c_void_p, _c_size_t, _c_int, _c_void_p, _c_int,
+                                          _c_void_p, _c_void_p, _c_void_p, _c_void_p]),
+    "zs_sdf_query_grid_fold": (_c_int, [_c_void_p, _c_size_t, _c_int, _c_void_p, _c_int, _c_int,
+                                        _c_int, _c_int, _c_void_p, _c_void_p, _c_void_p, _c_void_p]),
+    "zs_sdf_query_grid_range_fold": (_c_int, [_c_void_p, _c_size_t, _c_int, _c_void_p, _c_int,
+                                              ctypes.c_longlong, ctypes.c_longlong, _c_int, _c_void_p,
+                                              _c_void_p, _c_void_p, _c_void_p]),
     "zs_erode_mask": (_c_int, [_c_void_p, _c_int, _c_int, _c_int, _c_int, _c_void_p, _c_void_p]),
     "zs_bf_grid_bytes": (_c_size_t, []),
     "zs_bf_scratch_bytes": (_c_size_t, []),
@@ -198,7 +208,7 @@
     "zs_readout_concat_bwd": (_c_int, [_c_void_p, _c_void_p, _c_int, _c_int, _c_int, _c_void_p]),
 }
 
-ABI_VERSION = 38
+ABI_VERSION = 39
 _lib = None
 
 
diff --git a/zeroshape_amd/csrc/sdf_decoder_split.hip b/zeroshape_amd/csrc/sdf_decoder_split.hip
--- a/zeroshape_amd/csrc/sdf_decoder_split.hip
+++ b/zeroshape_amd/csrc/sdf_decoder_split.hip
@@ -546,11 +546,18 @@
     __syncthreads();
 }
 
-template <bool MASK>
+template <bool MASK, bool FOLDED = false>
 DEV void attn_tile(AStream &s, const PT &q, f32x16 &o, float &m_run, float &z_run, float c, int hi,
                    int pos0) {
     f32x16 S = zero16();
-    gemm_one(s, q, S, pos0);
+    if (FOLDED) {
+        u32x4 ahi, alo;
+        s.step(pos0 & (CK - 1), ahi, alo);
+        pin(ahi, alo);
+        mfma3(S, ahi, alo, q.v[0], q.v[1]);
+    } else {
+        gemm_one(s, q, S, pos0);
+    }
     float mt = -INFINITY;
 #pragma unroll
     for (int r = 0; r < 16; r++) {
@@ -579,7 +586,7 @@
         zs_ += p;
     }
     z_run += zs_;
-    gemm_one(s, pack_tile(S), o, pos0 + 2);
+    gemm_one(s, pack_tile(S), o, pos0 + (FOLDED ? 1 : 2));
 }
 
 #ifdef ZS_EXP_TIMING
@@ -589,9 +596,9 @@
 #endif
 DEV float decode_tile(const char *prog, float *prm, u32x4 *stage, unsigned stage_addr, u32x4 *slab,
                       f32x4 *zs, float px, float py, float pz, int wave, int lane, float &guard,
-                      unsigned long long *dbg) {
+                      unsigned long long *dbg, int fold) {
     const int hi = lane >> 5;
-    const float *prog_params = reinterpret_cast<const float *>(prog) + REC_FLOATS;
+    const float *prog_params = reinterpret_cast<const float *>(prog) + (fold ? FREC_FLOATS : REC_FLOATS);
     AStream s;
     s.init(prog, stage, stage_addr, wave, lane);
     Slab sl;
@@ -609,6 +616,101 @@
 
 #pragma unroll 1
     for (int blk = 0; blk < BLOCKS; blk++) {
+      if (fold && blk == 0) {
+        load_params(prm, prog_params, FP_FOLD, FB_WINDOW);
+        float u[5];
+        {
+            const float *R = prm + FB_R;
+            const float r0 = fmaf(R[2], pz, fmaf(R[1], py, fmaf(R[0], px, R[3])));
+            const float r1 = fmaf(R[6], pz, fmaf(R[5], py, R[7]));
+            const float r2 = fmaf(R[10], pz, R[11]);
+            const float r3 = R[15];
+            const float ss = fmaf(r3, r3, fmaf(r2, r2, fmaf(r1, r1, r0 * r0)));
+            const float rs = 1.0f / sqrtf(ss + 1e-6f);
+            u[0] = px * rs;
+            u[1] = py * rs;
+            u[2] = pz * rs;
+            u[3] = rs;
+            u[4] = 1.0f;
+        }
+        if (!(fmaxf(fmaxf(fabsf(u[0]), fabsf(u[1])), fabsf(u[2])) <= 65504.0f)) guard = INFINITY;
+        PT up;
+        {
+            unsigned h0, l0, h1, l1;
+            split2(u[0], u[1], h0, l0);
+            split2(u[2], u[3], h1, l1);
+            const bool lo_half = hi == 0;
+            up.v[0] = u32x4{lo_half ? h0 : 0u, lo_half ? h1 : 0u, lo_half ? 0x3c00u : 0u, 0u};
+            up.v[1] = u32x4{lo_half ? l0 : 0u, lo_half ? l1 : 0u, 0u, 0u};
+            up.v[2] = up.v[3] = u32x4{0u, 0u, 0u, 0u};
+        }
+#pragma unroll
+        for (int nt = 0; nt < NT; nt++) y[nt] += rp16(prm, PB_BPROJ, nt, hi);
+
+        auto fhead = [&](int hd, auto Ptag) {
+            constexpr int P = decltype(Ptag)::value;
+            const float c = scale * 1.44269504088896340736f;
+            float m_run = -INFINITY, z_run = 0.f;
+            f32x16 o = zero16();
+            attn_tile<false, true>(s, up, o, m_run, z_run, c, hi, P);
+            attn_tile<false, true>(s, up, o, m_run, z_run, c, hi, P + 3);
+            attn_tile<false, true>(s, up, o, m_run, z_run, c, hi, P + 6);
+            attn_tile<false, true>(s, up, o, m_run, z_run, c, hi, P + 9);
+            attn_tile<false, true>(s, up, o, m_run, z_run, c, hi, P + 12);
+            attn_tile<false, true>(s, up, o, m_run, z_run, c, hi, P + 15);
+            attn_tile<true, true>(s, up, o, m_run, z_run, c, hi, P + 18);
+            float s_self, qq;
+            {
+                const float *M = prm + FB_M + hd * 32, *T = prm + FB_T + hd * 32;
+                s_self = 0.f;
+                qq = 0.f;
+#pragma unroll
+                for (int i = 0; i < 5; i++) {
+                    float mi = 0.f, ti = 0.f;
+#pragma unroll
+                    for (int j = 0; j < 5; j++) mi = fmaf(M[i * 5 + j], u[j], mi);
+#pragma unroll
+                    for (int j = i; j < 5; j++) ti = fmaf(T[i * 5 + j], u[j], ti);
+                    s_self = fmaf(u[i], mi, s_self);
+                    qq = fmaf(ti, ti, qq);
+                }
+                s_self *= c;
+            }
+            {
+                const float km = prog_params[P_KMAX + hd] * scale;
+                guard = fmaxf(guard, qq * (km * km));
+            }
+            f32x16 v = rp16(prm, FB_VC4, hd, hi);
+#pragma unroll
+            for (int cc = 0; cc < 4; cc++) {
+                const f32x16 w = rp16(prm, cc == 0 ? FB_VC0 : cc == 1 ? FB_VC1 : cc == 2 ? FB_VC2 : FB_VC3, hd, hi);
+#pragma unroll
+                for (int r = 0; r < 16; r++) v[r] = fmaf(w[r], u[cc], v[r]);
+            }
+            {
+                const float m_new = fmaxf(m_run, s_self);
+                const float alpha = __builtin_amdgcn_exp2f(m_run - m_new);
+                const float p_self = __builtin_amdgcn_exp2f(s_self - m_new);
+                const float z = fmaf(half_sum(z_run), alpha, p_self);
+                const float inv = 1.0f / z;
+                const float a_i = alpha * inv, p_i = p_self * inv;
+#pragma unroll
+                for (int r = 0; r < 16; r++) o[r] = fmaf(p_i, v[r], o[r] * a_i);
+            }
+            const PT op = pack_tile(o);
+#pragma unroll
+            for (int nt = 0; nt < NT; nt++) gemm_one(s, op, y[nt], (P + LT * 3 + 2 * nt) & (CK - 1));
+        };
+        static_assert(FKB_HEAD == 37 && (HEADS * FKB_HEAD) % CK == 0, "folded head = 37 K-blocks, section = 37 chunks");
+        fhead(0, std::integral_constant<int, 0>());
+        fhead(1, std::integral_constant<int, 5>());
+        fhead(2, std::integral_constant<int, 2>());
+        fhead(3, std::integral_constant<int, 7>());
+        fhead(4, std::integral_constant<int, 4>());
+        fhead(5, std::integral_constant<int, 1>());
+        fhead(6, std::integral_constant<int, 6>());
+        fhead(7, std::integral_constant<int, 3>());
+      } else {
         load_params(prm, prog_params, W_BLK + blk * P_BLK_STRIDE, P_BLK_STRIDE);
         layer_norm_lds(y, sl, prm, PB_LN1G, PB_LN1B, hi);
         ZS_STAMP(2 + blk * 4);
@@ -667,6 +769,7 @@
             head(hd, std::integral_constant<int, 0>());
             head(hd + 1, std::integral_constant<int, 4>());
         }
+      }
 
         ZS_STAMP(3 + blk * 4);
         layer_norm_lds(y, sl, prm, PB_LN2G, PB_LN2B, hi);
@@ -867,7 +970,8 @@
     int m,
     float *__restrict__ out, int apply_sigmoid, f32x4 *__restrict__ workspace,
     int *__restrict__ tile_flags,
-    int static_order) {
+    int static_order,
+    int fold) {
     __shared__ __attribute__((aligned(16))) float lds[LDS_FLOATS];
     float *prm = lds;
     const int lane = threadIdx.x & 63;
@@ -915,9 +1019,9 @@
         unsigned long long *dbg = nullptr;
 #endif
         float guard = 0.f;
-        float logit = decode_tile(prog, prm, stage, stage_addr, fl, zslab, px, py, pz, wave, lane, guard, dbg);
+        float logit = decode_tile(prog, prm, stage, stage_addr, fl, zslab, px, py, pz, wave, lane, guard, dbg, fold);
         if (apply_sigmoid) logit = 1.0f / (1.0f + expf(-logit));
-        const unsigned bad = reinterpret_cast<const unsigned *>(prog)[REC_FLOATS + P_FLAG];
+        const unsigned bad = reinterpret_cast<const unsigned *>(prog)[(fold ? FREC_FLOATS : REC_FLOATS) + P_FLAG];
         const bool pt_bad = (__builtin_bit_cast(unsigned, px) & 0x7f800000u) == 0x7f800000u ||
                             (__builtin_bit_cast(unsigned, py) & 0x7f800000u) == 0x7f800000u ||
                             (__builtin_bit_cast(unsigned, pz) & 0x7f800000u) == 0x7f800000u;
@@ -1039,17 +1143,89 @@
         reinterpret_cast<float *>(dst + (size_t)img * dst_stride_u4)[REC_FLOATS + P_KMAX + bh] = sqrtf(red[0]);
 }
 
+__global__ __launch_bounds__(256) void fold_program_kernel(const float *__restrict__ src, size_t src_stride_floats,
+                                                           const u32x4 *__restrict__ split, size_t split_stride_u4,
+                                                           const float *__restrict__ fold_params,
+                                                           u32x4 *__restrict__ dst, size_t dst_stride_u4) {
+    const int img = blockIdx.y;
+    const float *s = src + (size_t)img * src_stride_floats;
+    const u32x4 *sp = split + (size_t)img * split_stride_u4;
+    u32x4 *d = dst + (size_t)img * dst_stride_u4;
+    unsigned *flag = reinterpret_cast<unsigned *>(d) + FREC_FLOATS + P_FLAG;
+    const int e = blockIdx.x * 256 + threadIdx.x;
+    constexpr int FREC_KB = FREC_FLOATS / (KB_U4 * 4);
+    constexpr int KB_ATT0 = HEADS * FKB_HEAD;
+    constexpr int KB_HEAD = G_HEAD / 2, KB_QKV = G_QKV_HEAD / 2;
+    if (e < FREC_KB * 64) {
+        const int kb = e >> 6, lane = e & 63;
+        int src_kb = -1;
+        int hd = 0, lt = 0;
+        if (kb >= KB_ATT0) {
+            src_kb = kb + HEADS * KB_HEAD - KB_ATT0;
+        } else {
+            hd = kb / FKB_HEAD;
+            const int w = kb - hd * FKB_HEAD;
+            lt = w / 3;
+            if (w >= LT * 3) src_kb = hd * KB_HEAD + KB_QKV + LT * 4 + (w - LT * 3);
+            else if (w - lt * 3 > 0) src_kb = hd * KB_HEAD + KB_QKV + lt * 4 + 1 + (w - lt * 3);
+        }
+        if (src_kb >= 0) {
+            d[(size_t)kb * KB_U4 + lane] = sp[(size_t)src_kb * KB_U4 + lane];
+            d[(size_t)kb * KB_U4 + 64 + lane] = sp[(size_t)src_kb * KB_U4 + 64 + lane];
+            return;
+        }
+        float a[5] = {0.f, 0.f, 0.f, 0.f, 0.f};
+        const int rw = 32 * lt + (lane & 31);
+        if (lane < 32 && rw < L) {
+            const float *kv = s + (size_t)(hd * G_HEAD + G_QKV_HEAD + lt * 8) * GROUP_FLOATS;
+            const float *qt = fold_params + FB_QT + hd * 5 * HD;
+            double acc[5] = {0.0, 0.0, 0.0, 0.0, 0.0};
+            for (int h2 = 0; h2 < 2; h2++)
+                for (int r = 0; r < 16; r++) {
+                    const double k = kv[(r >> 2) * GROUP_FLOATS + (lane + 32 * h2) * 4 + (r & 3)];
+                    const int dd = (r & 3) + 8 * (r >> 2) + 4 * h2;
+#pragma unroll
+                    for (int c = 0; c < 5; c++) acc[c] = fma(k, (double)qt[c * HD + dd], acc[c]);
+                }
+#pragma unroll
+            for (int c = 0; c < 5; c++) a[c] = (float)acc[c];
+        }
+        if (out_of_range(f32x4{a[0], a[1], a[2], a[3]}) || out_of_range(f32x4{a[4], 0.f, 0.f, 0.f})) atomicOr(flag, 1u);
+        unsigned h[3], l[3];
+        split2(a[0], a[1], h[0], l[0]);
+        split2(a[2], a[3], h[1], l[1]);
+        split2(a[4], 0.f, h[2], l[2]);
+        d[(size_t)kb * KB_U4 + lane] = u32x4{h[0], h[1], h[2], 0u};
+        d[(size_t)kb * KB_U4 + 64 + lane] = u32x4{l[0], l[1], l[2], 0u};
+    } else {
+        const int i = e - FREC_KB * 64;
+        if (i < PARAM_FLOATS / 4) {
+            if (i == P_FLAG / 4) {
+                const unsigned f = reinterpret_cast<const unsigned *>(sp + REC_FLOATS / 4)[P_FLAG];
+                if (f) atomicOr(flag, f);
+            } else {
+                d[FREC_FLOATS / 4 + i] = sp[REC_FLOATS / 4 + i];
+            }
+        } else if (i < FPARAM_FLOATS / 4) {
+            const int j = i - PARAM_FLOATS / 4;
+            const f32x4 v = reinterpret_cast<const f32x4 *>(fold_params)[j];
+            if (4 * j < FB_WINDOW && out_of_range(v)) atomicOr(flag, 1u);
+            d[FREC_FLOATS / 4 + i] = __builtin_bit_cast(u32x4, v);
+        }
+    }
+}
+
 int decode_grid_size(int batch, int m) {
     const long long tiles = (long long)batch * ((m + PTS_PER_BLOCK - 1) / PTS_PER_BLOCK);
     return (int)(tiles < MAX_WGS ? tiles : MAX_WGS);
 }
 
-bool check_programs(const char *what, const void *programs, size_t stride) {
+bool check_programs(const char *what, const void *programs, size_t stride, int fold = 0) {
     if (!programs) {
         zs::set_err("%s: null pointer", what);
         return false;
     }
-    if (stride % 16 != 0 || stride < zs_sdf_program_bytes()) {
+    if (stride % 16 != 0 || stride < (fold ? (size_t)FPROGRAM_FLOATS * 4 : zs_sdf_program_bytes())) {
         zs::set_err("%s: bad program stride %zu", what, stride);
         return false;
     }
@@ -1085,6 +1261,36 @@
     return zs::check_launch("zs_sdf_split_programs") ? 1 : 0;
 }
 
+extern "C" size_t zs_sdf_fold_program_bytes(void) { return (size_t)FPROGRAM_FLOATS * 4; }
+
+extern "C" int zs_sdf_fold_programs(const void *programs, size_t program_stride_bytes, const void *split_programs,
+                                    size_t split_stride_bytes, const float *fold_params, void *folded_programs,
+                                    size_t folded_stride_bytes, int batch, void *stream) {
+    if (batch < 0 || batch > 65535) {
+        zs::set_err("zs_sdf_fold_programs: bad batch %d", batch);
+        return 0;
+    }
+    if (batch == 0) return 1;
+    if (!fold_params || !check_programs("zs_sdf_fold_programs", programs, program_stride_bytes) ||
+        !check_programs("zs_sdf_fold_programs", split_programs, split_stride_bytes) ||
+        !check_programs("zs_sdf_fold_programs", folded_programs, folded_stride_bytes, 1)) {
+        if (!fold_params) zs::set_err("zs_sdf_fold_programs: null pointer");
+        return 0;
+    }
+    hipStream_t st = static_cast<hipStream_t>(stream);
+    if (hipMemset2DAsync(static_cast<char *>(folded_programs) + (size_t)(FREC_FLOATS + P_FLAG) * 4, folded_stride_bytes,
+                         0, 16, batch, st) != hipSuccess) {
+        zs::set_err("zs_sdf_fold_programs: hipMemset2DAsync failed");
+        return 0;
+    }
+    const int elems = (FREC_FLOATS / (KB_U4 * 4)) * 64 + FPARAM_FLOATS / 4;
+    hipLaunchKernelGGL(fold_program_kernel, dim3((elems + 255) / 256, batch), dim3(256), 0, st,
+                       static_cast<const float *>(programs), program_stride_bytes / sizeof(float),
+                       static_cast<const u32x4 *>(split_programs), split_stride_bytes / sizeof(u32x4), fold_params,
+                       static_cast<u32x4 *>(folded_programs), folded_stride_bytes / sizeof(u32x4));
+    return zs::check_launch("zs_sdf_fold_programs") ? 1 : 0;
+}
+
 static int launch_counter_reset(void *workspace, hipStream_t st) {
     const char *e = getenv("ZS_SPLIT_STATIC_TILES");
     if (e && atoi(e) != 0) return 1;
@@ -1093,87 +1299,124 @@
     return 0;
 }
 
-extern "C" int zs_sdf_query_points_split(const void *split_programs, size_t program_stride_bytes,
-                                         int batch, const float *points, int m, float *logits,
-                                         int *tile_flags, void *workspace, void *stream) {
+static int query_points_impl(const char *what, const void *split_programs, size_t program_stride_bytes,
+                             int batch, const float *points, int m, float *logits,
+                             int *tile_flags, void *workspace, void *stream, int fold) {
     if (batch < 0 || m < 0) {
-        zs::set_err("zs_sdf_query_points_split: negative size (batch=%d m=%d)", batch, m);
+        zs::set_err("%s: negative size (batch=%d m=%d)", what, batch, m);
         return 0;
     }
     if (batch == 0 || m == 0) return 1;
     if (!points || !logits || !workspace) {
-        zs::set_err("zs_sdf_query_points_split: null pointer");
+        zs::set_err("%s: null pointer", what);
         return 0;
     }
-    if (!check_programs("zs_sdf_query_points_split", split_programs, program_stride_bytes)) return 0;
+    if (!check_programs(what, split_programs, program_stride_bytes, fold)) return 0;
     if ((long long)batch * ((m + PTS_PER_BLOCK - 1) / PTS_PER_BLOCK) > 0x7fffffffLL) {
-        zs::set_err("zs_sdf_query_points_split: too many tiles");
+        zs::set_err("%s: too many tiles", what);
         return 0;
     }
     const int static_order = launch_counter_reset(workspace, static_cast<hipStream_t>(stream));
     hipLaunchKernelGGL((sdf_decode_split_kernel<false>), dim3(decode_grid_size(batch, m)),
                        dim3(WAVES * 64), 0, static_cast<hipStream_t>(stream),
                        static_cast<const char *>(split_programs), program_stride_bytes, batch, points,
-                       nullptr, 0, 0LL, m, logits, 0, static_cast<f32x4 *>(workspace), tile_flags, static_order);
-    return zs::check_launch("zs_sdf_query_points_split") ? 1 : 0;
-}
-
-extern "C" int zs_sdf_query_grid_range_split(const void *split_programs, size_t program_stride_bytes,
-                                             int batch, const float *axis, int G, long long point_begin,
-                                             long long point_end, int apply_sigmoid, float *out,
-                                             int *tile_flags, void *workspace, void *stream) {
+                       nullptr, 0, 0LL, m, logits, 0, static_cast<f32x4 *>(workspace), tile_flags, static_order, fold);
+    return zs::check_launch(what) ? 1 : 0;
+}
+
+static int query_grid_range_impl(const char *what, const void *split_programs, size_t program_stride_bytes,
+                                 int batch, const float *axis, int G, long long point_begin,
+                                 long long point_end, int apply_sigmoid, float *out,
+                                 int *tile_flags, void *workspace, void *stream, int fold) {
     const long long P = (long long)G * G * G;
     if (batch < 0 || G <= 0 || point_begin < 0 || point_end > P || point_begin > point_end) {
-        zs::set_err("zs_sdf_query_grid_range_split: bad range (batch=%d G=%d points=[%lld,%lld))", batch, G,
+        zs::set_err("%s: bad range (batch=%d G=%d points=[%lld,%lld))", what, batch, G,
                     point_begin, point_end);
         return 0;
     }
     const long long mm = point_end - point_begin;
     if (batch == 0 || mm == 0) return 1;
     if (!axis || !out || !workspace) {
-        zs::set_err("zs_sdf_query_grid_range_split: null pointer");
+        zs::set_err("%s: null pointer", what);
         return 0;
     }
     if (mm > 0x7fffffffLL - PTS_PER_BLOCK) {
-        zs::set_err("zs_sdf_query_grid_range_split: %lld points per launch exceed 2^31; split the range", mm);
+        zs::set_err("%s: %lld points per launch exceed 2^31; split the range", what, mm);
         return 0;
     }
-    if (!check_programs("zs_sdf_query_grid_range_split", split_programs, program_stride_bytes)) return 0;
+    if (!check_programs(what, split_programs, program_stride_bytes, fold)) return 0;
     const int m = (int)mm;
     const int static_order = launch_counter_reset(workspace, static_cast<hipStream_t>(stream));
     hipLaunchKernelGGL((sdf_decode_split_kernel<true>), dim3(decode_grid_size(batch, m)),
                        dim3(WAVES * 64), 0, static_cast<hipStream_t>(stream),
                        static_cast<const char *>(split_programs), program_stride_bytes, batch, nullptr,
-                       axis, G, point_begin, m, out, apply_sigmoid, static_cast<f32x4 *>(workspace), tile_flags, static_order);
-    return zs::check_launch("zs_sdf_query_grid_range_split") ? 1 : 0;
-}
-
-extern "C" int zs_sdf_query_grid_split(const void *split_programs, size_t program_stride_bytes,
-                                       int batch, const float *axis, int G, int slice_begin,
-                                       int slice_end, int apply_sigmoid, float *out, int *tile_flags,
-                                       void *workspace, void *stream) {
+                       axis, G, point_begin, m, out, apply_sigmoid, static_cast<f32x4 *>(workspace), tile_flags, static_order, fold);
+    return zs::check_launch(what) ? 1 : 0;
+}
+
+static int query_grid_impl(const char *what, const void *split_programs, size_t program_stride_bytes,
+                           int batch, const float *axis, int G, int slice_begin,
+                           int slice_end, int apply_sigmoid, float *out, int *tile_flags,
+                           void *workspace, void *stream, int fold) {
     if (batch < 0 || G <= 0 || slice_begin < 0 || slice_end > G || slice_begin > slice_end) {
-        zs::set_err("zs_sdf_query_grid_split: bad range (batch=%d G=%d slices=[%d,%d))", batch, G,
+        zs::set_err("%s: bad range (batch=%d G=%d slices=[%d,%d))", what, batch, G,
                     slice_begin, slice_end);
         return 0;
     }
     const long long mm = (long long)(slice_end - slice_begin) * G * G;
     if (batch == 0 || mm == 0) return 1;
     if (!axis || !out || !workspace) {
-        zs::set_err("zs_sdf_query_grid_split: null pointer");
+        zs::set_err("%s: null pointer", what);
         return 0;
     }
     if (mm > 0x7fffffffLL - PTS_PER_BLOCK) {
-        zs::set_err("zs_sdf_query_grid_split: %lld points per launch exceed 2^31; split the slab", mm);
+        zs::set_err("%s: %lld points per launch exceed 2^31; split the slab", what, mm);
         return 0;
     }
-    if (!check_programs("zs_sdf_query_grid_split", split_programs, program_stride_bytes)) return 0;
+    if (!check_programs(what, split_programs, program_stride_bytes, fold)) return 0;
     const int m = (int)mm;
     const int static_order = launch_counter_reset(workspace, static_cast<hipStream_t>(stream));
     hipLaunchKernelGGL((sdf_decode_split_kernel<true>), dim3(decode_grid_size(batch, m)),
                        dim3(WAVES * 64), 0, static_cast<hipStream_t>(stream),
                        static_cast<const char *>(split_programs), program_stride_bytes, batch, nullptr,
                        axis, G, (long long)slice_begin * G * G, m, out, apply_sigmoid,
-                       static_cast<f32x4 *>(workspace), tile_flags, static_order);
-    return zs::check_launch("zs_sdf_query_grid_split") ? 1 : 0;
-}
+                       static_cast<f32x4 *>(workspace), tile_flags, static_order, fold);
+    return zs::check_launch(what) ? 1 : 0;
+}
+
+extern "C" int zs_sdf_query_points_split(const void *split_programs, size_t program_stride_bytes, int batch,
+                                         const float *points, int m, float *logits, int *tile_flags, void *workspace,
+                                         void *stream) {
+    return query_points_impl("zs_sdf_query_points_split", split_programs, program_stride_bytes, batch, points, m, logits,
+                             tile_flags, workspace, stream, 0);
+}
+extern "C" int zs_sdf_query_grid_range_split(const void *split_programs, size_t program_stride_bytes, int batch,
+                                             const float *axis, int G, long long point_begin, long long point_end,
+                                             int apply_sigmoid, float *out, int *tile_flags, void *workspace, void *stream) {
+    return query_grid_range_impl("zs_sdf_query_grid_range_split", split_programs, program_stride_bytes, batch, axis, G,
+                                 point_begin, point_end, apply_sigmoid, out, tile_flags, workspace, stream, 0);
+}
+extern "C" int zs_sdf_query_grid_split(const void *split_programs, size_t program_stride_bytes, int batch,
+                                       const float *axis, int G, int slice_begin, int slice_end, int apply_sigmoid,
+                                       float *out, int *tile_flags, void *workspace, void *stream) {
+    return query_grid_impl("zs_sdf_query_grid_split", split_programs, program_stride_bytes, batch, axis, G, slice_begin,
+                           slice_end, apply_sigmoid, out, tile_flags, workspace, stream, 0);
+}
+extern "C" int zs_sdf_query_points_fold(const void *folded_programs, size_t program_stride_bytes, int batch,
+                                        const float *points, int m, float *logits, int *tile_flags, void *workspace,
+                                        void *stream) {
+    return query_points_impl("zs_sdf_query_points_fold", folded_programs, program_stride_bytes, batch, points, m, logits,
+                             tile_flags, workspace, stream, 1);
+}
+extern "C" int zs_sdf_query_grid_range_fold(const void *folded_programs, size_t program_stride_bytes, int batch,
+                                            const float *axis, int G, long long point_begin, long long point_end,
+                                            int apply_sigmoid, float *out, int *tile_flags, void *workspace, void *stream) {
+    return query_grid_range_impl("zs_sdf_query_grid_range_fold", folded_programs, program_stride_bytes, batch, axis, G,
+                                 point_begin, point_end, apply_sigmoid, out, tile_flags, workspace, stream, 1);
+}
+extern "C" int zs_sdf_query_grid_fold(const void *folded_programs, size_t program_stride_bytes, int batch,
+                                      const float *axis, int G, int slice_begin, int slice_end, int apply_sigmoid,
+                                      float *out, int *tile_flags, void *workspace, void *stream) {
+    return query_grid_impl("zs_sdf_query_grid_fold", folded_programs, program_stride_bytes, batch, axis, G, slice_begin,
+                           slice_end, apply_sigmoid, out, tile_flags, workspace, stream, 1);
+}
diff --git a/zeroshape_amd/csrc/sdf_layout.h b/zeroshape_amd/csrc/sdf_layout.h
--- a/zeroshape_amd/csrc/sdf_layout.h
+++ b/zeroshape_amd/csrc/sdf_layout.h
@@ -36,6 +36,21 @@
 constexpr int P_KMAX = 13616;
 constexpr int P_PHASE_B = 8192;
 
+constexpr int FKB_HEAD = LT * 3 + NT * 2;
+constexpr int FG_BLOCK0 = HEADS * FKB_HEAD * 2 + HT * G_MLP_TILE;
+constexpr int FG_TOTAL = FG_BLOCK0 + (BLOCKS - 1) * G_BLOCK + G_IMPL;
+constexpr int FREC_FLOATS = (FG_TOTAL + RING) * GROUP_FLOATS;
+constexpr int FP_FOLD = PARAM_FLOATS;
+constexpr int FB_VC0 = 0, FB_VC1 = 256, FB_VC2 = 768, FB_VC3 = 1024, FB_VC4 = 1280;
+constexpr int FB_R = 3328;
+constexpr int FB_M = 3344;
+constexpr int FB_T = 3600;
+constexpr int FB_WINDOW = 3856;
+constexpr int FB_QT = 4096;
+constexpr int FOLD_FLOATS = FB_QT + HEADS * 5 * HD;
+constexpr int FPARAM_FLOATS = PARAM_FLOATS + FOLD_FLOATS;
+constexpr int FPROGRAM_FLOATS = FREC_FLOATS + FPARAM_FLOATS;
+
 constexpr int LQ_WLP = 0, LQ_BLP = 65536, LQ_POS = 65792, LQ_LN1G0 = 116224, LQ_LN1B0 = 116480,
               LQ_WQKV0 = 116736, LQ_BQKV0 = 313344, LQ_WPROJ0 = 314112, LQ_BPROJ0 = 379648,
               LQ_LN2G0 = 379904, LQ_LN2B0 = 380160, LQ_W1 = 380416, LQ_B1 = 642560,
diff --git a/zeroshape_amd/model/shape/implicit.py b/zeroshape_amd/model/shape/implicit.py
--- a/zeroshape_amd/model/shape/implicit.py
+++ b/zeroshape_amd/model/shape/implicit.py
@@ -53,8 +53,9 @@
 
 class DecoderState(object):
 
-    def __init__(self, programs, batch, precision="f32", exact=None):
+    def __init__(self, programs, batch, precision="f32", exact=None, folded=None):
         self.programs, self.batch, self.precision, self.exact = programs, batch, precision, exact
+        self.folded = folded
         self.image_flags = None
         self.image_flags_occ = None
         self.check_event = None
@@ -64,6 +65,11 @@
     @property
     def stride_bytes(self):
         return self.programs.stride(0) * 4
+
+    def split_launch(self):
+        if self.folded is not None and os.environ.get("ZS_SPLIT_FOLD0", "1") != "0":
+            return "fold", self.folded, self.folded.stride(0) * 4
+        return "split", self.programs, self.stride_bytes
 
 
 class Implicit(nn.Module):
@@ -158,8 +164,22 @@
             sd = {k: v.detach().float().cpu().numpy() for k, v in self.state_dict().items()}
             prog = torch.from_numpy(P.pack_program(sd)).to(device)
             lat = torch.from_numpy(P.pack_latent_params(sd)).to(device)
-            self._packed = (key, prog, lat, P.split_envelope(sd)[0])
+            fold = torch.from_numpy(P.fold_params(sd)).to(device)
+            self._packed = (key, prog, lat, P.split_envelope(sd)[0], fold)
         return self._packed[1], self._packed[2]
+
+    def _fold(self, programs, split):
+        lib = _lib.load()
+        assert lib.zs_sdf_fold_program_bytes() == P.FPROGRAM_BYTES, "layout mismatch between program.py and the library"
+        self.packed(programs.device)
+        fold = self._packed[4]
+        folded = torch.empty(programs.shape[0], P.FPROGRAM_FLOATS, dtype=torch.float32, device=programs.device)
+        with _lib.on(programs.device):
+            rc = lib.zs_sdf_fold_programs(_lib.ptr(programs), programs.stride(0) * 4, _lib.ptr(split), split.stride(0) * 4,
+                                          _lib.ptr(fold), _lib.ptr(folded), folded.stride(0) * 4, programs.shape[0],
+                                          _lib.current_stream_ptr(programs.device))
+        _lib.check(rc, "zs_sdf_fold_programs")
+        return folded
 
     @property
     def last_calibration(self):
@@ -212,7 +232,7 @@
         return stats, flags
 
     @torch.no_grad()
-    def _calibrate(self, split, exact):
+    def _calibrate(self, split, exact, folded=None):
         key = self._weights_key()
         if self._calibration is not None and self._calibration[0] == key:
             self.last_calibration = self._calibration[1]
@@ -224,7 +244,7 @@
         guard, flags = self.envelope_guard, self.last_tile_flags
         self.envelope_guard = False
         try:
-            raw = DecoderState(split[:1], 1, "f16x3", exact=exact[:1])
+            raw = DecoderState(split[:1], 1, "f16x3", exact=exact[:1], folded=None if folded is None else folded[:1])
             got = self.query_points(raw, pts)
         finally:
             self.envelope_guard, self.last_tile_flags = guard, flags
@@ -275,18 +295,19 @@
                 rc = lib.zs_sdf_split_programs(_lib.ptr(programs), programs.stride(0) * 4, _lib.ptr(split),
                                                split.stride(0) * 4, B, _lib.current_stream_ptr(lat.device))
             _lib.check(rc, "zs_sdf_split_programs")
+            folded = self._fold(programs, split)
             if not calibrate:
-                return DecoderState(split, B, "f16x3", exact=programs)
-            ok, ok_occ = self._calibrate(split, programs)
+                return DecoderState(split, B, "f16x3", exact=programs, folded=folded)
+            ok, ok_occ = self._calibrate(split, programs, folded)
             if ok or ok_occ:
-                state = DecoderState(split, B, "f16x3", exact=programs)
+                state = DecoderState(split, B, "f16x3", exact=programs, folded=folded)
                 state.logit_ok, state.occ_ok = ok, ok_occ
                 if self.image_check:
                     self._launch_image_check(state, split, programs, shard)
                 return state
         return DecoderState(programs, B)
 
-    def _sharded_image_check(self, split, exact, shard, streams=None):
+    def _sharded_image_check(self, split, exact, shard, streams=None, folded=None):
         rank, world, exchange = shard
         B = split.shape[0]
         k = (B + world - 1) // world
@@ -294,7 +315,8 @@
         ctx = (lambda st: torch.cuda.stream(st)) if streams is not None else (lambda st: contextlib.nullcontext())
         mine = len(range(rank, B, world))
         if mine:
-            f, f_occ, mx, mx_occ = self._image_check(split[rank::world], exact[rank::world], streams=streams)
+            f, f_occ, mx, mx_occ = self._image_check(split[rank::world], exact[rank::world], streams=streams,
+                                                     folded=None if folded is None else folded[rank::world])
         with ctx(a):
             own = torch.zeros(k, 2, dtype=torch.int32, device=split.device)
             maxima = torch.full((B,), -1.0, dtype=torch.float32, device=split.device)
@@ -310,7 +332,8 @@
         main = torch.cuda.current_stream(dev)
         if torch.cuda.is_current_stream_capturing() or os.environ.get("ZS_DECODER_CHECK_INLINE", "0") != "0":
             state.image_flags, state.image_flags_occ, maxima, maxima_occ = \
-                self._image_check(split, exact) if shard is None else self._sharded_image_check(split, exact, shard)
+                self._image_check(split, exact, folded=state.folded) if shard is None else \
+                self._sharded_image_check(split, exact, shard, folded=state.folded)
             self._last_check_event = None
         else:
             pair = self._check_streams.get(str(dev))
@@ -325,25 +348,25 @@
                 head.record(st_)
                 main.wait_event(head)
             state.image_flags, state.image_flags_occ, maxima, maxima_occ = \
-                self._image_check(split, exact, streams=(side, side2)) if shard is None else \
-                self._sharded_image_check(split, exact, shard, streams=(side, side2))
+                self._image_check(split, exact, streams=(side, side2), folded=state.folded) if shard is None else \
+                self._sharded_image_check(split, exact, shard, streams=(side, side2), folded=state.folded)
             state.check_event = torch.cuda.Event()
             state.check_event.record(side)
             if os.environ.get("ZS_DECODER_CHECK_RECORD_STREAM", "0") != "0":
-                for t in (split, exact):
+                for t in (split, exact) + ((state.folded,) if state.folded is not None else ()):
                     t.record_stream(side)
                     t.record_stream(side2)
             else:
                 while self._check_keepalive and self._check_keepalive[0][0].query():
                     self._check_keepalive.pop(0)
-                self._check_keepalive.append((state.check_event, split, exact))
+                self._check_keepalive.append((state.check_event, split, exact, state.folded))
             for t in (state.image_flags, state.image_flags_occ, maxima, maxima_occ):
                 t.record_stream(main)
             self._last_check_event = state.check_event
         self._last_calibration = dict(self._last_calibration, per_image_max_abs_diff=maxima, per_image_max_abs_occ_diff=maxima_occ)
 
     @torch.no_grad()
-    def _image_check(self, split, exact, streams=None):
+    def _image_check(self, split, exact, streams=None, folded=None):
         B = split.shape[0]
         a, b = streams if streams is not None else (None, None)
         ctx = (lambda st: torch.cuda.stream(st)) if streams is not None else (lambda st: contextlib.nullcontext())
@@ -357,7 +380,7 @@
         self.envelope_guard = False
         try:
             with ctx(b):
-                got = self.query_points(DecoderState(split, B, "f16x3", exact=exact), pts)
+                got = self.query_points(DecoderState(split, B, "f16x3", exact=exact, folded=folded), pts)
         finally:
             self.envelope_guard, self.last_tile_flags = guard, flags
         if b is not None:
@@ -406,9 +429,10 @@
             flags = self._tile_flags(state.batch, M, pts.device, state)
             ws, st = _lib.ptr(self.workspace(pts.device)), _lib.current_stream_ptr(pts.device)
             with _lib.on(pts.device):
-                rc = lib.zs_sdf_query_points_split(_lib.ptr(state.programs), state.stride_bytes, state.batch,
-                                                   _lib.ptr(pts), M, _lib.ptr(out), _lib.ptr(flags), ws, st)
-                _lib.check(rc, "zs_sdf_query_points_split")
+                arm, progs, stride = state.split_launch()
+                fn = "zs_sdf_query_points_" + arm
+                rc = getattr(lib, fn)(_lib.ptr(progs), stride, state.batch, _lib.ptr(pts), M, _lib.ptr(out), _lib.ptr(flags), ws, st)
+                _lib.check(rc, fn)
                 self._join_image_check(state, flags)
                 if flags is not None:
                     rc = lib.zs_sdf_query_points(_lib.ptr(state.exact), state.exact.stride(0) * 4, state.batch,
@@ -445,10 +469,11 @@
             flags = self._tile_flags(state.batch, (slice_end - slice_begin) * G * G, axis.device, state)
             ws, st = _lib.ptr(self.workspace(axis.device)), _lib.current_stream_ptr(axis.device)
             with _lib.on(axis.device):
-                rc = lib.zs_sdf_query_grid_split(_lib.ptr(state.programs), state.stride_bytes, state.batch,
-                                                 _lib.ptr(axis), G, slice_begin, slice_end,
-                                                 1 if apply_sigmoid else 0, _lib.ptr(out), _lib.ptr(flags), ws, st)
-                _lib.check(rc, "zs_sdf_query_grid_split")
+                arm, progs, stride = state.split_launch()
+                fn = "zs_sdf_query_grid_" + arm
+                rc = getattr(lib, fn)(_lib.ptr(progs), stride, state.batch, _lib.ptr(axis), G, slice_begin, slice_end,
+                                      1 if apply_sigmoid else 0, _lib.ptr(out), _lib.ptr(flags), ws, st)
+                _lib.check(rc, fn)
                 self._join_image_check(state, flags, occupancy=bool(apply_sigmoid))
                 if flags is not None:
                     rc = lib.zs_sdf_query_grid(_lib.ptr(state.exact), state.exact.stride(0) * 4, state.batch,
@@ -482,10 +507,11 @@
         with _lib.on(axis.device):
             if state.precision == "f16x3":
                 flags = self._tile_flags(state.batch, point_end - point_begin, axis.device, state)
-                rc = lib.zs_sdf_query_grid_range_split(_lib.ptr(state.programs), state.stride_bytes, state.batch,
-                                                       _lib.ptr(axis), G, point_begin, point_end, sig, _lib.ptr(out),
-                                                       _lib.ptr(flags), ws, st)
-                _lib.check(rc, "zs_sdf_query_grid_range_split")
+                arm, progs, stride = state.split_launch()
+                fn = "zs_sdf_query_grid_range_" + arm
+                rc = getattr(lib, fn)(_lib.ptr(progs), stride, state.batch, _lib.ptr(axis), G, point_begin, point_end, sig,
+                                      _lib.ptr(out), _lib.ptr(flags), ws, st)
+                _lib.check(rc, fn)
                 self._join_image_check(state, flags, occupancy=bool(apply_sigmoid))
                 if flags is not None:
                     rc = lib.zs_sdf_query_grid_range(_lib.ptr(state.exact), state.exact.stride(0) * 4, state.batch,
diff --git a/zeroshape_amd/program.py b/zeroshape_amd/program.py
--- a/zeroshape_amd/program.py
+++ b/zeroshape_amd/program.py
@@ -369,3 +369,110 @@
             row = sq[:, :32] + sq[:, 32:]
             out[blk, h] = np.sqrt(row.max())
     return out
+
+
+FKB_HEAD = LT * 3 + NT * 2
+FG_BLOCK0 = HEADS * FKB_HEAD * 2 + HT * G_MLP_TILE
+FG_TOTAL = FG_BLOCK0 + (BLOCKS - 1) * G_BLOCK + G_IMPL
+FREC_FLOATS = (FG_TOTAL + RING) * GROUP_FLOATS
+FP_FOLD = PARAM_FLOATS
+FB_VC = (0, 256, 768, 1024, 1280)
+FB_R, FB_M, FB_T, FB_WINDOW, FB_QT = 3328, 3344, 3600, 3856, 4096
+FOLD_FLOATS = FB_QT + HEADS * 5 * HD
+FPARAM_FLOATS = PARAM_FLOATS + FOLD_FLOATS
+FPROGRAM_FLOATS = FREC_FLOATS + FPARAM_FLOATS
+FPROGRAM_BYTES = FPROGRAM_FLOATS * 4
+LN_EPS = 1e-6
+assert PARAMS.blk[0]["bproj"] - PARAMS.blk[0]["ln1_g"] == 512 and BLOCK_PARAM_FLOATS == FB_R
+
+
+def fold_terms(sd):
+    g = lambda k: np.asarray(sd[k], np.float64)
+    W = np.concatenate([g("point_proj.proj.weight"), g("point_proj.proj.bias")[:, None]], 1)
+    C0 = W - W.mean(0, keepdims=True)
+    R = np.linalg.qr(C0 / np.sqrt(C), mode="r")
+    R = R * np.where(np.diag(R) < 0, -1.0, 1.0)[:, None]
+    p = "blocks_attn.0."
+    F = np.concatenate([g(p + "norm1.weight")[:, None] * C0, g(p + "norm1.bias")[:, None]], 1)
+    Wqkv, bqkv = g(p + "attn.qkv.weight"), g(p + "attn.qkv.bias")
+    out = dict(R=R, F=F)
+    for name, part in (("Q", 0), ("K", 1), ("V", 2)):
+        Wt = Wqkv[part * C:(part + 1) * C].reshape(HEADS, HD, C)
+        X = Wt @ F
+        X[:, :, 4] += bqkv[part * C:(part + 1) * C].reshape(HEADS, HD)
+        out[name] = X
+    out["M"] = np.einsum("hdi,hdj->hij", out["Q"], out["K"])
+    T = np.stack([np.linalg.qr(out["Q"][h], mode="r") for h in range(HEADS)])
+    out["T"] = T
+    return out
+
+
+def fold_params(sd):
+    f = fold_terms(sd)
+    blockp = pack_params(sd)[PARAMS.blk[0]["ln1_g"]:PARAMS.blk[0]["ln1_g"] + BLOCK_PARAM_FLOATS]
+    out = np.zeros(FOLD_FLOATS, np.float64)
+    out[:BLOCK_PARAM_FLOATS] = blockp
+    for c in range(5):
+        out[FB_VC[c]:FB_VC[c] + C] = f["V"][:, :, c].reshape(-1)[(32 * np.arange(NT))[:, None, None] + ROW_TABLE[None]].reshape(-1)
+    out[FB_R:FB_R + 16] = f["R"].reshape(-1)
+    for h in range(HEADS):
+        out[FB_M + 32 * h:FB_M + 32 * h + 25] = f["M"][h].reshape(-1)
+        out[FB_T + 32 * h:FB_T + 32 * h + 25] = f["T"][h].reshape(-1)
+    out[FB_QT:] = f["Q"].transpose(0, 2, 1).reshape(-1)
+    return out.astype(np.float32)
+
+
+def fold_source_kblocks():
+    n = FREC_FLOATS // GROUP_FLOATS // 2
+    kb_head, kb_qkv, att0 = G_HEAD // 2, G_QKV_HEAD // 2, HEADS * FKB_HEAD
+    src = np.arange(n) + HEADS * kb_head - att0
+    for hd in range(HEADS):
+        for w in range(FKB_HEAD):
+            lt = w // 3
+            if w >= LT * 3:
+                s = hd * kb_head + kb_qkv + LT * 4 + (w - LT * 3)
+            elif w % 3:
+                s = hd * kb_head + kb_qkv + lt * 4 + 1 + w % 3
+            else:
+                s = -1
+            src[hd * FKB_HEAD + w] = s
+    return src
+
+
+def score_records(prog, fparams):
+    prog = np.ascontiguousarray(prog, np.float32)
+    qt = fparams[FB_QT:].astype(np.float64).reshape(HEADS, 5, HD)
+    out = np.zeros((HEADS, LT, 64, 8), np.float32)
+    for h in range(HEADS):
+        o = kv_group_offset(0, h) * GROUP_FLOATS
+        g = prog[o:o + G_KV_HEAD * GROUP_FLOATS].reshape(LT, 8, 64, 4)[:, :4]
+        rec = g.transpose(0, 1, 3, 2).reshape(LT, 16, 64)
+        K = np.zeros((LT * 32, HD))
+        for hi in range(2):
+            K[:, ROW_TABLE[hi]] = rec[:, :, 32 * hi:32 * hi + 32].transpose(0, 2, 1).reshape(LT * 32, 16)
+        A = K @ qt[h].T
+        A[L:] = 0
+        out[h, :, :32, :5] = A.reshape(LT, 32, 5)
+    return out
+
+
+def fold_program(prog, split_words, fparams):
+    kbw = KB_WORDS
+    rec = split_words[:REC_FLOATS].reshape(-1, kbw)
+    src = fold_source_kblocks()
+    out = np.zeros((src.size, kbw), np.uint32)
+    out[src >= 0] = rec[src[src >= 0]]
+    A = score_records(prog, fparams)
+    hi16, hif = f16_round(A)
+    with np.errstate(invalid="ignore"):
+        lo16, _ = f16_round(A - hif)
+    sc = np.stack([hi16, lo16], axis=2).reshape(HEADS, LT, -1).view(np.uint32)
+    for h in range(HEADS):
+        for lt in range(LT):
+            out[h * FKB_HEAD + 3 * lt] = sc[h, lt]
+    params = split_words[REC_FLOATS:].copy()
+    fw = fparams.view(np.uint32)
+    bad = params[P_FLAG] != 0 or not (np.all(np.isfinite(A)) and float(np.abs(A).max()) <= F16_MAX) or \
+        not (np.all(np.isfinite(fparams[:FB_WINDOW])) and float(np.abs(fparams[:FB_WINDOW]).max()) <= F16_MAX)
+    params[P_FLAG] = 1 if bad else 0
+    return np.concatenate([out.reshape(-1), params, fw])
```

Result: slower. 29.12 million points/s, median of 2 (-61.7%).
